# RuanJohn/Mava

Measured on AMD Instinct MI355X. Metric: env-steps/sec (whole node), ff_mappo RWARE tiny-4ag, higher is better.
Workload: dtype f32 via 2 x f16 split operands on the MFMA (3 products, f32 accumulate); 1 GPU; ff_mappo RWARE tiny-4ag-shaped synthetic obs, 4096 envs/GPU (update_batch_size=1 x num_envs=4096), rollout_length=128, ppo_epochs=4, num_minibatches=2, agents=4, obs=70/264, actions=5, one step = one PPO update = 524288 env-steps per GPU; parallelism=dp1

## Files before the change

### include/mava_hip.h

```cpp
#ifndef MAVA_HIP_H
#define MAVA_HIP_H

#include <stddef.h>
#include <stdint.h>

#ifdef __cplusplus
extern "C" {
#endif

typedef struct ihipStream_t* mava_stream_t;

const char* mava_last_error(void);
int mava_abi_version(void);

typedef struct mava_ctx mava_ctx;
enum {
  MAVA_CTX_MATMUL_MODE = 0,
  MAVA_CTX_CRITIC_AGGREGATION = 1,
  MAVA_CTX_GAE_VARIANT = 2,
  MAVA_CTX_POLICY_VARIANT = 3,
  MAVA_CTX_H2_LAUNCHES = 4,
  MAVA_CTX_TRAIN_VARIANT = 5,
  MAVA_CTX_W8_LAUNCHES = 6,
  MAVA_CTX_W1_SPLIT_FRESH = 7,
  MAVA_CTX_EXACT_TILES = 8,
  MAVA_CTX_X16_LAUNCHES = 9
};
int mava_ctx_create(mava_ctx** out);
int mava_ctx_destroy(mava_ctx* ctx);
int mava_ctx_set(mava_ctx* ctx, int key, long value);
int mava_ctx_get(const mava_ctx* ctx, int key, long* value);

int mava_gae_f32(const mava_ctx* ctx, const float* reward, const float* value, const uint8_t* done,
                 const float* last_val, const uint8_t* last_done, int T, int N, float gamma,
                 float lambda, float* adv, float* tgt, mava_stream_t s);

int mava_permutation_i32(long n, uint64_t seed, uint64_t counter, int32_t* out, mava_stream_t s);
int mava_permutation_batched_i32(long n, uint64_t seed, uint64_t counter, int n_perm, int32_t* out, long out_stride,
                                 mava_stream_t s);

int mava_clip_adam(float* p, const float* g, float* m, float* v, int32_t* count,
                   const int* seg_off, const float* seg_lr, int n_seg, float grad_scale,
                   float max_norm, int decay, int steps_per_update, int num_updates, float b1,
                   float b2, float eps, const float* loss_sums, float vf_coef, float ent_coef,
                   float* metrics_out, mava_stream_t s);

size_t mava_ppo_finish_workspace_bytes(int Pa, int Pc);
int mava_ppo_finish_f32(mava_ctx* ctx, const float* slab_a, long stride_a, const float* slab_c, long stride_c, int n_slab,
                        int Pa, int Pc, float* g, float* p, float* m, float* v, int32_t* count, float lr_a, float lr_c,
                        float grad_scale, float max_norm, int decay, int steps_per_update, int num_updates, float b1,
                        float b2, float eps, float vf_coef, float ent_coef, float* metrics_out, int critic_din,
                        void* workspace, size_t workspace_bytes, mava_stream_t s);

int mava_slab_reduce_f32(const float* slab, int n_slab, long slab_stride, int n, int accumulate,
                         float* out, mava_stream_t s);

int mava_slab_reduce2_f32(const float* slab, int n_slab, long slab_stride, int n_main,
                          float* out_main, int n_tail, float* out_tail, int accumulate,
                          mava_stream_t s);

int mava_mlp_param_count(int din, int n_out);

int mava_mlp_forward_f32(const mava_ctx* ctx, const float* params, int din, int n_out, const float* x, int x_share,
                         int rows, float* out, mava_stream_t s);

int mava_policy_step_f32(const mava_ctx* ctx, const float* actor_params, int actor_din, int n_actions,
                         const float* agents_view, const uint8_t* action_mask,
                         const float* critic_params, int critic_din, const float* critic_input,
                         int critic_share, int critic_rows, int value_broadcast, int rows,
                         uint64_t seed, uint32_t step, const uint32_t* step_base, uint32_t row_offset, int greedy,
                         const int32_t* forced_action, int32_t* action, float* log_prob,
                         float* value, float* logits, mava_stream_t s);


int mava_adv_stats_blocks(void);

int mava_adv_stats_f64(const float* advantages, const int32_t* idx, long idx_base, int Rb, int A,
                       double* partials, mava_stream_t s);
int mava_adv_stats_batched_f64(const float* advantages, const int32_t* idx, long idx_stride, int Rb, int A,
                               int n_batch, double* partials, mava_stream_t s);

int mava_ppo_actor_grad_f32(mava_ctx* ctx, const float* params, int din, int n_actions, const float* agents_view,
                            const uint8_t* action_mask, const int32_t* action,
                            const float* old_log_prob, const float* advantages,
                            const double* adv_stats, const int32_t* idx, long idx_base, int Rb,
                            int A, float clip_eps, float ent_coef, float* slab, long slab_stride,
                            int n_slab, mava_stream_t s);

int mava_policy_step_continuous_f32(const mava_ctx* ctx, const float* actor_params, int actor_din, int action_dim, float min_scale,
                                    const float* agents_view, const float* critic_params, int critic_din,
                                    const float* critic_input, int critic_share, int critic_rows,
                                    int value_broadcast, int rows, uint64_t seed, uint32_t step,
                                    const uint32_t* step_base, uint32_t row_offset, int greedy,
                                    const float* forced_action, float* action, float* log_prob, float* value,
                                    float* mean, mava_stream_t s);
int mava_ppo_actor_grad_continuous_f32(const float* params, int din, int action_dim, float min_scale, const float* agents_view,
                                       const float* action, const float* old_log_prob, const float* advantages,
                                       const double* adv_stats, const int32_t* idx, long idx_base, int Rb, int A,
                                       float clip_eps, float ent_coef, uint64_t seed, uint32_t ent_step,
                                       uint32_t row_offset, float* slab, long slab_stride, int n_slab,
                                       mava_stream_t s);

int mava_ppo_critic_grad_f32(mava_ctx* ctx, const float* params, int din, const float* critic_input, int x_share,
                             const float* old_value, const float* targets, const int32_t* idx,
                             long idx_base, int Rb, int A, float clip_eps, float vf_coef,
                             float* slab, long slab_stride, int n_slab, mava_stream_t s);

int mava_ppo_critic_grad_x16_f32(mava_ctx* ctx, const float* params, int din, const float* critic_input, int x_share,
                                 const float* old_value, const float* targets, const int32_t* idx,
                                 long idx_base, int Rb, int A, float clip_eps, float vf_coef,
                                 float* slab, long slab_stride, int n_slab, const uint16_t* input16,
                                 const uint32_t* input16_valid, mava_stream_t s);


int mava_synth_rware_step(int E, int A, int O, int n_actions, int gs_tiles, int state_dim, int time_limit,
                          uint64_t seed, uint32_t t, const uint32_t* t_base, uint32_t env_offset, int is_reset,
                          int32_t* step_count, float* run_return, int32_t* run_length,
                          float* ep_return, int32_t* ep_length, float* agents_view,
                          float* global_state, uint8_t* action_mask, int32_t* obs_step_count,
                          float* reward, uint8_t* done, float* info_return, int32_t* info_length,
                          uint8_t* info_terminal, const int32_t* action, int reward_mode, mava_stream_t s);

int mava_lbf_step(int E, int A, int F, int G, int fov, int max_agent_level, int force_coop, int individual_rewards,
                  int time_limit, uint64_t seed, uint32_t t, const uint32_t* t_base, uint32_t env_offset, int is_reset,
                  int32_t* agent_pos, int32_t* agent_level, int32_t* food_pos, int32_t* food_level, uint8_t* food_alive,
                  float* total_food_level, int32_t* step_count, float* run_return, int32_t* run_length,
                  float* ep_return, int32_t* ep_length, float* agents_view, float* global_state,
                  uint8_t* action_mask, int32_t* obs_step_count, float* reward, uint8_t* done, float* info_return,
                  int32_t* info_length, uint8_t* info_terminal, const int32_t* action, mava_stream_t s);

int mava_lbf_step_real_next(int E, int A, int F, int G, int fov, int max_agent_level, int force_coop, int individual_rewards,
                            int time_limit, uint64_t seed, uint32_t t, const uint32_t* t_base, uint32_t env_offset, int is_reset,
                            int32_t* agent_pos, int32_t* agent_level, int32_t* food_pos, int32_t* food_level, uint8_t* food_alive,
                            float* total_food_level, int32_t* step_count, float* run_return, int32_t* run_length,
                            float* ep_return, int32_t* ep_length, float* agents_view, float* global_state,
                            uint8_t* action_mask, int32_t* obs_step_count, float* reward, uint8_t* done, float* info_return,
                            int32_t* info_length, uint8_t* info_terminal, const int32_t* action, float* real_view,
                            uint8_t* real_mask, uint8_t* terminated, mava_stream_t s);

int mava_rware_step(int E, int A, int S, int R, int H, int W, int sensor_range, int time_limit, int collision_terminates,
                    const uint32_t* highway_rows, const int32_t* shelf_home, uint64_t seed, uint32_t t,
                    const uint32_t* t_base, uint32_t env_offset, int is_reset, int32_t* agent_pos, int32_t* agent_dir,
                    int32_t* agent_carry, int32_t* shelf_pos, int32_t* request_queue, int32_t* step_count,
                    float* run_return, int32_t* run_length, float* ep_return, int32_t* ep_length, float* agents_view,
                    float* global_state, uint8_t* action_mask, int32_t* obs_step_count, float* reward, uint8_t* done,
                    float* info_return, int32_t* info_length, uint8_t* info_terminal, const int32_t* action,
                    mava_stream_t s);

int mava_rware_step_real_next(int E, int A, int S, int R, int H, int W, int sensor_range, int time_limit,
                              int collision_terminates, const uint32_t* highway_rows, const int32_t* shelf_home,
                              uint64_t seed, uint32_t t, const uint32_t* t_base, uint32_t env_offset, int is_reset,
                              int32_t* agent_pos, int32_t* agent_dir, int32_t* agent_carry, int32_t* shelf_pos,
                              int32_t* request_queue, int32_t* step_count, float* run_return, int32_t* run_length,
                              float* ep_return, int32_t* ep_length, float* agents_view, float* global_state,
                              uint8_t* action_mask, int32_t* obs_step_count, float* reward, uint8_t* done,
                              float* info_return, int32_t* info_length, uint8_t* info_terminal, const int32_t* action,
                              float* real_view, uint8_t* real_mask, uint8_t* terminated, mava_stream_t s);

int mava_connector_step(int E, int A, int G, int time_limit, uint64_t seed, uint32_t t, const uint32_t* t_base,
                        uint32_t env_offset, int is_reset, int32_t* head, int32_t* target, uint8_t* connected,
                        uint8_t* grid, int32_t* step_count, float* run_return, int32_t* run_length, float* ep_return,
                        int32_t* ep_length, float* agents_view, float* global_state, uint8_t* action_mask,
                        int32_t* obs_step_count, float* reward, uint8_t* done, float* info_return, int32_t* info_length,
                        uint8_t* info_terminal, const int32_t* action, mava_stream_t s);

// ... 31 lines not shown
int mava_smax_step_real_next(int E, int A, int Ne, uint64_t ally_types, uint64_t enemy_types, int time_limit,
                             int see_enemy_actions, int walls_cause_death, uint64_t seed, uint32_t t,
                             const uint32_t* t_base, uint32_t env_offset, int is_reset, float* pos, float* health,
                             int32_t* cd, int32_t* last_action, int32_t* step_count, float* run_return,
                             int32_t* run_length, float* ep_return, int32_t* ep_length, float* agents_view,
                             float* global_state, uint8_t* action_mask, int32_t* obs_step_count, float* reward,
                             uint8_t* done, float* info_return, int32_t* info_length, uint8_t* info_terminal,
                             uint8_t* info_won, const int32_t* action, float* real_view, uint8_t* real_mask,
                             uint8_t* terminated, mava_stream_t s);

int mava_spread_step(int E, int A, int add_agent_id, int time_limit, uint64_t seed, uint32_t t, const uint32_t* t_base,
                     uint32_t env_offset, int is_reset, float* agent_pos, float* landmark_pos, int32_t* step_count,
                     float* run_return, int32_t* run_length, float* ep_return, int32_t* ep_length, float* agents_view,
                     float* global_state, uint8_t* action_mask, int32_t* obs_step_count, float* reward, uint8_t* done,
                     float* info_return, int32_t* info_length, uint8_t* info_terminal, const float* action,
                     mava_stream_t s);

int mava_spread_step_real_next(int E, int A, int add_agent_id, int time_limit, uint64_t seed, uint32_t t,
                               const uint32_t* t_base, uint32_t env_offset, int is_reset, float* agent_pos,
                               float* landmark_pos, int32_t* step_count, float* run_return, int32_t* run_length,
                               float* ep_return, int32_t* ep_length, float* agents_view, float* global_state,
                               uint8_t* action_mask, int32_t* obs_step_count, float* reward, uint8_t* done,
                               float* info_return, int32_t* info_length, uint8_t* info_terminal, const float* action,
                               float* real_view, uint8_t* real_mask, uint8_t* terminated, float* real_state,
                               mava_stream_t s);

int mava_rollout_ff_f32(const float* actor_params, int n_actions, const float* critic_params, int critic_shared,
                        int E, int A, int O, int T, int time_limit, uint64_t policy_seed, uint64_t env_seed,
                        uint32_t t0, uint32_t row_offset, uint32_t env_offset, int reward_mode,
                        int32_t* step_count, float* run_return, int32_t* run_length, float* ep_return,
                        int32_t* ep_length, float* agents_view, float* global_state, uint8_t* action_mask,
                        int32_t* obs_step_count, int32_t* action, float* value, float* reward, float* log_prob,
                        uint8_t* done, float* last_val, float* info_return, int32_t* info_length,
                        uint8_t* info_terminal, float* adv, float* tgt, float gamma, float gae_lambda, mava_stream_t s);
int mava_rollout_ff_tail_f32(const float* actor_params, int n_actions, const float* critic_params, int critic_shared,
                             int E, int A, int O, int T, int time_limit, uint64_t policy_seed, uint64_t env_seed,
                             uint32_t t0, uint32_t row_offset, uint32_t env_offset, int reward_mode,
                             int32_t* step_count, float* run_return, int32_t* run_length, float* ep_return,
                             int32_t* ep_length, float* agents_view, float* global_state, uint8_t* action_mask,
                             int32_t* obs_step_count, int32_t* action, float* value, float* reward, float* log_prob,
                             uint8_t* done, float* last_val, float* info_return, int32_t* info_length,
                             uint8_t* info_terminal, float* adv, float* tgt, float gamma, float gae_lambda,
                             float* last_reward, uint8_t* last_done, int32_t* step_counter, mava_stream_t s);
int mava_rollout_ff_x16_f32(const float* actor_params, int n_actions, const float* critic_params, int critic_shared,
                            int E, int A, int O, int T, int time_limit, uint64_t policy_seed, uint64_t env_seed,
                            uint32_t t0, uint32_t row_offset, uint32_t env_offset, int reward_mode,
                            int32_t* step_count, float* run_return, int32_t* run_length, float* ep_return,
                            int32_t* ep_length, float* agents_view, float* global_state, uint8_t* action_mask,
                            int32_t* obs_step_count, int32_t* action, float* value, float* reward, float* log_prob,
                            uint8_t* done, float* last_val, float* info_return, int32_t* info_length,
                            uint8_t* info_terminal, float* adv, float* tgt, float gamma, float gae_lambda,
                            float* last_reward, uint8_t* last_done, int32_t* step_counter, uint16_t* state16,
                            uint32_t* state16_valid, mava_stream_t s);
int mava_rollout_carry(int T, int E, int A, int obs_dim, long gs_dim, int n_actions, float* agents_view,
                       float* global_state, uint8_t* action_mask, int32_t* step_count, mava_stream_t s);


int mava_rec_dense_f32(const mava_ctx* ctx, const float* x, int x_rowmajor, const int32_t* idx, int Rm, int E, int A,
                       int x_share, int x_ld, int accumulate, const float* w, int ldw, const float* bias,
                       const float* gate, float* y, int y_ld, int K, int N, int rows, int relu, mava_stream_t s);

int mava_rec_xty_f32(const mava_ctx* ctx, const float* x, int x_rowmajor, const int32_t* idx, int Rm, int E, int A,
                     int x_share, int x_ld, const float* y, int y_ld, const float* y_tail, int y_split, int y_tail_ld, int K, int N,
                     int rows, int want_bias, float out_scale, float* slab, long slab_stride, int n_slab, mava_stream_t s);
int mava_rec_gather_t32_f32(const float* x, const int32_t* idx, int Rm, int E, int A, int x_share, int x_ld, int K,
                            int rows, int k_pad, float* out, mava_stream_t s);

int mava_gru_scan_fwd_f32(const mava_ctx* ctx, int T, int Rm, int E, int A, const int32_t* idx, const uint8_t* done,
                          const float* h0, int h0_t32, const float* wh, const float* bhn,
                          const float* gi, float* hs, float* hprev, float* saved, mava_stream_t s);

int mava_gru_scan_bwd_f32(const mava_ctx* ctx, int T, int Rm, int E, int A, const int32_t* idx, const uint8_t* done,
                          const float* wh, const float* saved, const float* hprev, const float* dh_out,
                          float* dgi, float* dgh, int dgh_n_only, mava_stream_t s);

int mava_seq_actor_loss_f32(int T, int Rm, int E, int A, int n_actions, const int32_t* idx,
                            const float* logits, const uint8_t* mask, const int32_t* action,
                            const float* old_log_prob, const float* advantages, const double* adv_stats,
                            int n_stats, float clip_eps, float ent_coef, float grad_scale, float* dlogits,
                            float* loss_partials, int n_blocks, mava_stream_t s);
int mava_seq_actor_loss_continuous_f32(int T, int Rm, int E, int A, int action_dim, float min_scale, const int32_t* idx,
                                       const float* mean, const float* log_std, const float* log_std_rows,
                                       const float* action, const float* old_log_prob, const float* advantages,
                                       const double* adv_stats, int n_stats, float clip_eps, float ent_coef, uint64_t seed,
                                       uint32_t ent_step, uint32_t row_offset, float grad_scale, float* dmean,
                                       float* dlog_std_rows, float* loss_partials, float* dscale_partials, int n_blocks,
                                       mava_stream_t s);
int mava_seq_sample_continuous_f32(int rows, int action_dim, float min_scale, const float* mean, const float* log_std,
                                   const float* log_std_rows, uint64_t seed,
                                   uint32_t step, uint32_t row_offset, int greedy, float* action, float* log_prob,
                                   mava_stream_t s);
int mava_seq_critic_loss_f32(int T, int Rm, int E, int A, int agents_per_row, const int32_t* idx, const float* values,
                             const float* old_value, const float* targets, float clip_eps, float vf_coef,
                             float grad_scale, float* dvalues, float* loss_partials, int n_blocks, mava_stream_t s);

int mava_rec_out_f32(int T, int Rm, int E, int A, int n_out, int agents_per_row, const int32_t* idx, const float* hs,
                     const float* params_post_head, const uint8_t* mask, const int32_t* action, const float* f0,
                     const float* f1, const double* adv_stats, int n_stats, float clip_eps, float coef, float grad_scale,
                     int is_actor, float* dh, float* slab, long slab_stride, int n_slab, mava_stream_t s);

int mava_seq_sample_f32(int rows, int n_actions, const float* logits, const uint8_t* mask, uint64_t seed,
                        uint32_t step, uint32_t row_offset, int greedy, int32_t* action, float* log_prob,
                        mava_stream_t s);

int mava_rec_step_f32(const float* actor_params, int actor_din, int n_actions, const float* agents_view,
                      const uint8_t* action_mask, const uint8_t* done_a, const float* h_actor_in,
// ... 131 lines not shown
```

### mava_amd/_lib.py

```python
from __future__ import annotations

import ctypes as C
import os
from typing import Optional

import torch

_HERE = os.path.dirname(os.path.abspath(__file__))
LIB_PATH = os.environ.get("MAVA_LIB_PATH") or os.path.join(_HERE, "libmavahip.so")

_lib: Optional[C.CDLL] = None


class MavaHipError(RuntimeError):
    pass


vp = C.c_void_p
i32 = C.c_int
u32 = C.c_uint32
u64 = C.c_uint64
f32 = C.c_float
lng = C.c_long

_SIGNATURES = {
    "mava_abi_version": [],
    "mava_ctx_create": [vp],
    "mava_ctx_destroy": [vp],
    "mava_ctx_set": [vp, i32, lng],
    "mava_ctx_get": [vp, i32, vp],
    "mava_gae_f32": [vp, vp, vp, vp, vp, vp, i32, i32, f32, f32, vp, vp, vp],
    "mava_permutation_i32": [lng, u64, u64, vp, vp],
    "mava_permutation_batched_i32": [lng, u64, u64, i32, vp, lng, vp],
    "mava_clip_adam": [vp, vp, vp, vp, vp, C.POINTER(i32), C.POINTER(f32), i32, f32, f32, i32, i32, i32,
                       f32, f32, f32, vp, f32, f32, vp, vp],
    "mava_slab_reduce_f32": [vp, i32, lng, i32, i32, vp, vp],
    "mava_ppo_finish_workspace_bytes": [i32, i32],
    "mava_ppo_finish_f32": [vp, vp, lng, vp, lng, i32, i32, i32, vp, vp, vp, vp, vp, f32, f32, f32, f32, i32, i32, i32, f32, f32, f32,
                            f32, f32, vp, i32, vp, C.c_size_t, vp],
    "mava_slab_reduce2_f32": [vp, i32, lng, i32, vp, i32, vp, i32, vp],
    "mava_mlp_param_count": [i32, i32],
    "mava_mlp_forward_f32": [vp, vp, i32, i32, vp, i32, i32, vp, vp],
    "mava_policy_step_f32": [vp, vp, i32, i32, vp, vp, vp, i32, vp, i32, i32, i32, i32, u64, u32, vp, u32, i32,
                             vp, vp, vp, vp, vp, vp],
    "mava_policy_step_continuous_f32": [vp, vp, i32, i32, f32, vp, vp, i32, vp, i32, i32, i32, i32, u64, u32, vp, u32, i32, vp, vp, vp, vp, vp, vp],
    "mava_ppo_actor_grad_continuous_f32": [vp, i32, i32, f32, vp, vp, vp, vp, vp, vp, lng, i32, i32, f32, f32, u64, u32, u32, vp, lng, i32, vp],
    "mava_seq_actor_loss_continuous_f32": [i32, i32, i32, i32, i32, f32, vp, vp, vp, vp, vp, vp, vp, vp, i32, f32, f32, u64, u32, u32, f32, vp, vp, vp, vp, i32, vp],
    "mava_seq_sample_continuous_f32": [i32, i32, f32, vp, vp, vp, u64, u32, u32, i32, vp, vp, vp],
    "mava_adv_stats_blocks": [],
    "mava_adv_stats_f64": [vp, vp, lng, i32, i32, vp, vp],
    "mava_adv_stats_batched_f64": [vp, vp, lng, i32, i32, i32, vp, vp],
    "mava_ppo_actor_grad_f32": [vp, vp, i32, i32, vp, vp, vp, vp, vp, vp, vp, lng, i32, i32, f32, f32, vp, lng, i32,
                                vp],
    "mava_ppo_critic_grad_f32": [vp, vp, i32, vp, i32, vp, vp, vp, lng, i32, i32, f32, f32, vp, lng, i32, vp],
    "mava_ppo_critic_grad_x16_f32": [vp, vp, i32, vp, i32, vp, vp, vp, lng, i32, i32, f32, f32, vp, lng, i32, vp, vp, vp],
    "mava_synth_rware_step": [i32, i32, i32, i32, i32, i32, i32, u64, u32, vp, u32, i32] + [vp] * 14 + [vp, i32, vp],
    "mava_lbf_step": [i32] * 9 + [u64, u32, vp, u32, i32] + [vp] * 21 + [vp],
    "mava_lbf_step_real_next": [i32] * 9 + [u64, u32, vp, u32, i32] + [vp] * 24 + [vp],
    "mava_rware_step": [i32] * 9 + [vp, vp, u64, u32, vp, u32, i32] + [vp] * 20 + [vp],
    "mava_rware_step_real_next": [i32] * 9 + [vp, vp, u64, u32, vp, u32, i32] + [vp] * 23 + [vp],
    "mava_connector_step": [i32] * 4 + [u64, u32, vp, u32, i32] + [vp] * 19 + [vp],
    "mava_connector_step_real_next": [i32] * 4 + [u64, u32, vp, u32, i32] + [vp] * 22 + [vp],
    "mava_cleaner_step": [i32] * 5 + [u64, u32, vp, u32, i32] + [vp] * 18 + [vp],
    "mava_cleaner_step_real_next": [i32] * 5 + [u64, u32, vp, u32, i32] + [vp] * 21 + [vp],
    "mava_smax_step": [i32] * 3 + [u64, u64] + [i32] * 3 + [u64, u32, vp, u32, i32] + [vp] * 20 + [vp],
    "mava_smax_step_real_next": [i32] * 3 + [u64, u64] + [i32] * 3 + [u64, u32, vp, u32, i32] + [vp] * 23 + [vp],
    "mava_spread_step": [i32] * 4 + [u64, u32, vp, u32, i32] + [vp] * 17 + [vp],
    "mava_spread_step_real_next": [i32] * 4 + [u64, u32, vp, u32, i32] + [vp] * 21 + [vp],
    "mava_rec_q_step_f32": [vp, i32, i32, vp, vp, vp, vp, vp, i32, f32, u64, u32, u32, vp, vp, vp],
    "mava_replay_add_f32": [i32] * 6 + [vp] * 16 + [vp],
    "mava_replay_sample_f32": [i32] * 5 + [u32, i32, i32, i32, u64, u32] + [vp] * 17 + [vp],
    "mava_q_td_loss_f32": [i32, i32, i32, i32] + [vp] * 7 + [f32, f32, vp, vp, i32, vp],
    "mava_target_update_f32": [lng, vp, vp, f32, i32, vp],
    "mava_qmix_state_t32_f32": [i32] * 6 + [vp] * 4 + [vp],
    "mava_qmix_td_f32": [i32] * 7 + [vp] * 15 + [f32, f32] + [vp] * 6 + [i32, vp],
    "mava_sac_replay_add_f32": [i32] * 7 + [vp] * 14 + [vp],
    "mava_sac_replay_sample_f32": [i32] * 5 + [u32, i32, i32, u64, u32] + [vp] * 15 + [vp],
    "mava_sac_sample_f32": [i32, i32, i32, f32, vp, vp, u64, u32, u32, vp, vp, vp, vp],
    "mava_sac_concat_f32": [i32] * 7 + [vp] * 4 + [i32, vp],
    "mava_sac_q_loss_f32": [i32] * 3 + [vp] * 8 + [f32, f32] + [vp] * 4 + [i32, vp],
    "mava_sac_actor_grad_f32": [i32] * 4 + [f32] + [vp] * 9 + [i32, i32, i32, f32, f32] + [vp] * 3 + [i32, vp],
    "mava_sac_alpha_loss_f32": [i32, i32, vp, vp, f32, vp, vp, vp],
    "mava_rollout_ff_f32": [vp, i32, vp, i32, i32, i32, i32, i32, i32, u64, u64, u32, u32, u32, i32] + [vp] * 18 + [vp, vp, f32, f32, vp],
    "mava_rollout_ff_tail_f32": [vp, i32, vp, i32, i32, i32, i32, i32, i32, u64, u64, u32, u32, u32, i32] + [vp] * 18
                                + [vp, vp, f32, f32, vp, vp, vp, vp],
    "mava_rollout_ff_x16_f32": [vp, i32, vp, i32, i32, i32, i32, i32, i32, u64, u64, u32, u32, u32, i32] + [vp] * 18
                               + [vp, vp, f32, f32, vp, vp, vp, vp, vp, vp],
    "mava_rollout_carry": [i32, i32, i32, i32, lng, i32, vp, vp, vp, vp, vp],
    "mava_rec_dense_f32": [vp, vp, i32, vp, i32, i32, i32, i32, i32, i32, vp, i32, vp, vp, vp, i32, i32, i32, i32, i32, vp],
    "mava_rec_xty_f32": [vp, vp, i32, vp, i32, i32, i32, i32, i32, vp, i32, vp, i32, i32, i32, i32, i32, i32, f32, vp, lng, i32, vp],
    "mava_rec_gather_t32_f32": [vp, vp, i32, i32, i32, i32, i32, i32, i32, i32, vp, vp],
    "mava_gru_scan_fwd_f32": [vp, i32, i32, i32, i32, vp, vp, vp, i32, vp, vp, vp, vp, vp, vp, vp],
    "mava_t32_gru_mask_f32": [vp, vp, vp, i32, i32, i32, lng, vp, vp],
    "mava_t32_gru_gates_f32": [vp, vp, vp, vp, i32, lng, vp, vp, vp, vp, vp, i32, i32, vp],
    "mava_t32_gru_gates_bwd_f32": [vp, vp, vp, vp, vp, vp, vp, i32, i32, i32, lng, vp, vp, vp, vp],
    "mava_gru_scan_bwd_f32": [vp, i32, i32, i32, i32, vp, vp, vp, vp, vp, vp, vp, vp, i32, vp],
    "mava_seq_actor_loss_f32": [i32, i32, i32, i32, i32, vp, vp, vp, vp, vp, vp, vp, i32, f32, f32, f32, vp, vp, i32, vp],
    "mava_rec_step_continuous_f32": [vp, i32, i32, f32, vp, vp, vp, vp, i32, u64, u32, u32, i32, vp, vp, vp, i32, vp, i32, vp, i32, vp, vp, i32, i32, vp, vp],
    "mava_rec_step_f32": [vp, i32, i32, vp, vp, vp, vp, vp, i32, u64, u32, u32, i32, vp, vp, vp, i32, vp, i32, vp, i32, vp, vp,
                          i32, i32, vp, vp],
    "mava_seq_critic_loss_f32": [i32, i32, i32, i32, i32, vp, vp, vp, vp, f32, f32, f32, vp, vp, i32, vp],
    "mava_rec_out_f32": [i32, i32, i32, i32, i32, i32, vp, vp, vp, vp, vp, vp, vp, vp, i32, f32, f32, f32, i32, vp, vp, lng, i32, vp],
    "mava_rec_step_pack_bytes": [i32],
    "mava_t32_norm_act_f32": [vp, i32, lng, i32, vp, i32, vp, vp, vp, vp],
    "mava_t32_norm_act_bwd_f32": [vp, vp, i32, lng, i32, vp, vp, i32, vp, vp, vp],
    "mava_t32_colsum_f32": [vp, i32, lng, f32, vp, lng, i32, vp],
    "mava_t32_im2col_f32": [vp, i32, lng, i32, i32, i32, i32, i32, vp, vp],
    "mava_t32_col2im_f32": [vp, i32, lng, i32, i32, i32, i32, i32, vp, vp],
    "mava_t32_flatten_f32": [vp, lng, i32, i32, i32, vp, vp],
    "mava_comm_unique_id": [vp],
    "mava_comm_create": [vp, i32, i32, vp],
    "mava_allreduce_sum_f32": [vp, vp, C.c_size_t, vp],
    "mava_broadcast_f32": [vp, vp, C.c_size_t, i32, vp],
    "mava_comm_destroy": [vp],
    "mava_rec_step_pack_f32": [vp, i32, vp, vp],
    "mava_rec_step_packed_f32": [vp, vp, vp, i32, i32, f32, vp, vp, vp, vp, vp, i32, u64, u32, u32, i32, vp, vp, vp, vp, i32, vp, i32, vp, i32, vp, vp, i32, i32, vp, vp],
    "mava_seq_sample_f32": [i32, i32, vp, vp, u64, u32, u32, i32, vp, vp, vp],
    "mava_t32_convert_f32": [vp, i32, i32, i32, vp, vp],
    "mava_mat_attn_fwd_f32": [vp, vp, vp, lng, i32, i32, i32, i32, i32, vp, vp, i32, vp],
    "mava_mat_attn_bwd_f32": [vp, vp, vp, vp, lng, i32, i32, i32, i32, i32, vp, vp, vp, i32, vp],
    "mava_mat_ln_fwd_f32": [vp, vp, vp, vp, i32, lng, lng, vp, vp, vp, i32, vp],
    "mava_mat_ln_bwd_f32": [vp, vp, vp, vp, i32, lng, lng, f32, vp, vp, lng, i32, vp],
    "mava_mat_gelu_f32": [vp, lng, vp, vp],
    "mava_mat_gelu_bwd_f32": [vp, vp, lng, vp, vp],
    "mava_mat_shift_onehot_f32": [vp, vp, i32, i32, i32, i32, lng, i32, vp, vp],
    "mava_mat_sample_f32": [i32, i32, i32, i32, vp, vp, u64, u32, u32, i32, vp, vp, vp],
    "mava_mat_loss_f32": [i32, i32, i32, lng, vp, vp, vp, vp, vp, vp, vp, vp, vp, vp, i32, f32, f32, f32, f32, vp, vp, vp, i32, vp],
}
_RESTYPES = {"mava_last_error": C.c_char_p, "mava_rec_step_pack_bytes": C.c_long, "mava_ppo_finish_workspace_bytes": C.c_size_t}


def declared_symbols():
    return sorted(set(_SIGNATURES) | set(_RESTYPES))


def lib() -> C.CDLL:
    global _lib
    if _lib is None:
        if not os.path.exists(LIB_PATH):
            raise MavaHipError(
                f"{LIB_PATH} is missing: build it with `python -m mava_amd.build` "
                "(hipcc --offload-arch=gfx950). There is no CPU fallback."
            )
        _lib = C.CDLL(LIB_PATH)
        _lib.mava_last_error.restype = C.c_char_p
        _lib.mava_last_error.argtypes = []
        for name, args in _SIGNATURES.items():
            fn = getattr(_lib, name)
            fn.argtypes = args
            fn.restype = _RESTYPES.get(name, C.c_int)
    return _lib


class Ctx:

    MATMUL_MODE, CRITIC_AGGREGATION, GAE_VARIANT, POLICY_VARIANT, H2_LAUNCHES, TRAIN_VARIANT, W8_LAUNCHES, W1_SPLIT_FRESH = 0, 1, 2, 3, 4, 5, 6, 7
    EXACT_TILES = 8
    X16_LAUNCHES = 9

    def __init__(self, matmul_mode: str = "f32", critic_aggregation: bool = True):
        if matmul_mode not in ("f32", "f16x2"):
            raise ValueError(f"matmul_mode must be 'f16x2' or 'f32', got {matmul_mode!r}")
        h = C.c_void_p()
        check(lib().mava_ctx_create(C.byref(h)), "mava_ctx_create")
        self.handle: Optional[int] = h.value
        self.set(self.MATMUL_MODE, 1 if matmul_mode == "f16x2" else 0)
        self.set(self.CRITIC_AGGREGATION, int(bool(critic_aggregation)))

    def set(self, key: int, value: int) -> None:
        check(lib().mava_ctx_set(self.handle, key, int(value)), "mava_ctx_set")

    def get(self, key: int) -> int:
        out = C.c_long()
        check(lib().mava_ctx_get(self.handle, key, C.byref(out)), "mava_ctx_get")
        return int(out.value)

    @property
    def matmul_mode(self) -> str:
        return "f16x2" if self.get(self.MATMUL_MODE) == 1 else "f32"

    @property
    def h2_launches(self) -> int:
        return self.get(self.H2_LAUNCHES)

    def close(self) -> None:
        if getattr(self, "handle", None) is not None and _lib is not None:
            _lib.mava_ctx_destroy(self.handle)
        self.handle = None

    def __del__(self):
        try:
            self.close()
        except Exception:
            pass


def ctx_ptr(ctx: Optional["Ctx"]) -> Optional[int]:
    return None if ctx is None else ctx.handle


def check(rc: int, what: str) -> None:
    if rc != 0:
        msg = lib().mava_last_error().decode("utf-8", "replace")
        raise MavaHipError(f"{what} failed with code {rc}: {msg}")


TIMERS: Optional[dict] = None


def launch(what: str, fn, *args, ok=(0,)) -> int:
    if TIMERS is None:
# ... 21 lines not shown
```

### mava_amd/csrc/api.cpp

```cpp
#include <stdarg.h>
#include <stdio.h>
#include <string.h>

#include "common.h"
#include "ctx.h"

static thread_local char g_err[512] = "";

void mava_set_error(const char* fmt, ...) {
  va_list ap;
  va_start(ap, fmt);
  vsnprintf(g_err, sizeof(g_err), fmt, ap);
  va_end(ap);
}

extern "C" const char* mava_last_error(void) { return g_err; }

extern "C" int mava_abi_version(void) { return 3; }

enum { CTX_MATMUL_MODE = 0, CTX_CRITIC_AGGREGATION = 1, CTX_GAE_VARIANT = 2, CTX_POLICY_VARIANT = 3, CTX_H2_LAUNCHES = 4, CTX_TRAIN_VARIANT = 5, CTX_W8_LAUNCHES = 6, CTX_W1_SPLIT_FRESH = 7, CTX_EXACT_TILES = 8, CTX_X16_LAUNCHES = 9 };

extern "C" int mava_ctx_create(mava_ctx** out) {
  MAVA_ARG_CHECK(out != nullptr, 0, "mava_ctx_create: null output pointer");
  mava_ctx* c = new mava_ctx();
  c->matmul_mode = 0;
  c->critic_aggregation = 1;
  c->gae_variant = 0;
  c->policy_variant = 0;
  c->h2_launches = 0;
  c->train_variant = 0;
  c->w8_launches = 0;
  c->w1_split[0] = c->w1_split[1] = nullptr;
  for (int i = 0; i < 2; ++i) {
    c->w1_fresh[i] = 0;
    c->w1_key_params[i] = nullptr;
    c->w1_key_din[i] = c->w1_key_steps[i] = 0;
  }
  c->exact_tiles = nullptr;
  *out = c;
  return MAVA_OK;
}

extern "C" int mava_ctx_destroy(mava_ctx* c) {
  if (c == nullptr) return MAVA_OK;
  for (int i = 0; i < 2; ++i)
    if (c->w1_split[i] != nullptr) (void)hipFree(c->w1_split[i]);
  if (c->exact_tiles != nullptr) (void)hipFree(c->exact_tiles);
  delete c;
  return MAVA_OK;
}

extern "C" int mava_ctx_set(mava_ctx* c, int key, long value) {
  MAVA_ARG_CHECK(c != nullptr, 0, "mava_ctx_set: null context");
  switch (key) {
    case CTX_MATMUL_MODE:
      MAVA_ARG_CHECK(value == 0 || value == 1, 1, "mava_ctx_set: matmul mode %ld (0 = exact f32, 1 = f16x2)", value);
      c->matmul_mode = (int)value;
      c->w1_fresh[0] = c->w1_fresh[1] = 0;
      return MAVA_OK;
    case CTX_CRITIC_AGGREGATION: c->critic_aggregation = value ? 1 : 0; return MAVA_OK;
    case CTX_GAE_VARIANT: c->gae_variant = (int)value; return MAVA_OK;
    case CTX_POLICY_VARIANT: c->policy_variant = (int)value; return MAVA_OK;
    case CTX_H2_LAUNCHES: c->h2_launches = value; return MAVA_OK;
    case CTX_TRAIN_VARIANT: c->train_variant = (int)value; return MAVA_OK;
    case CTX_W8_LAUNCHES: c->w8_launches = value; return MAVA_OK;
    case CTX_W1_SPLIT_FRESH:
      MAVA_ARG_CHECK(value == 0, 1, "mava_ctx_set: MAVA_CTX_W1_SPLIT_FRESH can only be cleared (0) by the caller");
      c->w1_fresh[0] = c->w1_fresh[1] = 0;
      return MAVA_OK;
    case CTX_EXACT_TILES:
      MAVA_ARG_CHECK(value == 0, 1, "mava_ctx_set: MAVA_CTX_EXACT_TILES can only be reset (0) by the caller");
      if (c->exact_tiles != nullptr) {
        MAVA_HIP_CHECK(hipDeviceSynchronize());
        MAVA_HIP_CHECK(hipMemset(c->exact_tiles, 0, sizeof(unsigned long long)));
      }
      return MAVA_OK;
    case CTX_X16_LAUNCHES:
      MAVA_ARG_CHECK(value == 0, 1, "mava_ctx_set: MAVA_CTX_X16_LAUNCHES can only be reset (0) by the caller");
      if (c->exact_tiles != nullptr) {
        MAVA_HIP_CHECK(hipDeviceSynchronize());
        MAVA_HIP_CHECK(hipMemset(c->exact_tiles + 1, 0, sizeof(unsigned long long)));
      }
      return MAVA_OK;
    default: mava_set_error("mava_ctx_set: unknown key %d", key); return MAVA_EARG(2);
  }
}

extern "C" int mava_ctx_get(const mava_ctx* c, int key, long* value) {
  MAVA_ARG_CHECK(c != nullptr && value != nullptr, 0, "mava_ctx_get: null argument");
  switch (key) {
    case CTX_MATMUL_MODE: *value = c->matmul_mode; return MAVA_OK;
    case CTX_CRITIC_AGGREGATION: *value = c->critic_aggregation; return MAVA_OK;
    case CTX_GAE_VARIANT: *value = c->gae_variant; return MAVA_OK;
    case CTX_POLICY_VARIANT: *value = c->policy_variant; return MAVA_OK;
    case CTX_H2_LAUNCHES: *value = c->h2_launches; return MAVA_OK;
    case CTX_TRAIN_VARIANT: *value = c->train_variant; return MAVA_OK;
    case CTX_W8_LAUNCHES: *value = c->w8_launches; return MAVA_OK;
    case CTX_W1_SPLIT_FRESH: *value = c->w1_fresh[1]; return MAVA_OK;
    case CTX_EXACT_TILES:
    case CTX_X16_LAUNCHES: {
      unsigned long long n = 0;
      if (c->exact_tiles != nullptr) {
        MAVA_HIP_CHECK(hipDeviceSynchronize());
        MAVA_HIP_CHECK(hipMemcpy(&n, c->exact_tiles + (key == CTX_X16_LAUNCHES ? 1 : 0), sizeof(n), hipMemcpyDeviceToHost));
      }
      *value = (long)n;
      return MAVA_OK;
    }
    default: mava_set_error("mava_ctx_get: unknown key %d", key); return MAVA_EARG(2);
  }
}
```

### mava_amd/csrc/ppo_train.hip

```cpp
#include "mlp_core.h"
#include "ppo_train_task.h"
#include "ctx.h"
#include "tanh_normal.h"

namespace {

constexpr int STATS_BLOCKS = 128;
constexpr int LDT = 33;


#ifdef MAVA_STAMPS
#define STAMP_DECL unsigned long long st_prev = __builtin_readcyclecounter(), st_acc[16] = {0, 0, 0, 0, 0, 0, 0, 0, 0, 0, 0, 0, 0, 0, 0, 0};
#define STAMP(i)                                                   \
  do {                                                             \
    const unsigned long long st_now = __builtin_readcyclecounter(); \
    st_acc[i] += st_now - st_prev;                                 \
    st_prev = st_now;                                              \
  } while (0)
#else
#define STAMP_DECL
#define STAMP(i)
#endif

struct TrainLdsLayout {
// ... 799 lines not shown
  switch (kt) {
    case 1: return launch_xv<NO, 1, ACTOR, CONT>(tk, n_slab, s);
    case 2: return launch_xv<NO, 2, ACTOR, CONT>(tk, n_slab, s);
    case 3: return launch_xv<NO, 3, ACTOR, CONT>(tk, n_slab, s);
    case 4: return launch_xv<NO, 4, ACTOR, CONT>(tk, n_slab, s);
    case 5: case 6: return launch_xv<NO, 6, ACTOR, CONT>(tk, n_slab, s);
    case 7: case 8: case 9: return launch_xv<NO, 9, ACTOR, CONT>(tk, n_slab, s);
    default:
      mava_set_error("ppo_train: input width %d > 287 is not instantiated", tk.din);
      return MAVA_EARG(9);
  }
#endif
}

}

#ifdef MAVA_STAMPS
static unsigned long long* g_stamps = nullptr;
extern "C" int mava_debug_set_stamps(unsigned long long* p) {
  g_stamps = p;
  return MAVA_OK;
}
#else
static constexpr unsigned long long* g_stamps = nullptr;
#endif


extern "C" int mava_adv_stats_blocks(void) { return STATS_BLOCKS; }

int g_train_last_instance = 0;
extern "C" int mava_debug_train_last_instance(void) { return g_train_last_instance; }

extern "C" int mava_adv_stats_f64(const float* adv, const int32_t* idx, long idx_base, int Rb, int A,
                                  double* partials, hipStream_t s) {
  MAVA_ARG_CHECK(Rb >= 1 && A >= 1, 0, "mava_adv_stats_f64: Rb=%d A=%d", Rb, A);
  MAVA_ARG_CHECK(adv && partials, 1, "mava_adv_stats_f64: null pointer argument");
  hipLaunchKernelGGL(adv_stats_kernel, dim3(STATS_BLOCKS), dim3(256), 0, s, adv, idx, idx_base, Rb, A,
                     partials, 0L);
  MAVA_LAUNCH_CHECK();
  return MAVA_OK;
}

extern "C" int mava_adv_stats_batched_f64(const float* adv, const int32_t* idx, long idx_stride, int Rb, int A,
                                          int n_batch, double* partials, hipStream_t s) {
  MAVA_ARG_CHECK(Rb >= 1 && A >= 1 && n_batch >= 1 && n_batch <= 65535 && idx_stride >= 0, 0,
                 "mava_adv_stats_batched_f64: Rb=%d A=%d n_batch=%d idx_stride=%ld", Rb, A, n_batch, idx_stride);
  MAVA_ARG_CHECK(adv && idx && partials, 1, "mava_adv_stats_batched_f64: null pointer argument");
  hipLaunchKernelGGL(adv_stats_kernel, dim3(STATS_BLOCKS, n_batch), dim3(256), 0, s, adv, idx, 0L, Rb, A, partials,
                     idx_stride);
  MAVA_LAUNCH_CHECK();
  return MAVA_OK;
}

extern "C" int mava_ppo_actor_grad_f32(mava_ctx* ctx, const float* params, int din, int n_actions,
                                       const float* agents_view, const uint8_t* action_mask,
                                       const int32_t* action, const float* old_log_prob,
                                       const float* advantages, const double* adv_stats,
                                       const int32_t* idx, long idx_base, int Rb, int A,
                                       float clip_eps, float ent_coef, float* slab, long slab_stride,
                                       int n_slab, hipStream_t s) {
  MAVA_ARG_CHECK(din >= 1 && n_actions >= 1 && n_actions <= 32, 0,
                 "mava_ppo_actor_grad_f32: din=%d n_actions=%d unsupported", din, n_actions);
  MAVA_ARG_CHECK(Rb >= 1 && A >= 1 && n_slab >= 1 && n_slab <= 1024 && (long)Rb * A < (1L << 31), 1,
                 "mava_ppo_actor_grad_f32: Rb=%d A=%d n_slab=%d", Rb, A, n_slab);
  MAVA_ARG_CHECK(slab_stride >= mlp_param_count(din, n_actions) + 2, 2,
                 "mava_ppo_actor_grad_f32: slab_stride too small");
  MAVA_ARG_CHECK(params && agents_view && action && old_log_prob && advantages && adv_stats && slab, 3,
                 "mava_ppo_actor_grad_f32: null pointer argument");
  TrainTask tk = {};
  tk.params = params; tk.x = agents_view; tk.din = din; tk.no = n_actions; tk.xshare = 1; tk.agg = 1;
  tk.xv = pick_xv(agents_view, din); tk.A = A; tk.idx = idx; tk.idx_base = idx_base; tk.Rb = Rb;
  tk.mask = action_mask; tk.action = action; tk.old_logp = old_log_prob; tk.adv = advantages;
  tk.stats = adv_stats; tk.clip_eps = clip_eps; tk.ent_coef = ent_coef; tk.slab = slab;
  tk.slab_stride = slab_stride;
  tk.stamps = g_stamps;
  if (mava_ctx_matmul_mode(ctx) == 1) {
    const int rc = mava_train_h2_launch(ctx, tk, n_slab, true, s);
    if (rc <= 0) return rc;
  }
  if (n_actions <= 8) return dispatch_kt<8, true>(tk, n_slab, s);
  if (n_actions <= 16) return dispatch_kt<16, true>(tk, n_slab, s);
  return dispatch_kt<32, true>(tk, n_slab, s);
}

extern "C" int mava_ppo_actor_grad_continuous_f32(const float* params, int din, int action_dim, float min_scale,
                                                  const float* agents_view, const float* action,
                                                  const float* old_log_prob, const float* advantages,
                                                  const double* adv_stats, const int32_t* idx, long idx_base, int Rb,
                                                  int A, float clip_eps, float ent_coef, uint64_t seed,
                                                  uint32_t ent_step, uint32_t row_offset, float* slab,
                                                  long slab_stride, int n_slab, hipStream_t s) {
  MAVA_ARG_CHECK(din >= 1 && action_dim >= 1 && action_dim <= 16, 0,
                 "mava_ppo_actor_grad_continuous_f32: din=%d action_dim=%d unsupported (action_dim <= 16)", din,
                 action_dim);
  MAVA_ARG_CHECK(Rb >= 1 && A >= 1 && n_slab >= 1 && n_slab <= 1024 && (long)Rb * A < (1L << 31), 1,
                 "mava_ppo_actor_grad_continuous_f32: Rb=%d A=%d n_slab=%d", Rb, A, n_slab);
  MAVA_ARG_CHECK(slab_stride >= mlp_param_count(din, action_dim) + action_dim + 2, 2,
                 "mava_ppo_actor_grad_continuous_f32: slab_stride too small");
  MAVA_ARG_CHECK(params && agents_view && action && old_log_prob && advantages && adv_stats && slab, 3,
                 "mava_ppo_actor_grad_continuous_f32: null pointer argument");
  TrainTask tk = {};
  tk.params = params; tk.x = agents_view; tk.din = din; tk.no = action_dim; tk.xshare = 1; tk.agg = 1;
  tk.xv = pick_xv(agents_view, din); tk.A = A; tk.idx = idx; tk.idx_base = idx_base; tk.Rb = Rb;
  tk.action_f = action; tk.old_logp = old_log_prob; tk.adv = advantages;
  tk.stats = adv_stats; tk.clip_eps = clip_eps; tk.ent_coef = ent_coef; tk.slab = slab;
  tk.slab_stride = slab_stride;
  tk.seed_lo = (uint32_t)seed; tk.seed_hi = (uint32_t)(seed >> 32); tk.ent_step = ent_step; tk.row_offset = row_offset;
  tk.min_scale = min_scale;
  tk.stamps = g_stamps;
  if (action_dim <= 8) return dispatch_kt<8, true, true>(tk, n_slab, s);
  return dispatch_kt<16, true, true>(tk, n_slab, s);
}

static int critic_grad_impl(mava_ctx* ctx, const float* params, int din, const float* critic_input, int x_share,
                            const float* old_value, const float* targets, const int32_t* idx, long idx_base, int Rb, int A,
                            float clip_eps, float vf_coef, float* slab, long slab_stride, int n_slab, const uint16_t* input16,
                            const uint32_t* input16_valid, hipStream_t s) {
  MAVA_ARG_CHECK(din >= 1 && x_share >= 1, 0, "mava_ppo_critic_grad_f32: din=%d x_share=%d", din, x_share);
  MAVA_ARG_CHECK(Rb >= 1 && A >= 1 && n_slab >= 1 && n_slab <= 1024 && (long)Rb * A < (1L << 31), 1,
                 "mava_ppo_critic_grad_f32: Rb=%d A=%d n_slab=%d", Rb, A, n_slab);
  MAVA_ARG_CHECK(slab_stride >= mlp_param_count(din, 1) + 2, 2,
                 "mava_ppo_critic_grad_f32: slab_stride too small");
  MAVA_ARG_CHECK(params && critic_input && old_value && targets && slab, 3,
                 "mava_ppo_critic_grad_f32: null pointer argument");
  TrainTask tk = {};
  tk.params = params; tk.x = critic_input; tk.din = din; tk.no = 1; tk.xshare = x_share; tk.agg = 1;
  if (mava_ctx_critic_aggregation(ctx) && A > 1 && A <= 8 && x_share == A) {
    tk.agg = A;
    tk.xshare = 1;
  }
  tk.xv = pick_xv(critic_input, din); tk.A = A; tk.idx = idx; tk.idx_base = idx_base; tk.Rb = Rb;
  tk.old_value = old_value; tk.targets = targets; tk.clip_eps = clip_eps; tk.vf_coef = vf_coef;
  tk.slab = slab; tk.slab_stride = slab_stride;
  tk.stamps = g_stamps;
  tk.x16 = reinterpret_cast<const _Float16*>(input16); tk.x16_valid = input16_valid;
  int rc = 1;
  if (mava_ctx_matmul_mode(ctx) == 1) rc = mava_train_h2_launch(ctx, tk, n_slab, false, s);
  if (ctx != nullptr) ctx->w1_fresh[1] = 0;
  if (rc <= 0) return rc;
  return dispatch_kt<1, false>(tk, n_slab, s);
}

extern "C" int mava_ppo_critic_grad_f32(mava_ctx* ctx, const float* params, int din, const float* critic_input,
                                        int x_share, const float* old_value, const float* targets,
                                        const int32_t* idx, long idx_base, int Rb, int A,
                                        float clip_eps, float vf_coef, float* slab, long slab_stride,
                                        int n_slab, hipStream_t s) {
  return critic_grad_impl(ctx, params, din, critic_input, x_share, old_value, targets, idx, idx_base, Rb, A, clip_eps, vf_coef,
                          slab, slab_stride, n_slab, nullptr, nullptr, s);
}

extern "C" int mava_ppo_critic_grad_x16_f32(mava_ctx* ctx, const float* params, int din, const float* critic_input,
                                            int x_share, const float* old_value, const float* targets,
                                            const int32_t* idx, long idx_base, int Rb, int A,
                                            float clip_eps, float vf_coef, float* slab, long slab_stride,
                                            int n_slab, const uint16_t* input16, const uint32_t* input16_valid,
                                            hipStream_t s) {
  MAVA_ARG_CHECK((input16 == nullptr) == (input16_valid == nullptr), 3,
                 "mava_ppo_critic_grad_x16_f32: input16 and input16_valid go together");
  return critic_grad_impl(ctx, params, din, critic_input, x_share, old_value, targets, idx, idx_base, Rb, A, clip_eps, vf_coef,
                          slab, slab_stride, n_slab, input16, input16_valid, s);
}
```

### mava_amd/csrc/ppo_train_h2.hip

```cpp
#include "h2_core.h"
#include "ppo_train_task.h"
#include "ctx.h"

#include <type_traits>

#ifndef MAVA_GW_DEPTH
#define MAVA_GW_DEPTH 0
#endif
#define GW_DEPTH MAVA_GW_DEPTH
#ifndef MAVA_GW_DEPTH_WIDE
#define MAVA_GW_DEPTH_WIDE 0
#endif
#ifndef MAVA_P1_EARLY_HALVES
#define MAVA_P1_EARLY_HALVES 2
#endif
#ifndef MAVA_P1_EARLY_RING
#define MAVA_P1_EARLY_RING 3
#endif

namespace {

using namespace h2;

constexpr int STATS_BLOCKS = 128;
// ... 1022 lines not shown
      slab[Pn + 1] = ((red[4 * NO + 1] + red[4 * NO + 3]) + red[4 * NO + 5]) + red[4 * NO + 7];
    }
  } else {
#pragma unroll
    for (int q = 0; q < 16; ++q) {
      float v = aW3r[q];
#pragma unroll
      for (int m = 1; m < 32; m <<= 1) v += __shfl_xor(v, m, 64);
      if (r == 0) slab[oW3 + 32 * w + (q & 3) + 8 * (q >> 2) + 4 * h] = v * invR;
    }
    float v = ab3, l = loss_a;
    for (int o = 32; o > 0; o >>= 1) {
      v += __shfl_down(v, o, 64);
      l += __shfl_down(l, o, 64);
    }
    if (lane == 0) { red[2 * w] = v; red[2 * w + 1] = l; }
    __syncthreads();
    if (tid == 0) {
      slab[oB3] = (((red[0] + red[2]) + red[4]) + red[6]) * invR;
      slab[Pn] = ((red[1] + red[3]) + red[5]) + red[7];
      slab[Pn + 1] = 0.0f;
    }
  }
}

template <int NO, int S1, bool ACTOR, bool WIDE, int XV>
__global__ __launch_bounds__(WIDE ? 512 : 256, WIDE ? 2 : 1) void ppo_train_h2_kernel(TrainTask tk, H2Layout L,
                                                                                     const uint4* __restrict__ w1p) {
  extern __shared__ __attribute__((aligned(16))) u8 lds[];
  if constexpr (WIDE) {
    constexpr bool X16_CAPABLE = !ACTOR && XV == 4;
    bool x16 = false;
    if constexpr (X16_CAPABLE) {
      if (tk.x16_valid != nullptr) x16 = __builtin_amdgcn_readfirstlane((int)*tk.x16_valid) == 1;
    }
    if (X16_CAPABLE && x16) {
      if constexpr (X16_CAPABLE) {
        if (threadIdx.x < 256) {
          h2_body<NO, S1, ACTOR, WIDE, XV, 1, true>(tk, L, w1p, lds);
        } else {
          h2_body<NO, S1, ACTOR, WIDE, XV, 2, true>(tk, L, w1p, lds);
        }
      }
    } else if (threadIdx.x < 256) {
      h2_body<NO, S1, ACTOR, WIDE, XV, 1>(tk, L, w1p, lds);
    } else {
      h2_body<NO, S1, ACTOR, WIDE, XV, 2>(tk, L, w1p, lds);
    }
  } else {
    h2_body<NO, S1, ACTOR, WIDE, XV, 0>(tk, L, w1p, lds);
  }
}

template <int NO, int S1, bool ACTOR, bool WIDE, int XV>
int launch_h2(mava_ctx* ctx, const TrainTask& tk, int n_slab, hipStream_t s) {
  const H2Layout L = make_h2_layout<NO, S1, WIDE>(ACTOR);
  MAVA_ARG_CHECK(L.end <= 163840, 8, "ppo_train_h2: %d bytes of LDS exceed the 160 KiB of a CU", L.end);
  static bool attr_set = false;
  if (!attr_set) {
    MAVA_HIP_CHECK(hipFuncSetAttribute((const void*)ppo_train_h2_kernel<NO, S1, ACTOR, WIDE, XV>,
                                       hipFuncAttributeMaxDynamicSharedMemorySize, L.end));
    attr_set = true;
  }
  const uint4* w1p = nullptr;
  if (WIDE) {
    void*& slot = ctx->w1_split[ACTOR ? 0 : 1];
    if (slot == nullptr) MAVA_HIP_CHECK(hipMalloc(&slot, W1_SPLIT_BYTES));
    uint4* const buf = static_cast<uint4*>(slot);
    const int kind = ACTOR ? 0 : 1;
    int& fresh = ctx->w1_fresh[kind];
    const bool keyed = ctx->w1_key_params[kind] == tk.params && ctx->w1_key_din[kind] == tk.din && ctx->w1_key_steps[kind] == S1;
    if (!(fresh && keyed)) {
      hipLaunchKernelGGL((pack_w1_kernel<S1>), dim3(1), dim3(256), 0, s, tk.params, tk.din, buf, ACTOR ? 1.0f : W_SCALE_CRITIC);
      MAVA_LAUNCH_CHECK();
    }
    fresh = 0;
    w1p = buf;
    if (ctx->exact_tiles == nullptr) {
      void* word = nullptr;
      MAVA_HIP_CHECK(hipMalloc(&word, 2 * sizeof(unsigned long long)));
      ctx->exact_tiles = static_cast<unsigned long long*>(word);
      MAVA_HIP_CHECK(hipMemsetAsync(word, 0, 2 * sizeof(unsigned long long), s));
    }
  }
  TrainTask tkl = tk;
  tkl.exact_tiles = WIDE ? ctx->exact_tiles : nullptr;
  const bool x16_ok = WIDE && !ACTOR && XV == 4 && tk.x16 != nullptr && tk.x16_valid != nullptr && tk.din % 8 == 0 &&
                      (uintptr_t)tk.x16 % 16 == 0 && tk.force_xlo == 0;
  if (!x16_ok) { tkl.x16 = nullptr; tkl.x16_valid = nullptr; }
  tkl.x16_launches = x16_ok ? ctx->exact_tiles + 1 : nullptr;
  g_train_last_instance = train_instance_id(2, ACTOR, false, WIDE, NO, S1, XV);
  hipLaunchKernelGGL((ppo_train_h2_kernel<NO, S1, ACTOR, WIDE, XV>), dim3(n_slab), dim3(WIDE ? 512 : 256), L.end, s, tkl, L,
                     w1p);
  MAVA_LAUNCH_CHECK();
  return MAVA_OK;
}

template <int NO, int S1, bool ACTOR, bool WIDE>
int dispatch_xv(mava_ctx* ctx, const TrainTask& tk, int n_slab, hipStream_t s) {
  const uintptr_t a = (uintptr_t)tk.x;
  if constexpr (WIDE) {
    if (tk.din % 4 == 0 && a % 16 == 0) return launch_h2<NO, S1, ACTOR, WIDE, 4>(ctx, tk, n_slab, s);
  } else {
    if (tk.din % 2 == 0 && a % 8 == 0) return launch_h2<NO, S1, ACTOR, WIDE, 2>(ctx, tk, n_slab, s);
  }
  return launch_h2<NO, S1, ACTOR, WIDE, 1>(ctx, tk, n_slab, s);
}

template <int NO, bool ACTOR>
int dispatch_s1(mava_ctx* ctx, const TrainTask& tk, int n_slab, hipStream_t s) {
  const int s1 = (tk.din + 1 + 15) / 16;
  switch (s1) {
#ifndef MAVA_FAST_BUILD
    case 1: return dispatch_xv<NO, 1, ACTOR, false>(ctx, tk, n_slab, s);
    case 2: return dispatch_xv<NO, 2, ACTOR, false>(ctx, tk, n_slab, s);
    case 3: return dispatch_xv<NO, 3, ACTOR, false>(ctx, tk, n_slab, s);
    case 4: return dispatch_xv<NO, 4, ACTOR, false>(ctx, tk, n_slab, s);
    case 6: return dispatch_xv<NO, 6, ACTOR, false>(ctx, tk, n_slab, s);
    case 7: case 8: case 9: case 10: case 11: case 12: return dispatch_xv<NO, 12, ACTOR, true>(ctx, tk, n_slab, s);
#endif
    case 5: return dispatch_xv<NO, 5, ACTOR, false>(ctx, tk, n_slab, s);
    case 13: case 14: case 15: case 16: case 17: case 18: return dispatch_xv<NO, 18, ACTOR, true>(ctx, tk, n_slab, s);
    default: return 1;
  }
}

}

static int h2_dispatch(mava_ctx* ctx, const TrainTask& tk, int n_slab, bool actor, hipStream_t s) {
  if (actor) {
    if (tk.action_f != nullptr) return 1;
    if (tk.no <= 8) return dispatch_s1<8, true>(ctx, tk, n_slab, s);
#ifndef MAVA_FAST_BUILD
    if (tk.no <= 16) return dispatch_s1<16, true>(ctx, tk, n_slab, s);
    return dispatch_s1<32, true>(ctx, tk, n_slab, s);
#else
    return 1;
#endif
  }
  return dispatch_s1<1, false>(ctx, tk, n_slab, s);
}

int mava_train_h2_launch(mava_ctx* ctx, const TrainTask& tk_in, int n_slab, bool actor, hipStream_t s) {
  TrainTask tk = tk_in;
  tk.force_xlo = (ctx->train_variant & 2) != 0;
  if ((ctx->train_variant & 1) == 0) {
    const int rc8 = mava_train_w8_launch(tk, n_slab, actor, s);
    if (rc8 <= 0) {
      if (rc8 == 0) { ++ctx->h2_launches; ++ctx->w8_launches; }
      return rc8;
    }
  }
  const int rc = h2_dispatch(ctx, tk, n_slab, actor, s);
  if (rc == 0) ++ctx->h2_launches;
  return rc;
}
```

### mava_amd/csrc/ppo_train_task.h

```cpp
#pragma once
#include <stdint.h>

#include "common.h"

struct TrainTask {
  const float* params;
  const float* x;
  int din, no, xshare, xv;
  int A;
  int agg;
  const int32_t* idx;
  long idx_base;
  int Rb;
  const uint8_t* mask;
  const int32_t* action;
  const float* action_f;
  uint32_t seed_lo, seed_hi, ent_step, row_offset;
  float min_scale;
  const float* old_logp;
  const float* adv;
  const double* stats;
  const float* old_value;
  const float* targets;
  float clip_eps, ent_coef, vf_coef;
  float* slab;
  long slab_stride;
  unsigned long long* stamps;
  int force_xlo;
  unsigned long long* exact_tiles;
  const _Float16* x16;
  const uint32_t* x16_valid;
  unsigned long long* x16_launches;
};

struct mava_ctx;
int mava_train_w8_launch(const TrainTask& tk, int n_slab, bool actor, hipStream_t s);
int mava_train_h2_launch(mava_ctx* ctx, const TrainTask& tk, int n_slab, bool actor, hipStream_t s);

extern int g_train_last_instance;
constexpr int train_instance_id(int family, bool actor, bool cont, bool wide, int no, int k, int xv) {
  return family * 1000000 + ((actor ? 1 : 0) + (cont ? 2 : 0) + (wide ? 4 : 0)) * 100000 + no * 1000 + k * 10 + xv;
}
```

### mava_amd/csrc/ppo_train_w8.hip

```cpp
#include "h2_core.h"
#include "ppo_train_task.h"
#include "ctx.h"

namespace {

using namespace h2;
typedef float f32x4 __attribute__((ext_vector_type(4)));

constexpr int STATS_BLOCKS = 128;
#ifndef MAVA_W8_GWD
#define MAVA_W8_GWD 1
#endif
constexpr int GWD = MAVA_W8_GWD;

#ifdef MAVA_STAMPS
#define WSTAMP_DECL unsigned long long ws_prev = __builtin_readcyclecounter(), ws_acc[16] = {0, 0, 0, 0, 0, 0, 0, 0, 0, 0, 0, 0, 0, 0, 0, 0};
#define WSTAMP(i)                                                   \
  do {                                                              \
    __builtin_amdgcn_sched_barrier(0);                              \
    const unsigned long long ws_now = __builtin_readcyclecounter(); \
    ws_acc[i] += ws_now - ws_prev;                                  \
    ws_prev = ws_now;                                               \
    __builtin_amdgcn_sched_barrier(0);                              \
  } while (0)
// ... 10 lines not shown
  c = __builtin_amdgcn_mfma_f32_16x16x32_f16(a.hi, b.lo, c, 0, 0, 0);
  return __builtin_amdgcn_mfma_f32_16x16x32_f16(a.hi, b.hi, c, 0, 0, 0);
}
__device__ __forceinline__ f32x4 mfma2w_blo0(const Frag& a, const half8& bhi, f32x4 c) {
  c = __builtin_amdgcn_mfma_f32_16x16x32_f16(a.lo, bhi, c, 0, 0, 0);
  return __builtin_amdgcn_mfma_f32_16x16x32_f16(a.hi, bhi, c, 0, 0, 0);
}
__device__ __forceinline__ f32x4 mfma2w_alo0(const half8& ahi, const Frag& b, f32x4 c) {
  c = __builtin_amdgcn_mfma_f32_16x16x32_f16(ahi, b.lo, c, 0, 0, 0);
  return __builtin_amdgcn_mfma_f32_16x16x32_f16(ahi, b.hi, c, 0, 0, 0);
}
__device__ __forceinline__ f32x4 mfma3k16(const Frag4& a, const Frag4& b, f32x4 c) {
  c = __builtin_amdgcn_mfma_f32_16x16x16f16(a.lo, b.hi, c, 0, 0, 0);
  c = __builtin_amdgcn_mfma_f32_16x16x16f16(a.hi, b.lo, c, 0, 0, 0);
  return __builtin_amdgcn_mfma_f32_16x16x16f16(a.hi, b.hi, c, 0, 0, 0);
}
__device__ __forceinline__ Frag4 split4(const f32x4& v) {
  Frag4 f;
#pragma unroll
  for (int r = 0; r < 4; ++r) {
    _Float16 a, b;
    split1(v[r], a, b);
    f.hi[r] = a;
    f.lo[r] = b;
  }
  return f;
}

constexpr int WROW = 256;
constexpr int WPLANE32 = 32 * WROW;
constexpr int WIMG = 2 * WPLANE32;
constexpr int W2PLANE = 128 * WROW;
constexpr int DYROW = 48;
constexpr int DYPLANE = 32 * DYROW;
__host__ __device__ inline int w8_sw(int row) { return ((row & 3) << 1) | (((row >> 3) & 1) * 9); }
__host__ __device__ inline int w8_off(int row, int chunk) { return WROW * row + 16 * (chunk ^ w8_sw(row)); }

struct W8Layout {
  int h1, dz2, dz1, w2, xs, dy, small, end;
};
inline W8Layout make_w8_layout() {
  W8Layout L;
  L.h1 = 0;
  L.dz2 = L.h1 + WIMG;
  L.dz1 = L.dz2 + WIMG;
  L.w2 = L.dz1 + WIMG;
  L.xs = L.w2 + 2 * W2PLANE;
  L.dy = L.xs + 2 * WIMG;
  L.small = L.dy + 2 * DYPLANE;
  L.end = L.small + (32 + 16 + 16) * 4;
  return L;
}

template <int NO, int S1, int XV, int W2R, bool ACTOR, int ROLE>
__device__ __forceinline__ void w8_body(const TrainTask& tk, const W8Layout& L, u8* lds) {
  constexpr bool DO_LOSS = ROLE != 2, DO_STAGE = ROLE != 1;
  constexpr float WS = ACTOR ? 1.0f : W_SCALE_CRITIC, WU = 1.0f / WS;
  constexpr int KT1 = 2 * S1;
  u8* const H1I = lds + L.h1;
  u8* const DZ2I = lds + L.dz2;
  u8* const DZ1I = lds + L.dz1;
  u8* const W2I = lds + L.w2;
  u8* const DYI = lds + L.dy;
  float* const YP = reinterpret_cast<float*>(lds + L.dz2);
  constexpr int YSTR = (NO == 8) ? 9 : NO;
  float* const B3s = reinterpret_cast<float*>(lds + L.small);
  float* const misc = B3s + 32;
  unsigned* const xflag = reinterpret_cast<unsigned*>(misc + 2);

  const int tid = threadIdx.x;
  const int l = tid & 63, v = tid >> 6, i = l & 15, kg = l >> 4;
  const int din = tk.din, no = tk.no;
  const long R = (long)tk.Rb * tk.A;
  const float invR = 1.0f / (float)R;
  const float* const P = tk.params;
  const int oW2 = mlp_off_w2(din), oW3 = mlp_off_w3(din);

  for (int o = tid * 16; o < L.end; o += 512 * 16) *reinterpret_cast<uint4*>(lds + o) = make_uint4(0, 0, 0, 0);
  __syncthreads();
  if (tid < no) B3s[tid] = P[mlp_off_b3(din, no) + tid];
  if (tid < 64) {
    const int b = tid >> 5, row = tid & 31;
    *reinterpret_cast<_Float16*>(lds + L.xs + b * WIMG + w8_off(row, din >> 3) + 2 * (din & 7)) = (_Float16)1.0f;
  }
  {
    const int n = tid & 127, k0 = 32 * (tid >> 7);
    float carry = 0.0f;
#pragma unroll 8
    for (int k = k0; k < k0 + 32; ++k) {
      _Float16 x0, x1;
      split1_carry(P[oW2 + k * MLP_H + n] * WS, carry, x0, x1);
      const int o = w8_off(k, n >> 3) + 2 * (n & 7);
      *reinterpret_cast<_Float16*>(W2I + o) = x0;
      *reinterpret_cast<_Float16*>(W2I + W2PLANE + o) = x1;
    }
  }
  if (ACTOR && tid == 0) {
    double s1 = 0.0, s2 = 0.0;
    for (int b = 0; b < STATS_BLOCKS; ++b) { s1 += tk.stats[2 * b]; s2 += tk.stats[2 * b + 1]; }
    const double mean = s1 / (double)R;
    double var = s2 / (double)R - mean * mean;
    if (var < 0.0) var = 0.0;
    misc[0] = (float)mean;
    misc[1] = 1.0f / ((float)sqrt(var) + 1e-8f);
  }
  Frag W1f[S1], W2f[W2R > 0 ? W2R : 1];
  {
    float c1 = 0.0f, c2 = 0.0f;
#pragma unroll
// ... 40 lines not shown
  float ab2[4] = {0, 0, 0, 0}, ab3 = 0.0f, loss_a = 0.0f, loss_b = 0.0f;

  constexpr int LOSS_THREADS = 32 * NO;
  static_assert(ROLE == 0 ? LOSS_THREADS == 512 : LOSS_THREADS == 256, "role split belongs to 8 action lanes");
  const int lrow = tid / NO, lo = tid & (NO - 1);
  constexpr int TPR = (ROLE == 2) ? 8 : 16;
  const int st = (ROLE == 2) ? (tid - 256) : tid;
  const int srow = st / TPR, l16 = st % TPR;
  const int nv = din / XV;
  constexpr int NPC = (32 * S1 / XV + TPR - 1) / TPR;
  constexpr int NR = DO_STAGE ? NPC * XV : 1;
  const uint32_t Au = (uint32_t)tk.A;
  const uint32_t q_step = 32u * gridDim.x, b_step = q_step / Au, a_step = q_step % Au;
  const uint32_t b_last = (uint32_t)(R - 1) / Au, a_last = (uint32_t)(R - 1) % Au;
  struct Cursor { uint32_t q, b, a; };
  auto cursor_at = [&](int rr) {
    Cursor c;
    c.q = 32u * blockIdx.x + (uint32_t)rr;
    c.b = c.q / Au;
    c.a = c.q - c.b * Au;
    return c;
  };
  auto cursor_advance = [&](Cursor& c) {
    c.q += q_step; c.b += b_step; c.a += a_step;
    if (c.a >= Au) { c.a -= Au; c.b += 1u; }
  };
  auto cursor_gather = [&](const Cursor& c, int32_t& p_raw, uint32_t& a_out) {
    const bool in = c.q < (uint32_t)R;
    const uint32_t b = in ? c.b : b_last;
    a_out = in ? c.a : a_last;
    p_raw = tk.idx ? tk.idx[b] : (int32_t)(tk.idx_base + (long)b);
  };
  auto stage_row = [&](int32_t p_raw, uint32_t a) -> uint32_t {
    const uint32_t fr = (uint32_t)p_raw * Au + a;
    if constexpr (ACTOR) return fr;
    else return (tk.xshare == 1) ? fr : ((uint32_t)tk.xshare == Au ? (uint32_t)p_raw : fr / (uint32_t)tk.xshare);
  };
  auto stage_issue = [&](uint32_t fr, float (&xr)[NR]) {
    const float* xrow = tk.x + (long)fr * din;
#pragma unroll
    for (int k = 0; k < NPC; ++k) {
      const int c = l16 + TPR * k;
      const int cc = (c < nv) ? c : 0;
      if (XV == 2) {
        const float2 t = reinterpret_cast<const float2*>(xrow)[cc];
        xr[2 * k] = t.x; xr[2 * k + 1] = t.y;
      } else {
        xr[k] = xrow[cc];
      }
    }
  };
  u8* const xs_dummy = reinterpret_cast<u8*>(misc + 8);
  const int xsw = 16 * w8_sw(srow);
  auto stage_commit = [&](int buf, const float (&xr)[NR]) {
    u8* base = lds + L.xs + buf * WIMG + WROW * srow;
    uint32_t lo_any = 0;
#pragma unroll
    for (int k = 0; k < NPC; ++k) {
      const int c = l16 + TPR * k;
      const bool ok = c < nv;
      const int col = XV * c;
      u8* qa = ok ? (base + ((16 * (col >> 3)) ^ xsw) + 2 * (col & 7)) : xs_dummy;
      u8* qb = ok ? (qa + WPLANE32) : xs_dummy;
      if (XV == 2) {
        typedef _Float16 half2v __attribute__((ext_vector_type(2)));
        half2v a, b;
#pragma unroll
        for (int e = 0; e < 2; ++e) { _Float16 x0, x1; split1(xr[2 * k + e], x0, x1); a[e] = x0; b[e] = x1; }
        *reinterpret_cast<half2v*>(qa) = a;
        *reinterpret_cast<half2v*>(qb) = b;
        lo_any |= __builtin_bit_cast(uint32_t, b) & 0x7FFF7FFFu;
      } else {
        _Float16 x0, x1;
        split1(xr[k], x0, x1);
        *reinterpret_cast<_Float16*>(qa) = x0;
        *reinterpret_cast<_Float16*>(qb) = x1;
        lo_any |= (uint32_t)__builtin_bit_cast(uint16_t, x1) & 0x7FFFu;
      }
    }
    if (lo_any != 0) xflag[buf] = 1u;
  };
  auto load_row = [&](uint32_t fr, int& act, float& f0, float& f1, uint32_t& m) {
    if constexpr (ACTOR) {
      act = tk.action[fr];
      f0 = tk.old_logp[fr];
      f1 = tk.adv[fr];
      const uint8_t* mk = (tk.mask != nullptr && lo < no) ? (tk.mask + (long)fr * no + lo) : nullptr;
      m = 1u;
      if (mk != nullptr) m = *mk;
    } else {
      act = 0;
      f0 = tk.old_value[fr];
      f1 = tk.targets[fr];
      m = 0u;
    }
  };

  const long ntiles = (R + 31) / 32;
  long it = blockIdx.x;
  float xr[NR];
  int r_act = 0, n_act = 0;
  float r_f0 = 0.0f, r_f1 = 0.0f, n_f0 = 0.0f, n_f1 = 0.0f;
  uint32_t r_m = 1u, n_m = 1u;
  Cursor cs = cursor_at(DO_STAGE ? srow : 0), cl = cursor_at(DO_LOSS ? lrow : 0);
  int32_t ps_next = 0, pl_next = 0;
  uint32_t as_next = 0, al_next = 0;
  if (it < ntiles) {
    if constexpr (DO_STAGE) {
      cursor_gather(cs, ps_next, as_next);
      stage_issue(stage_row(ps_next, as_next), xr);
    }
    if constexpr (DO_LOSS) {
      cursor_gather(cl, pl_next, al_next);
      load_row((uint32_t)pl_next * Au + al_next, r_act, r_f0, r_f1, r_m);
    }
    if constexpr (DO_STAGE) {
      stage_commit(0, xr);
      cursor_advance(cs);
    }
    if constexpr (DO_LOSS) cursor_advance(cl);
    if (it + gridDim.x < ntiles) {
      if constexpr (DO_STAGE) { cursor_gather(cs, ps_next, as_next); cursor_advance(cs); }
      if constexpr (DO_LOSS) { cursor_gather(cl, pl_next, al_next); cursor_advance(cl); }
    }
  }
  __syncthreads();

  const int swi = w8_sw(i);
  int rdA[4];
#pragma unroll
  for (int s = 0; s < 4; ++s) rdA[s] = WROW * i + 16 * ((4 * s + kg) ^ swi);
  const int wrA = WROW * i + 16 * ((2 * v + (kg >> 1)) ^ swi) + 8 * (kg & 1);
  const int tq = i >> 2, tp = i & 3;
  const int trow = 8 * kg + tq;
  const int trb = WROW * trow + 8 * (tp & 1);
  const int thx = 16 * ((tp >> 1) ^ w8_sw(trow));
  int trA[8];
#pragma unroll
  for (int t = 0; t < 8; ++t) {
    trA[t] = trb + ((32 * t) ^ thx);
    asm volatile("" : "+v"(trA[t]));
  }
  auto tr_addr = [&](int t) -> int { return trA[t]; };
  const int trOwn = tr_addr(v);
  auto read_tr = [&](const u8* img, int plane, int a0) -> Frag {
    Frag f;
    f.hi = read_tr8(img + a0, WROW);
    f.lo = read_tr8(img + plane + a0, WROW);
    return f;
  };
  auto read_row = [&](const u8* img, int plane, int a0) -> Frag { return read_row_frag(img, plane, a0); };
  const int dyRd = DYROW * i + 8 * kg;
  const int dyTr = DYROW * trow + 8 * tp;
  int buf = 0;

  WSTAMP_DECL
  for (; it < ntiles; it += gridDim.x, buf ^= 1) {
    WSTAMP(14);
    const long itn = it + gridDim.x;
    const bool have_next = itn < ntiles;
    const u8* const XSI = lds + L.xs + buf * WIMG;
    uint32_t xrow_next = DO_STAGE ? stage_row(ps_next, as_next) : 0u, lrow_next = DO_LOSS ? ((uint32_t)pl_next * Au + al_next) : 0u;
    if constexpr (DO_STAGE) asm volatile("" : "+v"(xrow_next));
    if constexpr (DO_LOSS) asm volatile("" : "+v"(lrow_next));

    f32x4 acc[2] = {f32x4{0, 0, 0, 0}, f32x4{0, 0, 0, 0}};
    const bool x_lo = __builtin_amdgcn_readfirstlane((int)xflag[buf]) != 0 || tk.force_xlo != 0;
    if (x_lo) {
      Frag xb[2];
#pragma unroll
      for (int nt = 0; nt < 2; ++nt) xb[nt] = read_row(XSI + 4096 * nt, WPLANE32, rdA[0]);
#pragma unroll
      for (int s = 0; s < S1; ++s) {
        Frag b[2] = {xb[0], xb[1]};
        if (s + 1 < S1) {
#pragma unroll
          for (int nt = 0; nt < 2; ++nt) xb[nt] = read_row(XSI + 4096 * nt, WPLANE32, rdA[(s + 1) & 3]);
        }
#pragma unroll
        for (int nt = 0; nt < 2; ++nt) acc[nt] = mfma3w(W1f[s], b[nt], acc[nt]);
        __builtin_amdgcn_sched_barrier(0);
      }
    } else {
      half8 xb[2];
#pragma unroll
      for (int nt = 0; nt < 2; ++nt) xb[nt] = *reinterpret_cast<const half8*>(XSI + 4096 * nt + rdA[0]);
#pragma unroll
      for (int s = 0; s < S1; ++s) {
        const half8 b[2] = {xb[0], xb[1]};
        if (s + 1 < S1) {
#pragma unroll
          for (int nt = 0; nt < 2; ++nt) xb[nt] = *reinterpret_cast<const half8*>(XSI + 4096 * nt + rdA[(s + 1) & 3]);
        }
#pragma unroll
        for (int nt = 0; nt < 2; ++nt) acc[nt] = mfma2w_blo0(W1f[s], b[nt], acc[nt]);
        __builtin_amdgcn_sched_barrier(0);
      }
    }
    WSTAMP(0);
    uint32_t relu1 = 0;
#pragma unroll
    for (int nt = 0; nt < 2; ++nt) {
#pragma unroll
      for (int r = 0; r < 4; ++r) {
        acc[nt][r] = fmaxf(ACTOR ? acc[nt][r] : acc[nt][r] * WU, 0.0f);
        relu1 |= (acc[nt][r] > 0.0f) ? (1u << (4 * nt + r)) : 0u;
      }
      const Frag4 f = split4(acc[nt]);
      *reinterpret_cast<half4*>(H1I + 4096 * nt + wrA) = f.hi;
      *reinterpret_cast<half4*>(H1I + 4096 * nt + WPLANE32 + wrA) = f.lo;
    }
    WSTAMP(1);
    if (have_next) {
      if constexpr (DO_STAGE) stage_issue(xrow_next, xr);
      if constexpr (DO_LOSS) load_row(lrow_next, n_act, n_f0, n_f1, n_m);
      if (itn + gridDim.x < ntiles) {
        if constexpr (DO_STAGE) { cursor_gather(cs, ps_next, as_next); cursor_advance(cs); }
        if constexpr (DO_LOSS) { cursor_gather(cl, pl_next, al_next); cursor_advance(cl); }
      }
    }
    WSTAMP(2);
    __syncthreads();
    WSTAMP(3);
    if constexpr (DO_STAGE) {
      if (tid == (ROLE == 2 ? 256 : 0)) xflag[buf ^ 1] = 0u;
    }

    f32x4 h2[2];
#pragma unroll
    for (int nt = 0; nt < 2; ++nt) h2[nt] = f32x4{b2r[0], b2r[1], b2r[2], b2r[3]};
    {
      Frag hb[2], wn;
#pragma unroll
      for (int nt = 0; nt < 2; ++nt) hb[nt] = read_row(H1I + 4096 * nt, WPLANE32, rdA[0]);
      if constexpr (W2R < 1) wn = read_tr(W2I, W2PLANE, trOwn);
#pragma unroll
      for (int s = 0; s < 4; ++s) {
        Frag b[2] = {hb[0], hb[1]};
        const Frag a = (s < W2R) ? W2f[s < W2R ? s : 0] : wn;
        if (s + 1 < 4) {
#pragma unroll
          for (int nt = 0; nt < 2; ++nt) hb[nt] = read_row(H1I + 4096 * nt, WPLANE32, rdA[s + 1]);
          if (s + 1 >= W2R) wn = read_tr(W2I + 32 * (s + 1) * WROW, W2PLANE, trOwn);
        }
#pragma unroll
        for (int nt = 0; nt < 2; ++nt) h2[nt] = mfma3w(a, b[nt], h2[nt]);
        __builtin_amdgcn_sched_barrier(0);
      }
    }
    WSTAMP(4);
    uint32_t relu2 = 0;
#pragma unroll
    for (int nt = 0; nt < 2; ++nt) {
#pragma unroll
      for (int r = 0; r < 4; ++r) {
        h2[nt][r] = fmaxf(ACTOR ? h2[nt][r] : h2[nt][r] * WU, 0.0f);
        relu2 |= (h2[nt][r] > 0.0f) ? (1u << (4 * nt + r)) : 0u;
      }
      const Frag4 f = split4(h2[nt]);
      *reinterpret_cast<half4*>(DZ1I + 4096 * nt + wrA) = f.hi;
      *reinterpret_cast<half4*>(DZ1I + 4096 * nt + WPLANE32 + wrA) = f.lo;
      const f32x4 y = mfma3k16(W3h, f, f32x4{0, 0, 0, 0});
#pragma unroll
      for (int r = 0; r < 4; ++r) {
        if (4 * kg + r < NO) YP[(v * 32 + 16 * nt + i) * YSTR + 4 * kg + r] = y[r] * W3_UNSCALE;
      }
    }
    WSTAMP(5);
    __syncthreads();
    WSTAMP(6);

    if constexpr (DO_LOSS) {
      const float lo_c = 1.0f - tk.clip_eps, hi_c = 1.0f + tk.clip_eps;
      const bool rvalid = (it * 32 + lrow) < R;
      const float* yp = YP + lrow * YSTR + lo;
      float y = B3s[lo];
#pragma unroll
// ... 1 lines not shown
      float dyo = 0.0f, pg_row = 0.0f, ent_row = 0.0f;
      if constexpr (ACTOR) {
        const bool legal = (lo < no) && (r_m != 0u);
        const float z = legal ? y : -FLT_MAX;
        auto fmax_op = [](float a, float b) { return fmaxf(a, b); };
        auto add_op = [](float a, float b) { return a + b; };
        const float mx = group_allreduce<NO>(z, fmax_op);
        const float se = group_allreduce<NO>(expf(z - mx), add_op);
        const float logp = (mx == -FLT_MAX) ? ((lo < no) ? -logf((float)no) : -FLT_MAX) : z - (mx + logf(se));
        const float pr = expf(logp);
        const float ent = group_allreduce<NO>((pr > 0.0f) ? -(pr * logp) : 0.0f, add_op);
        const int act = r_act;
        const float lp = group_allreduce<NO>((lo == act) ? logp : 0.0f, add_op);
        const float gae = (r_f1 - adv_mean) * adv_rstd;
        const float ratio = expf(lp - r_f0);
        const float rc = fminf(fmaxf(ratio, lo_c), hi_c);
        const float l1 = ratio * gae, l2 = rc * gae;
        const float pg = -fminf(l1, l2);
        const bool inside = (ratio >= lo_c) && (ratio <= hi_c);
        const float g1 = (l1 < l2) ? 1.0f : ((l1 == l2) ? 0.5f : 0.0f);
        const float g2 = inside ? (1.0f - g1) : 0.0f;
        const float dlp = rvalid ? (-(g1 + g2) * gae * ratio) : 0.0f;
        const float ec = rvalid ? tk.ent_coef : 0.0f;
        const float oh = (lo == act) ? 1.0f : 0.0f;
        const float pl2 = (pr > 0.0f) ? logp : 0.0f;
        dyo = dlp * (oh - pr) + ec * pr * (pl2 + ent);
        if (z == -FLT_MAX) dyo = 0.0f;
        pg_row = pg;
        ent_row = ent;
      } else {
        const float ov = r_f0, tg = r_f1;
        const float diff = y - ov;
        const float vclip = ov + fminf(fmaxf(diff, -tk.clip_eps), tk.clip_eps);
        const float e1 = y - tg, e2 = vclip - tg;
        const float l1 = e1 * e1, l2 = e2 * e2;
        const bool inside = (diff >= -tk.clip_eps) && (diff <= tk.clip_eps);
        const float g1 = (l1 > l2) ? 1.0f : ((l1 == l2) ? 0.5f : 0.0f);
        const float g2 = inside ? (1.0f - g1) : 0.0f;
        dyo = (rvalid && lo == 0) ? (tk.vf_coef * (g1 * e1 + g2 * e2)) : 0.0f;
        pg_row = 0.5f * fmaxf(l1, l2);
      }
      _Float16 da, db;
      split1(dyo, da, db);
      *reinterpret_cast<_Float16*>(DYI + lrow * DYROW + 2 * lo) = da;
      *reinterpret_cast<_Float16*>(DYI + DYPLANE + lrow * DYROW + 2 * lo) = db;
      ab3 += dyo;
      if (rvalid && lo == 0) {
        loss_a += pg_row * invR;
        loss_b += ent_row * invR;
      }
      r_act = n_act; r_f0 = n_f0; r_f1 = n_f1; r_m = n_m;
    }
    if constexpr (DO_STAGE) {
      if (have_next) stage_commit(buf ^ 1, xr);
    }
    WSTAMP(7);
    __syncthreads();
    WSTAMP(8);

    {
      Frag a, b;
      a.hi = read_tr8(DYI + dyTr, DYROW);
      a.lo = read_tr8(DYI + DYPLANE + dyTr, DYROW);
      b = read_tr(DZ1I, WPLANE32, trOwn);
      gW3 = mfma3w(a, b, gW3);
    }
    f32x4 dz[2];
#pragma unroll
    for (int nt = 0; nt < 2; ++nt) {
      Frag4 b;
      b.hi = *reinterpret_cast<const half4*>(DYI + 16 * nt * DYROW + dyRd);
      b.lo = *reinterpret_cast<const half4*>(DYI + DYPLANE + 16 * nt * DYROW + dyRd);
      dz[nt] = mfma3k16(W3d, b, f32x4{0, 0, 0, 0});
#pragma unroll
      for (int r = 0; r < 4; ++r) {
        dz[nt][r] = ((relu2 >> (4 * nt + r)) & 1u) ? dz[nt][r] * W3_UNSCALE : 0.0f;
        ab2[r] += dz[nt][r];
      }
      const Frag4 f = split4(dz[nt]);
      *reinterpret_cast<half4*>(DZ2I + 4096 * nt + wrA) = f.hi;
      *reinterpret_cast<half4*>(DZ2I + 4096 * nt + WPLANE32 + wrA) = f.lo;
    }
    WSTAMP(9);
    {
      const Frag b = read_tr(DZ2I, WPLANE32, trOwn);
      Frag an[GWD];
#pragma unroll
      for (int t = 0; t < GWD; ++t) an[t] = read_tr(H1I, WPLANE32, tr_addr(t));
#pragma unroll
      for (int t = 0; t < 8; ++t) {
        const Frag a = an[t % GWD];
        if (t + GWD < 8) an[t % GWD] = read_tr(H1I, WPLANE32, tr_addr(t + GWD));
        gW2[t] = mfma3w(a, b, gW2[t]);
        __builtin_amdgcn_sched_barrier(0);
      }
    }
    WSTAMP(10);
    __syncthreads();
    WSTAMP(11);

    {
      acc[0] = f32x4{0, 0, 0, 0};
      acc[1] = f32x4{0, 0, 0, 0};
      Frag an = read_row(W2I + 4096 * v, W2PLANE, rdA[0]);
      Frag bn[2];
#pragma unroll
      for (int nt = 0; nt < 2; ++nt) bn[nt] = read_row(DZ2I + 4096 * nt, WPLANE32, rdA[0]);
// ... 6 lines not shown
#pragma unroll
          for (int nt = 0; nt < 2; ++nt) bn[nt] = read_row(DZ2I + 4096 * nt, WPLANE32, rdA[s + 1]);
        }
#pragma unroll
        for (int nt = 0; nt < 2; ++nt) acc[nt] = mfma3w(a, b[nt], acc[nt]);
        __builtin_amdgcn_sched_barrier(0);
      }
#pragma unroll
      for (int nt = 0; nt < 2; ++nt) {
#pragma unroll
        for (int r = 0; r < 4; ++r) acc[nt][r] = ((relu1 >> (4 * nt + r)) & 1u) ? (ACTOR ? acc[nt][r] : acc[nt][r] * WU) : 0.0f;
        const Frag4 f = split4(acc[nt]);
        *reinterpret_cast<half4*>(DZ1I + 4096 * nt + wrA) = f.hi;
        *reinterpret_cast<half4*>(DZ1I + 4096 * nt + WPLANE32 + wrA) = f.lo;
      }
    }
    WSTAMP(12);
    {
      const Frag b = read_tr(DZ1I, WPLANE32, trOwn);
      constexpr int D1 = GWD < KT1 ? GWD : KT1;
      if (x_lo) {
        Frag an[D1];
#pragma unroll
        for (int t = 0; t < D1; ++t) an[t] = read_tr(XSI, WPLANE32, tr_addr(t));
#pragma unroll
        for (int t = 0; t < KT1; ++t) {
          const Frag a = an[t % D1];
          if (t + D1 < KT1) an[t % D1] = read_tr(XSI, WPLANE32, tr_addr(t + D1));
          gW1[t] = mfma3w(a, b, gW1[t]);
          __builtin_amdgcn_sched_barrier(0);
        }
      } else {
        half8 an[D1];
#pragma unroll
        for (int t = 0; t < D1; ++t) an[t] = read_tr8(XSI + tr_addr(t), WROW);
#pragma unroll
        for (int t = 0; t < KT1; ++t) {
          const half8 a = an[t % D1];
          if (t + D1 < KT1) an[t % D1] = read_tr8(XSI + tr_addr(t + D1), WROW);
          gW1[t] = mfma2w_alo0(a, b, gW1[t]);
          __builtin_amdgcn_sched_barrier(0);
        }
      }
    }
    WSTAMP(13);
  }
#ifdef MAVA_STAMPS
  if (tk.stamps != nullptr && blockIdx.x == 0 && l == 0) {
    for (int k = 0; k < 16; ++k) tk.stamps[v * 16 + k] = ws_acc[k];
  }
#endif

  __syncthreads();
  float* slab = tk.slab + (long)blockIdx.x * tk.slab_stride;
  const int oB2 = mlp_off_b2(din), oB3 = mlp_off_b3(din, no);
  const int Pn = mlp_param_count(din, no);
#pragma unroll
  for (int t = 0; t < KT1; ++t)
#pragma unroll
    for (int r = 0; r < 4; ++r) {
      const int k = 16 * t + 4 * kg + r;
      if (k <= din) slab[k * MLP_H + 16 * v + i] = gW1[t][r] * invR;
    }
#pragma unroll
  for (int t = 0; t < 8; ++t)
#pragma unroll
    for (int r = 0; r < 4; ++r) slab[oW2 + (16 * t + 4 * kg + r) * MLP_H + 16 * v + i] = gW2[t][r] * invR;
#pragma unroll
  for (int r = 0; r < 4; ++r) {
    float x = ab2[r];
#pragma unroll
    for (int m = 1; m < 16; m <<= 1) x += __shfl_xor(x, m, 64);
    if (i == 0) slab[oB2 + 16 * v + 4 * kg + r] = x * invR;
    const int o = 4 * kg + r;
    if (o < no) slab[oW3 + (16 * v + i) * no + o] = gW3[r] * invR;
  }
  float* red = reinterpret_cast<float*>(lds + L.h1);
  if constexpr (DO_LOSS) {
    float x = ab3;
#pragma unroll
    for (int m = NO; m < 64; m <<= 1) x += __shfl_xor(x, m, 64);
    if (l < NO) red[v * NO + l] = x;
    for (int o = 32; o > 0; o >>= 1) {
      loss_a += __shfl_down(loss_a, o, 64);
      loss_b += __shfl_down(loss_b, o, 64);
    }
    if (l == 0) { red[8 * NO + 2 * v] = loss_a; red[8 * NO + 2 * v + 1] = loss_b; }
  }
  __syncthreads();
  constexpr int LW = LOSS_THREADS / 64;
  if (tid < no) {
    float x = 0.0f;
#pragma unroll
    for (int u = 0; u < LW; ++u) x += red[u * NO + tid];
    slab[oB3 + tid] = x * invR;
  }
  if (tid == 0) {
    float a = 0.0f, b = 0.0f;
#pragma unroll
    for (int u = 0; u < LW; ++u) { a += red[8 * NO + 2 * u]; b += red[8 * NO + 2 * u + 1]; }
    slab[Pn] = a;
    slab[Pn + 1] = b;
  }
}

constexpr int w8_w2r(int no, int s1, int xv) {
#ifdef MAVA_W8_W2R
  return MAVA_W8_W2R;
#else
  return (no == 8) ? ((s1 <= 2) ? 2 : ((s1 == 3 && xv == 2) ? 2 : 0)) : ((s1 <= 2) ? 2 : 0);
#endif
}
template <int NO, int S1, int XV, int W2R, bool ACTOR>
__global__ __launch_bounds__(512, 2) void ppo_train_w8_kernel(TrainTask tk, W8Layout L) {
  extern __shared__ __attribute__((aligned(16))) u8 lds[];
  if constexpr (NO == 8) {
    if (threadIdx.x < 256) {
      w8_body<NO, S1, XV, W2R, ACTOR, 1>(tk, L, lds);
    } else {
      w8_body<NO, S1, XV, W2R, ACTOR, 2>(tk, L, lds);
    }
  } else {
    w8_body<NO, S1, XV, W2R, ACTOR, 0>(tk, L, lds);
  }
}

template <int NO, int S1, int XV, bool ACTOR>
int launch_w8(const TrainTask& tk, int n_slab, hipStream_t s) {
  const W8Layout L = make_w8_layout();
  static bool attr_set = false;
  if (!attr_set) {
    MAVA_HIP_CHECK(hipFuncSetAttribute((const void*)ppo_train_w8_kernel<NO, S1, XV, w8_w2r(NO, S1, XV), ACTOR>, hipFuncAttributeMaxDynamicSharedMemorySize,
                                       L.end));
    attr_set = true;
  }
  g_train_last_instance = train_instance_id(3, ACTOR, false, false, NO, S1, XV);
  hipLaunchKernelGGL((ppo_train_w8_kernel<NO, S1, XV, w8_w2r(NO, S1, XV), ACTOR>), dim3(n_slab), dim3(512), L.end, s, tk, L);
  MAVA_LAUNCH_CHECK();
  return MAVA_OK;
}

template <int NO, int S1, bool ACTOR>
int dispatch_w8_xv(const TrainTask& tk, int n_slab, hipStream_t s) {
  if (tk.din % 2 == 0 && ((uintptr_t)tk.x) % 8 == 0) return launch_w8<NO, S1, 2, ACTOR>(tk, n_slab, s);
  if constexpr (S1 == 4) return 1;
  else return launch_w8<NO, S1, 1, ACTOR>(tk, n_slab, s);
}

template <int NO, bool ACTOR>
int dispatch_w8(const TrainTask& tk, int n_slab, hipStream_t s) {
  const int s1 = (tk.din + 1 + 31) / 32;
  switch (s1) {
#ifndef MAVA_FAST_BUILD
    case 1: return dispatch_w8_xv<NO, 1, ACTOR>(tk, n_slab, s);
    case 2: return dispatch_w8_xv<NO, 2, ACTOR>(tk, n_slab, s);
    case 4: return dispatch_w8_xv<NO, 4, ACTOR>(tk, n_slab, s);
#endif
    case 3: return dispatch_w8_xv<NO, 3, ACTOR>(tk, n_slab, s);
    default: return 1;
  }
}

}

int mava_train_w8_launch(const TrainTask& tk, int n_slab, bool actor, hipStream_t s) {
  if (tk.action_f != nullptr || tk.din + 1 > 128) return 1;
  if (!actor) {
    if (tk.agg > 1 || tk.no != 1) return 1;
    return dispatch_w8<8, false>(tk, n_slab, s);
  }
  if (tk.no <= 8) return dispatch_w8<8, true>(tk, n_slab, s);
#ifndef MAVA_FAST_BUILD
  if (tk.no <= 16) return dispatch_w8<16, true>(tk, n_slab, s);
#endif
  return 1;
}
```

### mava_amd/csrc/rollout_h2.hip

```cpp
#include "h2_core.h"

#ifdef MAVA_STAMPS
#define RSTAMP_DECL unsigned long long rs_prev = __builtin_readcyclecounter(), rs_acc[8] = {0, 0, 0, 0, 0, 0, 0, 0};
#define RSTAMP(i)                                                   \
  do {                                                              \
    __builtin_amdgcn_sched_barrier(0);                              \
    const unsigned long long rs_now = __builtin_readcyclecounter(); \
    rs_acc[i] += rs_now - rs_prev;                                  \
    rs_prev = rs_now;                                               \
    __builtin_amdgcn_sched_barrier(0);                              \
  } while (0)
static __device__ unsigned long long g_rollout_stamps[16];
#else
#define RSTAMP_DECL
#define RSTAMP(i)
#endif

namespace {
using namespace h2;
typedef _Float16 half2v __attribute__((ext_vector_type(2)));

constexpr uint32_t ENV_STREAM = 0x454E5653u;
constexpr uint32_t POLICY_STREAM = 0x504f4c49u;

struct RolloutArgs {
  const float* pa;
  const float* pc;
  int E, A, O, no, T, time_limit;
  uint32_t pseed_lo, pseed_hi, eseed_lo, eseed_hi;
  uint32_t t0;
  uint32_t row_offset;
  uint32_t env_offset;
  int reward_mode;
  int32_t* step_count;
  float* run_return; int32_t* run_length; float* ep_return; int32_t* ep_length;
  float* agents_view;
  float* global_state;
  uint8_t* action_mask;
  int32_t* obs_step_count;
  int32_t* action; float* value; float* reward; float* log_prob; uint8_t* done;
  float* last_val;
  float* info_return; int32_t* info_length; uint8_t* info_terminal;
  float* adv; float* tgt;
  float gamma, lam;
  float* last_reward; uint8_t* last_done; int32_t* step_counter;
  _Float16* state16; uint32_t* state16_valid;
};

#define MAVA_AS4 __attribute__((address_space(4)))
__device__ __forceinline__ const MAVA_AS4 RolloutArgs& args_here() {
  const MAVA_AS4 RolloutArgs* p = (const MAVA_AS4 RolloutArgs*)__builtin_amdgcn_kernarg_segment_ptr();
  asm volatile("" : "+s"(p));
  return *p;
}

__device__ __forceinline__ uint32_t div_small(uint32_t x, uint32_t m) { return __umul24(x, m) >> 16; }

struct RolloutLds {
  int xa, xa_row, xa_plane, xc, xc_row, xc_plane, h1, wl, ypa, ypc, act, mask, small, gum, xlf, end;
};
constexpr int W1_REG_STEPS = 12;

template <int NO, int S1A, int S1C, bool SHARED>
constexpr RolloutLds make_rollout_lds() {
  constexpr int KTA = (S1A + 1) / 2, KTC = (S1C + 1) / 2;
  RolloutLds L{};
  L.xa = 0;
  L.xa_row = 2 * 32 * KTA + 16;
  L.xa_plane = 32 * L.xa_row;
  L.xc = L.xa + 2 * 2 * L.xa_plane;
  L.xc_row = 2 * 32 * KTC + 16;
  L.xc_plane = ((S1C > W1_REG_STEPS) ? 16 : 32) * L.xc_row;
  L.h1 = L.xc + (SHARED ? 2 * L.xc_plane : 0);
  L.wl = L.h1 + (SHARED ? 3 : 4) * IMG_BYTES;
  L.ypa = L.wl + ((S1C > W1_REG_STEPS) ? (S1C - W1_REG_STEPS) * 4 * 64 * 32 : 0);
  L.ypc = L.ypa + 2 * 4 * 32 * (NO + 1) * 4;
  L.act = L.ypc + 2 * 4 * 32 * 4;
  L.mask = L.act + 64 * 4;
  L.small = L.mask + 64 * 32;
  L.gum = L.small + (128 + 32 + 128 + 4 + 128) * 4;
  L.gum = (L.gum + 15) & ~15;
  L.xlf = L.gum + 64 * NO * 4;
  L.end = L.xlf + 16;
  L.end = (L.end + 15) & ~15;
  return L;
}

template <int NO, int S1A, int S1C, bool SHARED, int ROLE>
__device__ __forceinline__ void rollout_body(const RolloutArgs& a, u8* lds) {
  constexpr bool ACT_ROLE = ROLE == 0;
  constexpr RolloutLds L = make_rollout_lds<NO, S1A, S1C, SHARED>();
  const int t512 = threadIdx.x;
  const int tid = t512 & 255, lane = tid & 63, w = tid >> 6, h = lane >> 5, r = lane & 31;
  const int A = a.A, O = a.O, no = a.no, W = A + O, E = a.E;
  const int EB = 64 / A;
  const int e0 = blockIdx.x * EB;
  const int din_a = W, din_c = SHARED ? A * O : W;
  constexpr int NTC = SHARED ? 1 : 2;
  float* const B2a = reinterpret_cast<float*>(lds + L.small);
// ... 31 lines not shown
  Frag W1r[S1REG], W2r[8], W3h[2];
  {
    float c1 = 0.0f, c2 = 0.0f;
#pragma unroll
    for (int s = 0; s < S1R; ++s) {
      float v[8];
#pragma unroll
      for (int e = 0; e < 8; ++e) {
        const int k = 16 * s + 8 * h + e;
        v[e] = (k <= din_r) ? PR[k * MLP_H + 32 * w + r] : 0.0f;
      }
      const Frag f = split8_carry(v, c1);
      if (s < S1REG) {
        W1r[s] = f;
      } else {
        WL[512 * (s - S1REG)] = __builtin_bit_cast(uint4, f.hi);
        WL[512 * (s - S1REG) + 1] = __builtin_bit_cast(uint4, f.lo);
      }
      __builtin_amdgcn_sched_barrier(0);
    }
#pragma unroll
    for (int s = 0; s < 8; ++s) {
      float v[8];
#pragma unroll
      for (int e = 0; e < 8; ++e) v[e] = PR[oW2r + (16 * s + 8 * h + e) * MLP_H + 32 * w + r];
      W2r[s] = split8_carry(v, c2);
      __builtin_amdgcn_sched_barrier(0);
    }
#pragma unroll
    for (int s = 0; s < (ACT_ROLE ? 2 : 0); ++s) {
      float v[8];
#pragma unroll
      for (int e = 0; e < 8; ++e) {
        const int f = 32 * w + 16 * s + 8 * (e >> 2) + 4 * h + (e & 3);
        v[e] = (r < no) ? a.pa[oW3a + f * no + r] * W3_SCALE : 0.0f;
      }
      W3h[s] = split8(v);
    }
  }
  {
    const long slot0_av = 0;
    uint32_t lo_any = 0, lo_gs = 0;
    for (int i = t512; i < 64 * W; i += 512) {
      const int row = i / W, c = i - row * W;
      const int e = e0 + row / A;
      const float v = (e < E) ? a.agents_view[slot0_av + ((long)e0 * A + row) * W + c] : 0.0f;
      _Float16 x0, x1;
      split1(v, x0, x1);
      u8* p = lds + L.xa + (row >> 5) * 2 * xa_plane + (row & 31) * xa_row + 2 * c;
      *reinterpret_cast<_Float16*>(p) = x0;
      *reinterpret_cast<_Float16*>(p + xa_plane) = x1;
      lo_any |= (uint32_t)__builtin_bit_cast(uint16_t, x1) & 0x7FFFu;
    }
    if (t512 < 64) {
      u8* p = lds + L.xa + (t512 >> 5) * 2 * xa_plane + (t512 & 31) * xa_row + 2 * din_a;
      *reinterpret_cast<_Float16*>(p) = (_Float16)1.0f;
    }
    if (SHARED) {
      const int gw = A * O;
      for (int i = t512; i < EB * gw; i += 512) {
        const int le = i / gw, c = i - le * gw;
        const float v = (e0 + le < E) ? a.global_state[(long)(e0 + le) * gw + c] : 0.0f;
        _Float16 x0, x1;
        split1(v, x0, x1);
        u8* p = lds + L.xc + le * xc_row + 2 * c;
        *reinterpret_cast<_Float16*>(p) = x0;
        *reinterpret_cast<_Float16*>(p + xc_plane) = x1;
        lo_gs |= (uint32_t)__builtin_bit_cast(uint16_t, x1) & 0x7FFFu;
      }
      lo_any |= lo_gs;
      if (lo_gs != 0) XLF[1] = 1u;
      if (t512 < XC_ROWS) *reinterpret_cast<_Float16*>(lds + L.xc + t512 * xc_row + 2 * din_c) = (_Float16)1.0f;
    }
    for (int i = t512; i < 64 * no; i += 512) {
      const int row = i / no, o = i - row * no;
      MASK[row * 32 + o] = (e0 + row / A < E) ? a.action_mask[((long)e0 * A + row) * no + o] : 1;
    }
    if (lo_any != 0) *XLF = 1u;
  }
  __syncthreads();

  const int lgA = __builtin_ctz((unsigned)A);
  const int bk_le = tid >> lgA, bk_ag = tid & (A - 1);
  const bool bk_on = !ACT_ROLE && tid < 64 && (e0 + bk_le) < E;
  const long bk_k = (long)e0 * A + tid;
  int sc_reg = bk_on ? a.step_count[bk_k] : 0;
  float rr_reg = 0.0f, er_reg = 0.0f;
  int rl_reg = 0, el_reg = 0;
  if (bk_on && bk_ag == 0) {
    rr_reg = a.run_return[e0 + bk_le]; rl_reg = a.run_length[e0 + bk_le];
    er_reg = a.ep_return[e0 + bk_le]; el_reg = a.ep_length[e0 + bk_le];
  }

  const bool x_lo = __builtin_amdgcn_readfirstlane((int)*XLF) != 0;
  if (SHARED && ACT_ROLE && tid == 0 && a.state16_valid != nullptr) {
    uint32_t seen = 0;
    if (XLF[1] != 0) seen = atomicOr(a.state16_valid, 0x80000000u);
    asm volatile("" : "+v"(seen) : : "memory");
    const uint32_t old = atomicAdd(a.state16_valid, 2u);
    if (((old >> 1) & 0x3FFFFFFFu) == gridDim.x - 1u) *a.state16_valid = (old & 0x80000000u) ? 0u : 1u;
  }
  const int rowB = r * IMG_ROW + 16 * h;
  const long EA = (long)E * A;
  const uint32_t nch = (O - 2 + 15) / 16 > 0 ? (O - 2 + 15) / 16 : 1;

  constexpr int NT = ACT_ROLE ? 2 : NTC;
  RSTAMP_DECL
  auto forward = [&](bool active, bool noise, uint32_t noise_step) __attribute__((always_inline)) {
    f32x16 z[NT];
#pragma unroll
    for (int i = 0; i < NT; ++i)
#pragma unroll
      for (int q = 0; q < 16; ++q) z[i][q] = 0.0f;
    if (active) {
      auto x_frag = [&](int s, int t) {
        return (!ACT_ROLE && SHARED) ? read_row_frag(lds + L.xc, xc_plane, (r & (XC_ROWS - 1)) * xc_row + 16 * h + 32 * s)
                                     : read_row_frag(lds + L.xa + t * 2 * xa_plane, xa_plane, r * xa_row + 16 * h + 32 * s);
      };
      auto w_frag = [&](int s) {
        Frag wf;
        wf.hi = __builtin_bit_cast(half8, WL[512 * (s - S1REG)]);
        wf.lo = __builtin_bit_cast(half8, WL[512 * (s - S1REG) + 1]);
        return wf;
      };
      auto x_hi = [&](int s, int t) -> half8 {
        return (!ACT_ROLE && SHARED)
                   ? *reinterpret_cast<const half8*>(lds + L.xc + (r & (XC_ROWS - 1)) * xc_row + 16 * h + 32 * s)
                   : *reinterpret_cast<const half8*>(lds + L.xa + t * 2 * xa_plane + r * xa_row + 16 * h + 32 * s);
      };
      if (x_lo) {
      Frag bn[NT], wn;
#pragma unroll
      for (int t = 0; t < NT; ++t) bn[t] = x_frag(0, t);
      if (S1REG == 0) wn = w_frag(0);
#pragma unroll
      for (int s = 0; s < S1R; ++s) {
        Frag b[NT];
#pragma unroll
        for (int t = 0; t < NT; ++t) b[t] = bn[t];
        const Frag wf = (s < S1REG) ? W1r[s < S1REG ? s : 0] : wn;
        if (s + 1 < S1R) {
#pragma unroll
          for (int t = 0; t < NT; ++t) bn[t] = x_frag(s + 1, t);
          if (s + 1 >= S1REG) wn = w_frag(s + 1);
        }
#pragma unroll
        for (int t = 0; t < NT; ++t) z[t] = mfma3(wf, b[t], z[t]);
        __builtin_amdgcn_sched_barrier(0);
      }
      } else {
      half8 bn[NT];
      Frag wn;
#pragma unroll
// ... 117 lines not shown
          part += __shfl_xor(part, 32, 64);
          if (h == 0) YPC[(t * 4 + w) * 32 + r] = part;
        }
      }
    }
    RSTAMP(2);
    __syncthreads();
    RSTAMP(3);
  };
  auto value_of = [&](int crow) -> float {
    const float* yp = YPC + (crow >> 5) * 4 * 32 + (crow & 31);
    return (((yp[0] + yp[32]) + yp[64]) + yp[96]) + B3c[0];
  };

  const int rows_ok = min(64, (E - e0) * A), envs_ok = min(EB, E - e0);
  const int AO = A * O;
  const uint32_t no_m = 65536u / (uint32_t)no + 1u, nch_m = 65536u / nch + 1u;
  const int tid_w = tid, wo_q = (W >> 1) > 0 ? (W >> 1) : 1, gs_q = (AO >> 2) > 0 ? (AO >> 2) : 1;
  const int wo_dr = 256 / wo_q, gs_dr = 256 / gs_q;
  const uint32_t wo_m = 65536u / (uint32_t)wo_q + 1u, gs_m = 65536u / (uint32_t)gs_q + 1u;
  auto write_gs = [&](long slot, bool f32_too) {
    const auto& a = args_here();
    int tid = tid_w;
    asm volatile("" : "+v"(tid));
    if (SHARED && a.global_state != nullptr) {
      float* dst = a.global_state + (slot * E + e0) * (long)AO;
      if ((AO & 3) == 0) {
        const bool h16 = a.state16 != nullptr;
        uint4* const dst16 = h16 ? reinterpret_cast<uint4*>(a.state16 + (slot * E + e0) * (long)AO) : nullptr;
        const int Q = AO >> 2, d_r = gs_dr, d_f = 256 - d_r * Q;
        int le = (int)div_small((uint32_t)tid, gs_m), k = tid - le * Q;
        for (int j = tid; j < EB * Q; j += 256) {
          if (le < envs_ok) {
            if (f32_too) {
              const half4 v = *reinterpret_cast<const half4*>(lds + L.xc + le * xc_row + 8 * k);
              reinterpret_cast<float4*>(dst)[j] = make_float4((float)v[0], (float)v[1], (float)v[2], (float)v[3]);
            }
            if (h16 && (k & 1) == 0) dst16[j >> 1] = *reinterpret_cast<const uint4*>(lds + L.xc + le * xc_row + 8 * k);
          }
          le += d_r; k += d_f;
          if (k >= Q) { k -= Q; ++le; }
        }
      } else if (f32_too) {
        const int d_r = 256 / AO, d_f = 256 - d_r * AO;
        int le = tid / AO, k = tid - le * AO;
        for (int j = tid; j < EB * AO; j += 256) {
          if (le < envs_ok) dst[j] = (float)*reinterpret_cast<const _Float16*>(lds + L.xc + le * xc_row + 2 * k);
          le += d_r; k += d_f;
          if (k >= AO) { k -= AO; ++le; }
        }
      }
    }
  };
  auto write_out = [&](long slot, bool part_gs) {
    const auto& a = args_here();
    int tid = tid_w;
    asm volatile("" : "+v"(tid));
    if (!part_gs) {
      float* dst = a.agents_view + (slot * EA + (long)e0 * A) * W;
      if ((W & 1) == 0) {
        const int W2 = W >> 1, d_r = wo_dr, d_f = 256 - d_r * W2;
        int row = (int)div_small((uint32_t)tid, wo_m), f = tid - row * W2;
        for (int j = tid; j < 64 * W2; j += 256) {
          if (row < rows_ok) {
            const u8* xa = lds + L.xa + (row >> 5) * 2 * xa_plane + (row & 31) * xa_row;
            const half2v v = *reinterpret_cast<const half2v*>(xa + 4 * f);
            reinterpret_cast<float2*>(dst)[j] = make_float2((float)v[0], (float)v[1]);
          }
          row += d_r; f += d_f;
          if (f >= W2) { f -= W2; ++row; }
        }
      } else {
        const int d_r = 256 / W, d_f = 256 - d_r * W;
        int row = tid / W, f = tid - row * W;
        for (int j = tid; j < 64 * W; j += 256) {
          if (row < rows_ok) {
            const u8* xa = lds + L.xa + (row >> 5) * 2 * xa_plane + (row & 31) * xa_row;
            dst[j] = (float)*reinterpret_cast<const _Float16*>(xa + 2 * f);
          }
          row += d_r; f += d_f;
          if (f >= W) { f -= W; ++row; }
        }
      }
    }
    if (part_gs) write_gs(slot, true);
    if (!part_gs) {
      uint8_t* dst = a.action_mask + (slot * EA + (long)e0 * A) * no;
      for (int j = tid; j < rows_ok * no; j += 256) {
        const int row = (int)div_small((uint32_t)j, no_m), o = j - row * no;
        dst[j] = MASK[row * 32 + o];
      }
    }
  };

  const int T_steps = a.T;
  const uint32_t t0 = a.t0;
  if (SHARED && ACT_ROLE && a.state16 != nullptr) write_gs(0L, false);
  for (int t = 0; t < T_steps; ++t) {
    const uint32_t step = t0 + (uint32_t)t;
    forward(true, true, step);
    const auto& a = args_here();
    if (ACT_ROLE) {
      constexpr int RPP = 256 / NO;
#pragma unroll
      for (int pass = 0; pass < 64 / RPP; ++pass) {
        const int row = pass * RPP + tid / NO, o = tid & (NO - 1);
        const float* yp = YPA + (((row >> 5) * 4) * 32 + (row & 31)) * (NO + 1) + o;
        const float y = (((yp[0] + yp[32 * (NO + 1)]) + yp[2 * 32 * (NO + 1)]) + yp[3 * 32 * (NO + 1)]) + B3a[o];
        const bool legal = (o < no) && (MASK[row * 32 + o] != 0);
        const float z = legal ? y : -FLT_MAX;
        auto fmax_op = [](float p, float q) { return fmaxf(p, q); };
        auto add_op = [](float p, float q) { return p + q; };
        const float mx = group_allreduce<NO>(z, fmax_op);
        const float se = group_allreduce<NO>(expf(z - mx), add_op);
        const float logp = (mx == -FLT_MAX) ? ((o < no) ? -logf((float)no) : -FLT_MAX) : z - (mx + logf(se));
        float sc = (o < no) ? (z + GUM[row * NO + o]) : -FLT_MAX;
        if (!(sc > -FLT_MAX)) sc = -FLT_MAX;
        int best = o;
#pragma unroll
        for (int m = 1; m < NO; m <<= 1) {
          const float so = __shfl_xor(sc, m, 64);
          const int bo = __shfl_xor(best, m, 64);
          const bool take = (so > sc) || (so == sc && bo < best);
          sc = take ? so : sc;
          best = take ? bo : best;
        }
        const float lp = group_allreduce<NO>((o == best) ? logp : 0.0f, add_op);
        const int e = e0 + (row >> lgA);
        if (o == 0) {
          ACT[row] = best;
          if (e < E) {
            const long k = (long)t * EA + (long)e0 * A + row;
            a.action[k] = best;
            a.log_prob[k] = lp;
          }
        }
      }
    } else {
      if (tid < 64 && (e0 + (tid >> lgA)) < E) {
        a.value[(long)t * EA + (long)e0 * A + tid] = value_of(SHARED ? (tid >> lgA) : tid);
      }
      if (t > 0) write_out((long)t, false);
    }
    if (ACT_ROLE && t > 0) write_out((long)t, true);
    RSTAMP(4);
    __syncthreads();
    RSTAMP(5);
    {
      const auto& a = args_here();
      const uint32_t tn = step + 1;
// ... 173 lines not shown
  if (!ACT_ROLE && blockIdx.x == 0 && tid == 0 && a.step_counter != nullptr) *a.step_counter += a.T;
  }
}

template <int NO, int S1A, int S1C, bool SHARED>
__global__ __launch_bounds__(512, 2) void rollout_h2_kernel(RolloutArgs a) {
  extern __shared__ __attribute__((aligned(16))) u8 lds[];
  if (threadIdx.x < 256) {
    rollout_body<NO, S1A, S1C, SHARED, 0>(a, lds);
  } else {
    rollout_body<NO, S1A, S1C, SHARED, 1>(a, lds);
  }
}

int g_rollout_last_instance = 0;

template <int NO, int S1A, int S1C, bool SHARED>
int launch_rollout(const RolloutArgs& a, hipStream_t s) {
  g_rollout_last_instance = NO * 100000 + S1A * 1000 + S1C * 10 + (SHARED ? 1 : 0);
  constexpr RolloutLds L = make_rollout_lds<NO, S1A, S1C, SHARED>();
  MAVA_ARG_CHECK(L.end <= 163840, 8, "mava_rollout_ff_f32: %d bytes of LDS exceed the 160 KiB of a CU", L.end);
  const int lds_bytes = L.end > 83968 ? L.end : 83968;
  static bool attr_set = false;
  if (!attr_set) {
    MAVA_HIP_CHECK(hipFuncSetAttribute((const void*)rollout_h2_kernel<NO, S1A, S1C, SHARED>,
                                       hipFuncAttributeMaxDynamicSharedMemorySize, lds_bytes));
    attr_set = true;
  }
  const int EB = 64 / a.A;
  hipLaunchKernelGGL((rollout_h2_kernel<NO, S1A, S1C, SHARED>), dim3(mava_cdiv(a.E, EB)), dim3(512), lds_bytes, s, a);
  MAVA_LAUNCH_CHECK();
  return MAVA_OK;
}

}

#ifdef MAVA_STAMPS
extern "C" int mava_debug_get_rollout_stamps(unsigned long long* out16) {
  return -(int)hipMemcpyFromSymbol(out16, HIP_SYMBOL(g_rollout_stamps), 16 * sizeof(unsigned long long));
}
#endif

extern "C" int mava_debug_rollout_last_instance(void) { return g_rollout_last_instance; }

static int rollout_ff_impl(const float* actor_params, int n_actions, const float* critic_params, int critic_shared,
                           int E, int A, int O, int T, int time_limit, uint64_t policy_seed, uint64_t env_seed,
                           uint32_t t0, uint32_t row_offset, uint32_t env_offset, int reward_mode,
                           int32_t* step_count, float* run_return, int32_t* run_length, float* ep_return,
                           int32_t* ep_length, float* agents_view, float* global_state, uint8_t* action_mask,
                           int32_t* obs_step_count, int32_t* action, float* value, float* reward, float* log_prob,
                           uint8_t* done, float* last_val, float* info_return, int32_t* info_length,
                           uint8_t* info_terminal, float* adv, float* tgt, float gamma, float gae_lambda,
                           float* last_reward, uint8_t* last_done, int32_t* step_counter, uint16_t* state16,
                           uint32_t* state16_valid, hipStream_t s) {
  MAVA_ARG_CHECK(E >= 1 && A >= 1 && O >= 2 && T >= 1 && n_actions >= 1 && time_limit >= 1, 0,
                 "mava_rollout_ff_f32: bad shape E=%d A=%d O=%d T=%d nA=%d", E, A, O, T, n_actions);
  MAVA_ARG_CHECK(actor_params && critic_params && step_count && run_return && run_length && ep_return && ep_length &&
                     agents_view && action_mask && obs_step_count && action && value && reward && log_prob && done &&
                     last_val && info_return && info_length && info_terminal && (!critic_shared || global_state),
                 1, "mava_rollout_ff_f32: null pointer argument");
  if (64 % A != 0 || n_actions > 8) return 1;
  if (critic_shared && A < 2) return 1;
  const int s1a = (A + O + 1 + 15) / 16, s1c = critic_shared ? (A * O + 1 + 15) / 16 : s1a;
  RolloutArgs a = {};
  a.pa = actor_params; a.pc = critic_params; a.E = E; a.A = A; a.O = O; a.no = n_actions; a.T = T; a.time_limit = time_limit;
  a.pseed_lo = (uint32_t)policy_seed; a.pseed_hi = (uint32_t)(policy_seed >> 32);
  a.eseed_lo = (uint32_t)env_seed; a.eseed_hi = (uint32_t)(env_seed >> 32);
  a.t0 = t0; a.row_offset = row_offset; a.env_offset = env_offset; a.reward_mode = reward_mode;
  a.step_count = step_count; a.run_return = run_return; a.run_length = run_length; a.ep_return = ep_return;
  a.ep_length = ep_length; a.agents_view = agents_view; a.global_state = critic_shared ? global_state : nullptr;
  a.action_mask = action_mask; a.obs_step_count = obs_step_count; a.action = action; a.value = value; a.reward = reward;
  a.log_prob = log_prob; a.done = done; a.last_val = last_val; a.info_return = info_return; a.info_length = info_length;
  a.info_terminal = info_terminal;
  MAVA_ARG_CHECK((adv == nullptr) == (tgt == nullptr), 1, "mava_rollout_ff_f32: adv and tgt go together");
  a.adv = adv; a.tgt = tgt; a.gamma = gamma; a.lam = gae_lambda;
  a.last_reward = last_reward; a.last_done = last_done; a.step_counter = step_counter;
  MAVA_ARG_CHECK((state16 == nullptr) == (state16_valid == nullptr), 1, "mava_rollout_ff_x16_f32: state16 and state16_valid go together");
  MAVA_ARG_CHECK(state16 == nullptr || (critic_shared && (A * O) % 8 == 0 && (uintptr_t)state16 % 16 == 0), 2,
                 "mava_rollout_ff_x16_f32: state16 needs the shared critic, A*O %% 8 == 0 (A*O=%d) and 16-byte alignment", A * O);
  a.state16 = reinterpret_cast<_Float16*>(state16); a.state16_valid = state16_valid;
  if (critic_shared) {
    if (s1a == 5 && s1c == 17 && A >= 4) return launch_rollout<8, 5, 17, true>(a, s);
#ifndef MAVA_FAST_BUILD
    if (s1a <= 2 && s1c <= 2) return launch_rollout<8, 2, 2, true>(a, s);
    if (s1a <= 2 && s1c <= 4) return launch_rollout<8, 2, 4, true>(a, s);
    if (s1a <= 5 && s1c <= 9) return launch_rollout<8, 5, 9, true>(a, s);
#endif
    return 1;
  }
  if (s1a == 5) return launch_rollout<8, 5, 5, false>(a, s);
#ifndef MAVA_FAST_BUILD
  if (s1a <= 2) return launch_rollout<8, 2, 2, false>(a, s);
#endif
  return 1;
}

extern "C" int mava_rollout_ff_f32(const float* actor_params, int n_actions, const float* critic_params, int critic_shared,
                                   int E, int A, int O, int T, int time_limit, uint64_t policy_seed, uint64_t env_seed,
                                   uint32_t t0, uint32_t row_offset, uint32_t env_offset, int reward_mode,
                                   int32_t* step_count, float* run_return, int32_t* run_length, float* ep_return,
                                   int32_t* ep_length, float* agents_view, float* global_state, uint8_t* action_mask,
                                   int32_t* obs_step_count, int32_t* action, float* value, float* reward, float* log_prob,
                                   uint8_t* done, float* last_val, float* info_return, int32_t* info_length,
                                   uint8_t* info_terminal, float* adv, float* tgt, float gamma, float gae_lambda,
                                   hipStream_t s) {
  return rollout_ff_impl(actor_params, n_actions, critic_params, critic_shared, E, A, O, T, time_limit, policy_seed, env_seed,
                         t0, row_offset, env_offset, reward_mode, step_count, run_return, run_length, ep_return, ep_length,
                         agents_view, global_state, action_mask, obs_step_count, action, value, reward, log_prob, done,
                         last_val, info_return, info_length, info_terminal, adv, tgt, gamma, gae_lambda, nullptr, nullptr,
                         nullptr, nullptr, nullptr, s);
}

extern "C" int mava_rollout_ff_tail_f32(const float* actor_params, int n_actions, const float* critic_params,
                                        int critic_shared, int E, int A, int O, int T, int time_limit,
                                        uint64_t policy_seed, uint64_t env_seed, uint32_t t0, uint32_t row_offset,
                                        uint32_t env_offset, int reward_mode, int32_t* step_count, float* run_return,
                                        int32_t* run_length, float* ep_return, int32_t* ep_length, float* agents_view,
                                        float* global_state, uint8_t* action_mask, int32_t* obs_step_count,
                                        int32_t* action, float* value, float* reward, float* log_prob, uint8_t* done,
                                        float* last_val, float* info_return, int32_t* info_length, uint8_t* info_terminal,
                                        float* adv, float* tgt, float gamma, float gae_lambda, float* last_reward,
                                        uint8_t* last_done, int32_t* step_counter, hipStream_t s) {
  MAVA_ARG_CHECK(last_reward && last_done, 1, "mava_rollout_ff_tail_f32: null pointer argument");
  return rollout_ff_impl(actor_params, n_actions, critic_params, critic_shared, E, A, O, T, time_limit, policy_seed, env_seed,
                         t0, row_offset, env_offset, reward_mode, step_count, run_return, run_length, ep_return, ep_length,
                         agents_view, global_state, action_mask, obs_step_count, action, value, reward, log_prob, done,
                         last_val, info_return, info_length, info_terminal, adv, tgt, gamma, gae_lambda, last_reward,
                         last_done, step_counter, nullptr, nullptr, s);
}

extern "C" int mava_rollout_ff_x16_f32(const float* actor_params, int n_actions, const float* critic_params,
                                       int critic_shared, int E, int A, int O, int T, int time_limit,
                                       uint64_t policy_seed, uint64_t env_seed, uint32_t t0, uint32_t row_offset,
                                       uint32_t env_offset, int reward_mode, int32_t* step_count, float* run_return,
                                       int32_t* run_length, float* ep_return, int32_t* ep_length, float* agents_view,
                                       float* global_state, uint8_t* action_mask, int32_t* obs_step_count,
                                       int32_t* action, float* value, float* reward, float* log_prob, uint8_t* done,
                                       float* last_val, float* info_return, int32_t* info_length, uint8_t* info_terminal,
                                       float* adv, float* tgt, float gamma, float gae_lambda, float* last_reward,
                                       uint8_t* last_done, int32_t* step_counter, uint16_t* state16,
                                       uint32_t* state16_valid, hipStream_t s) {
  MAVA_ARG_CHECK((last_reward == nullptr) == (last_done == nullptr) && (last_reward != nullptr || step_counter == nullptr), 1,
                 "mava_rollout_ff_x16_f32: last_reward, last_done (and step_counter) go together");
  return rollout_ff_impl(actor_params, n_actions, critic_params, critic_shared, E, A, O, T, time_limit, policy_seed, env_seed,
                         t0, row_offset, env_offset, reward_mode, step_count, run_return, run_length, ep_return, ep_length,
                         agents_view, global_state, action_mask, obs_step_count, action, value, reward, log_prob, done,
                         last_val, info_return, info_length, info_terminal, adv, tgt, gamma, gae_lambda, last_reward,
                         last_done, step_counter, state16, state16_valid, s);
}

namespace {
struct CarryArgs {
  uint8_t* base[4];
  long slot_bytes[4];
  int T;
};
template <typename V>
__device__ __forceinline__ void carry_copy(uint8_t* dst, const uint8_t* src, long bytes) {
  const long nv = bytes / (long)sizeof(V), stride = (long)gridDim.x * blockDim.x;
  const long i0 = (long)blockIdx.x * blockDim.x + threadIdx.x;
  for (long i = i0; i < nv; i += stride) reinterpret_cast<V*>(dst)[i] = reinterpret_cast<const V*>(src)[i];
  for (long i = nv * (long)sizeof(V) + i0; i < bytes; i += stride) dst[i] = src[i];
}
__global__ __launch_bounds__(256) void rollout_carry_kernel(CarryArgs c) {
  uint8_t* const dst = c.base[blockIdx.y];
  const long bytes = c.slot_bytes[blockIdx.y];
  if (dst == nullptr || bytes <= 0) return;
  const uint8_t* const src = dst + (long)c.T * bytes;
  const uintptr_t al = reinterpret_cast<uintptr_t>(dst) | reinterpret_cast<uintptr_t>(src);
  if ((al & 15) == 0) carry_copy<uint4>(dst, src, bytes);
  else if ((al & 3) == 0) carry_copy<uint32_t>(dst, src, bytes);
  else carry_copy<uint8_t>(dst, src, bytes);
}
}

extern "C" int mava_rollout_carry(int T, int E, int A, int obs_dim, long gs_dim, int n_actions, float* agents_view,
                                  float* global_state, uint8_t* action_mask, int32_t* step_count, hipStream_t s) {
  MAVA_ARG_CHECK(T >= 1 && E >= 1 && A >= 1 && obs_dim >= 1 && gs_dim >= 0 && n_actions >= 1, 0,
                 "mava_rollout_carry: bad shape T=%d E=%d A=%d obs_dim=%d gs_dim=%ld nA=%d", T, E, A, obs_dim, gs_dim, n_actions);
  MAVA_ARG_CHECK(agents_view && action_mask && step_count && (gs_dim == 0 || global_state), 1,
                 "mava_rollout_carry: null pointer argument");
  CarryArgs c = {};
  c.T = T;
  c.base[0] = reinterpret_cast<uint8_t*>(agents_view); c.slot_bytes[0] = (long)E * A * obs_dim * 4;
  c.base[1] = gs_dim ? reinterpret_cast<uint8_t*>(global_state) : nullptr; c.slot_bytes[1] = (long)E * gs_dim * 4;
  c.base[2] = action_mask; c.slot_bytes[2] = (long)E * A * n_actions;
  c.base[3] = reinterpret_cast<uint8_t*>(step_count); c.slot_bytes[3] = (long)E * A * 4;
  long most = 0;
  for (int i = 0; i < 4; ++i) most = c.slot_bytes[i] > most ? c.slot_bytes[i] : most;
  const long blocks = mava_cdiv(most, 256L * 16 * 4);
  hipLaunchKernelGGL(rollout_carry_kernel, dim3((unsigned)(blocks < 1 ? 1 : blocks > 2048 ? 2048 : blocks), 4), dim3(256), 0, s, c);
  MAVA_LAUNCH_CHECK();
  return MAVA_OK;
}
```

### mava_amd/learner.py

```python
from __future__ import annotations

import math
import contextlib
import os
from typing import Any, Dict, List, Optional, Tuple

import torch

from . import ops, parallel
from .guards import check_f16_range
from .learner_common import bind_learn, matmul_ctx
from .networks import FeedForwardActor, FeedForwardValueNet, MLPTorso, make_action_head
from .types import (AdamState, ExperimentOutput, LearnerState, Observation, ObservationGlobalState, OptStates, Params,
                    TimeStep)

NUM_CU = 256


def _dist_info() -> Tuple[int, int]:
    return parallel.rank_world()


class _Replica:

# ... 77 lines not shown
            state_shape = getattr(env0, "state_shape", None) if centralised_critic else obs_shape
            self.actor_network = gn.GenericActor(gn.torso_from_config(net.actor_network.pre_torso), action_head, self.Oa, obs_shape)
            self.critic_network = gn.GenericCritic(gn.torso_from_config(net.critic_network.pre_torso), centralised_critic, self.Oc,
                                                   state_shape)
        else:
            a_torso = MLPTorso(**{k: v for k, v in net.actor_network.pre_torso.items() if k != "_target_"})
            c_torso = MLPTorso(**{k: v for k, v in net.critic_network.pre_torso.items() if k != "_target_"})
            self.actor_network = FeedForwardActor(a_torso, action_head, self.Oa)
            self.critic_network = FeedForwardValueNet(c_torso, centralised_critic, self.Oc)
        self.Pa, self.Pc = self.actor_network.num_params, self.critic_network.num_params
        self.P = self.Pa + self.Pc

        d = self.device
        self.p = torch.zeros(self.P, device=d)
        self.m = torch.zeros(self.P, device=d)
        self.v = torch.zeros(self.P, device=d)
        self.count = torch.zeros(2, dtype=torch.int32, device=d)
        self.g = torch.zeros(self.P + 4, device=d)
        self.seg_off = [0, self.Pa, self.P]
        self.seg_lr = [float(s.actor_lr), float(s.critic_lr)]

        self.Rb = self.T * self.E // self.M
        ntiles = (self.Rb * self.A + 31) // 32
        self.rccl_cus = int(s.get("rccl_cus", None) if s.get("rccl_cus", None) is not None
                            else os.environ.get("MAVA_RCCL_CUS", "8" if self.world > 1 else "0"))
        self.n_slab = max(1, min(NUM_CU - max(0, min(self.rccl_cus, NUM_CU - 1)), ntiles))
        self.slab_a = torch.zeros((self.n_slab, self.Pa + 2), device=d)
        self.slab_c = torch.zeros((self.n_slab, self.Pc + 2), device=d)
        self.stats = torch.zeros((ops.lib().mava_adv_stats_blocks(), 2), dtype=torch.float64, device=d)
        self.train_metrics = torch.zeros((self.n_upd, self.K, self.M, 4), device=d)
        self.perm_count = 0
        self.t_global = 0
        self.ent_step = 0
        self.step_dev = torch.zeros(1, dtype=torch.int32, device=d)
        mode = os.environ.get("MAVA_GRAPH_ROLLOUT", "1")
        self.graph_rollout = (mode == "force" or (mode != "0" and self.world == 1)) and not self.generic
        self._graphs: Dict[int, Any] = {}
        self._graph_seen: set = set()
        self.seed = int(s.seed)
        self.timers: Optional[Dict[str, list]] = None
        self.matmul_mode, self.ctx = matmul_ctx(s, critic_aggregation=os.environ.get("MAVA_CRITIC_AGGREGATION", "1") != "0")
        self.ctx.set(self.ctx.TRAIN_VARIANT, int(os.environ.get("MAVA_TRAIN_VARIANT", "0")))
        for net_ in (self.actor_network, self.critic_network):
            net_.ctx = self.ctx
        self.fused_rollout = (self.matmul_mode == "f16x2" and not self.continuous and not self.generic
                              and os.environ.get("MAVA_FUSED_ROLLOUT", "1") != "0"
                              and bool(getattr(env0, "supports_fused_rollout", False))
                              and int(getattr(env0, "synth_state_dim", 0)) == 0
                              and (not centralised_critic or (env0.gs_tiles == 1 and env0.global_state_shared)))
        self.x16 = (self.fused_rollout and centralised_critic and self.Oc % 8 == 0 and os.environ.get("MAVA_X16", "1") != "0")
        for rep in self.reps:
            rep.state16 = torch.zeros((self.T + 1, self.E, 1, self.Oc), dtype=torch.float16, device=d) if self.x16 else None
            rep.state16_valid = torch.zeros((1,), dtype=torch.int32, device=d) if self.x16 else None
        self._learn_calls = 0
        self.fused_tail = (self.world == 1 and not self.generic and os.environ.get("MAVA_FUSED_TAIL", "1") != "0")
        self._finish_ws = ops.ppo_finish_workspace(self.Pa, self.Pc, d) if self.fused_tail else None
        self._finish_ws_mr = (ops.ppo_finish_workspace(self.Pa, self.Pc, d)
                              if (not self.fused_tail and not self.generic and os.environ.get("MAVA_FUSED_TAIL", "1") != "0") else None)
        if self.fused_tail and self.U > 1:
            self.slab_a = torch.zeros((self.U * self.n_slab, self.Pa + 2), device=d)
            self.slab_c = torch.zeros((self.U * self.n_slab, self.Pc + 2), device=d)

    def _timed(self, name: str, fn, *args, **kwargs):
        if self.timers is None:
            return fn(*args, **kwargs)
        a, b = torch.cuda.Event(enable_timing=True), torch.cuda.Event(enable_timing=True)
        a.record()
        out = fn(*args, **kwargs)
        b.record()
        self.timers.setdefault(name, []).append((a, b))
        return out

    def init_params(self, actor_seed: int, critic_seed: int) -> None:
        self.p[: self.Pa].copy_(self.actor_network.init_flat(actor_seed))
        self.p[self.Pa :].copy_(self.critic_network.init_flat(critic_seed))
        self.m.zero_()
        self.v.zero_()
        self.count.zero_()

    def reset_envs(self) -> None:
        for rep in self.reps:
            rep.env.step_into(rep.state, 0, rep.obs_slot(0), is_reset=True)
        self.t_global = 0
        self.ent_step = 0
        self.step_dev.zero_()
        self.perm_count = 0

    def _params_tree(self) -> Params:
        lead = (1, self.U)
        return Params(self.actor_network.tree(self.p[: self.Pa], lead), self.critic_network.tree(self.p[self.Pa :], lead))

    def _opt_tree(self) -> OptStates:
        lead = (1, self.U)
        out = []
        for i, (net, sl) in enumerate(((self.actor_network, slice(0, self.Pa)), (self.critic_network, slice(self.Pa, self.P)))):
            out.append(AdamState(self.count[i].expand(1, self.U), net.tree(self.m[sl], lead), net.tree(self.v[sl], lead)))
        return OptStates(*out)

    def _timestep(self, slot: int) -> TimeStep:
        def stack(f):
            return torch.stack([f(r) for r in self.reps], 0).unsqueeze(0)

        av = stack(lambda r: r.agents_view[slot])
        mask = stack(lambda r: r.action_mask[slot]).bool()
        sc = stack(lambda r: r.step_count[slot])
        if self.centralised:
# ... 42 lines not shown
            self._rollout_body()
            self._bootstrap_and_gae()
        else:
            key = self.seed
            graph = self._graphs.get(key)
            if graph is None and key in self._graph_seen:
                graph = torch.cuda.CUDAGraph()
                with torch.cuda.graph(graph, capture_error_mode="thread_local"):
                    self._rollout_body()
                    self._bootstrap_and_gae()
                self._graphs[key] = graph
            if graph is None:
                self._graph_seen.add(key)
                self._rollout_body()
                self._bootstrap_and_gae()
            else:
                graph.replay()
        for rep in self.reps:
            rep.info_return[n].copy_(rep.cur_return)
            rep.info_length[n].copy_(rep.cur_length)
            rep.info_terminal[n].copy_(rep.cur_terminal)
        self.t_global += self.T

    def _rollout_fused(self, n: int) -> bool:
        s = self.config.system
        pa, pc = self.p[: self.Pa], self.p[self.Pa :]
        EA = self.E * self.A
        main = torch.cuda.current_stream() if self.device.type == "cuda" else None
        side = self.U > 1 and self.timers is None and main is not None and os.environ.get("MAVA_ROLLOUT_STREAMS", "1") != "0"
        if side and not hasattr(self, "_roll_streams"):
            from .streams import overlapping_stream

            self._roll_streams = [overlapping_stream(self.device) for _ in range(self.U - 1)]
            if any(st is None for st in self._roll_streams):
                self._roll_streams = []
        side = side and len(self._roll_streams) == self.U - 1
        if side:
            for st in self._roll_streams:
                st.wait_stream(main)
        for u, rep in enumerate(self.reps):
            env = rep.env
            with (torch.cuda.stream(self._roll_streams[u - 1]) if (side and u > 0) else contextlib.nullcontext()):
              ok = self._timed(
                "rollout_fused", ops.rollout_ff, pa, pc, n_actions=self.nA, critic_shared=self.centralised, E=self.E,
                A=self.A, O=env.raw_obs_dim, T=self.T, time_limit=env.time_limit, policy_seed=self.seed,
                env_seed=env.seed, t0=self.t_global, row_offset=(self.rank * self.U + u) * EA, env_offset=env.env_offset,
                reward_mode=1 if env.reward_mode == "match" else 0, env_state=rep.state, agents_view=rep.agents_view,
                global_state=rep.global_state, action_mask=rep.action_mask, obs_step_count=rep.step_count,
                action=rep.action, value=rep.value, reward=rep.reward, log_prob=rep.log_prob, done=rep.done,
                last_val=rep.last_val, info_return=rep.info_return[n], info_length=rep.info_length[n],
                info_terminal=rep.info_terminal[n], adv=rep.adv, tgt=rep.tgt, gamma=float(s.gamma),
                gae_lambda=float(s.gae_lambda), last_reward=rep.last_reward, last_done=rep.last_done,
                step_counter=self.step_dev if u == 0 else None,
                state16=rep.state16, state16_valid=rep.state16_valid)
              if not ok:
                assert u == 0
                self.fused_rollout = self.x16 = False
                for r in self.reps:
                    r.state16 = r.state16_valid = None
                return False
        if side:
            for st in self._roll_streams:
                main.wait_stream(st)
        return True

    def _rollout_body(self) -> None:
        pa, pc = self.p[: self.Pa], self.p[self.Pa :]
        EA = self.E * self.A
        for t in range(self.T):
            step = t
            for u, rep in enumerate(self.reps):
                av = rep.agents_view[t].view(EA, self.Oa)
                if self.centralised:
                    cx = rep.global_state[t].view(-1, self.Oc)
                else:
                    cx = av
                shared = self.critic_share == self.A and self.A > 1
                common = dict(critic_share=1 if shared else self.critic_share, critic_rows=self.E if shared else EA,
                              value_broadcast=self.A if shared else 1, seed=self.seed, step=step,
                              step_base=self.step_dev, row_offset=(self.rank * self.U + u) * EA, ctx=self.ctx)
                if self.generic:
                    self._timed("policy_step", self._generic_act, u, rep, t, step)
                elif self.continuous:
                    self._timed("policy_step", ops.policy_step_continuous, pa, pc, av, cx, action_dim=self.nA, min_scale=self.min_scale,
                                out=(rep.action[t].view(EA, self.nA), rep.log_prob[t].view(EA), rep.value[t].view(EA)),
                                **common)
                else:
                    self._timed("policy_step", ops.policy_step, pa, pc, av, rep.action_mask[t].view(EA, self.nA), cx,
                                n_actions=self.nA,
                                out=(rep.action[t].view(EA), rep.log_prob[t].view(EA), rep.value[t].view(EA)), **common)
                last = t == self.T - 1
                self._timed("env_step", rep.env.step_into, rep.state, step + 1, rep.obs_slot(t + 1), rep.reward[t], rep.done[t],
                            rep.cur_return[t], rep.cur_length[t], rep.cur_terminal[t], t_base=self.step_dev,
                            action=rep.action[t] if self._env_reads_action else None)
                if last:
                    rep.last_reward.copy_(rep.reward[t])
                    rep.last_done.copy_(rep.done[t])
        self.step_dev.add_(self.T)

    def _bootstrap_and_gae(self) -> None:
        s = self.config.system
        pc = self.p[self.Pa :]
        EA = self.E * self.A
        for rep in self.reps:
            cx = rep.global_state[self.T].view(-1, self.Oc) if self.centralised else rep.agents_view[self.T].view(EA, self.Oa)
            if self.generic:
                v = self.critic_network.net.forward(pc, self._gws_roll[1], cx.view(1, self.E, -1, self.Oc), self.critic_share, None, EA,
                                                    self.E, self.A)[0]
                rep.last_val.view(EA).copy_(v)
            else:
                ops.mlp_forward(pc, self.Oc, 1, cx, rows=EA, x_share=self.critic_share, out=rep.last_val.view(EA, 1), ctx=self.ctx)
            self._timed("gae", ops.gae, rep.reward.view(self.T, EA), rep.value.view(self.T, EA), rep.done.view(self.T, EA),
                        rep.last_val.view(EA), float(s.gamma), float(s.gae_lambda),
                        out=(rep.adv.view(self.T, EA), rep.tgt.view(self.T, EA)), ctx=self.ctx)

    def _minibatch(self, n: int, k: int, mb: int, perm: Optional[torch.Tensor]) -> None:
        s = self.config.system
        T, E, A = self.T, self.E, self.A
        TEA = T * E * A
        pa, pc = self.p[: self.Pa], self.p[self.Pa :]
        idx = None if perm is None else perm[mb * self.Rb : (mb + 1) * self.Rb]
        base = mb * self.Rb
        if self.generic:
            return self._minibatch_generic(n, k, mb, idx if idx is not None else torch.arange(base, base + self.Rb, dtype=torch.int32,
                                                                                             device=self.device))
        ns = self.n_slab
        per_rep = self.fused_tail and self.U > 1
        for u, rep in enumerate(self.reps):
            slab_a = self.slab_a[u * ns : (u + 1) * ns] if per_rep else self.slab_a
            av = rep.agents_view[:T].view(TEA, self.Oa)
            if getattr(self, "_stats_batched", False) and perm is self._perm_bufs[k]:
                stats = self._stats_all[u, k * self.M + mb]
            else:
                stats = ops.adv_stats(rep.adv.view(TEA), idx, base, self.Rb, A, out=self.stats)
            if self.continuous:
                self._timed("actor_grad", ops.ppo_actor_grad_continuous, pa, av, rep.action.view(TEA, self.nA),
                            rep.log_prob.view(TEA), rep.adv.view(TEA), stats, idx, base, self.Rb, A, self.nA,
                            float(s.clip_eps), float(s.ent_coef), self.seed, self.ent_step,
                            (self.rank * self.U + u) * TEA, slab_a, min_scale=self.min_scale)
            else:
                self._timed("actor_grad", ops.ppo_actor_grad, pa, av, rep.action_mask[:T].view(TEA, self.nA),
                            rep.action.view(TEA), rep.log_prob.view(TEA), rep.adv.view(TEA), stats, idx, base,
                            self.Rb, A, self.nA, float(s.clip_eps), float(s.ent_coef), slab_a, ctx=self.ctx)
            if not self.fused_tail:
                ops.slab_reduce2(self.slab_a, self.Pa, self.g[: self.Pa], 2, self.g[self.P : self.P + 2], accumulate=u > 0)
        w_actor = parallel.allreduce_sum_async(self.g[: self.Pa])
        for u, rep in enumerate(self.reps):
            av = rep.agents_view[:T].view(TEA, self.Oa)
            cx = rep.global_state[:T].view(-1, self.Oc) if self.centralised else av
            self._timed("critic_grad", ops.ppo_critic_grad, pc, cx, self.critic_share, rep.value.view(TEA), rep.tgt.view(TEA),
                        idx, base, self.Rb, A, float(s.clip_eps), float(s.vf_coef),
                        self.slab_c[u * ns : (u + 1) * ns] if per_rep else self.slab_c, ctx=self.ctx,
                        input16=rep.state16[:T].view(-1, self.Oc) if self.x16 else None,
                        input16_valid=rep.state16_valid if self.x16 else None)
            if not self.fused_tail:
                ops.slab_reduce2(self.slab_c, self.Pc, self.g[self.Pa : self.P], 1, self.g[self.P + 2 : self.P + 3], accumulate=u > 0)
        if self.fused_tail:
            self._timed("finish", ops.ppo_finish, self.ctx, self.slab_a, self.slab_c, self.Pa, self.Pc, self.g, self.p, self.m, self.v,
                        self.count, self.seg_lr[0], self.seg_lr[1], grad_scale=1.0 / self.U, max_norm=float(s.max_grad_norm),
                        decay=bool(s.decay_learning_rates), steps_per_update=self.K * self.M,
                        num_updates=int(s.get("num_updates", 1) or 1), vf_coef=float(s.vf_coef), ent_coef=float(s.ent_coef),
                        metrics_out=self.train_metrics[n, k, mb], critic_din=self.Oc, workspace=self._finish_ws)
            self.ent_step += 1
            return
        w_rest = parallel.allreduce_sum_async(self.g[self.Pa :])
        for wk in (w_actor, w_rest):
            if wk is not None:
                wk.wait()
        if self._finish_ws_mr is not None:
            self._timed("clip_adam", ops.ppo_finish, self.ctx, None, None, self.Pa, self.Pc, self.g, self.p, self.m, self.v, self.count,
                        self.seg_lr[0], self.seg_lr[1], grad_scale=1.0 / (self.U * self.world), max_norm=float(s.max_grad_norm),
                        decay=bool(s.decay_learning_rates), steps_per_update=self.K * self.M,
                        num_updates=int(s.get("num_updates", 1) or 1), vf_coef=float(s.vf_coef), ent_coef=float(s.ent_coef),
                        metrics_out=self.train_metrics[n, k, mb], critic_din=self.Oc, workspace=self._finish_ws_mr)
            self.ent_step += 1
            return
        self._timed("clip_adam", ops.clip_adam, self.p, self.g, self.m, self.v, self.count, self.seg_off, self.seg_lr,
                      grad_scale=1.0 / (self.U * self.world), max_norm=float(s.max_grad_norm),
                      decay=bool(s.decay_learning_rates), steps_per_update=self.K * self.M,
                      num_updates=int(s.get("num_updates", 1) or 1), loss_sums=self.g[self.P :], vf_coef=float(s.vf_coef),
                      ent_coef=float(s.ent_coef), metrics_out=self.train_metrics[n, k, mb])
        self.ent_step += 1

    def _generic_setup(self) -> None:
        d = self.device
        EA, Rm = self.E * self.A, self.Rb * self.A
        a, c = self.actor_network.net, self.critic_network.net
        self._gws_roll = (a.workspace(EA, d, False), c.workspace(EA, d, False))
        self._gws = (a.workspace(Rm, d, True), c.workspace(Rm, d, True))
        self._g_scale = float(2 ** math.ceil(math.log2(Rm)))
        self._g_dscale = torch.zeros((self._gws[0].loss_partials.shape[0], max(self.nA, 1)), device=d)

    def _generic_act(self, u: int, rep, t: int, step: int) -> None:
        if not hasattr(self, "_gws_roll"):
            self._generic_setup()
        L, st = ops.lib(), ops.stream_ptr()
        pa, pc = self.p[: self.Pa], self.p[self.Pa :]
        E, A, EA = self.E, self.A, self.E * self.A
        an = self.actor_network
        outs = an.net.forward(pa, self._gws_roll[0], rep.agents_view[t : t + 1], 1, None, EA, E, A)
        seed, row_off = self.seed & (2**64 - 1), ((self.rank * self.U + u) * EA) & 0xFFFFFFFF
        gstep = (self.t_global + step) & 0xFFFFFFFF
        if self.continuous:
            ind = an.independent_std
            ops.check(L.mava_seq_sample_continuous_f32(EA, self.nA, self.min_scale, ops.ptr(outs[0]), ops.ptr(an.log_std(pa)) if ind else None,
                                                       None if ind else ops.ptr(outs[1]), seed, gstep, row_off, 0, ops.ptr(rep.action[t]),
                                                       ops.ptr(rep.log_prob[t]), st), "mava_seq_sample_continuous_f32")
# ... 126 lines not shown
```

### mava_amd/ops.py

```python
from __future__ import annotations

import ctypes as C
from typing import Optional, Sequence, Tuple

import torch

from . import _lib
from ._lib import Ctx, check, ctx_ptr, lib, ptr, stream_ptr


def _req(t: torch.Tensor, dtype: torch.dtype, name: str, shape: Optional[Tuple[int, ...]] = None) -> None:
    if not isinstance(t, torch.Tensor):
        raise TypeError(f"{name}: expected a torch.Tensor")
    if not t.is_cuda:
        raise _lib.MavaHipError(f"{name}: tensor must live on the GPU (got {t.device}); there is no CPU path")
    if t.dtype != dtype:
        raise TypeError(f"{name}: expected dtype {dtype}, got {t.dtype}")
    if not t.is_contiguous():
        raise ValueError(f"{name}: tensor must be contiguous")
    if shape is not None and tuple(t.shape) != tuple(shape):
        raise ValueError(f"{name}: expected shape {tuple(shape)}, got {tuple(t.shape)}")


def _as_u8(t: torch.Tensor) -> torch.Tensor:
# ... 310 lines not shown
                                                 ptr(old_log_prob), ptr(advantages), ptr(stats), ptr(idx), idx_base,
                                                 Rb, A, clip_eps, ent_coef, seed & 0xFFFFFFFFFFFFFFFF,
                                                 ent_step & 0xFFFFFFFF, row_offset & 0xFFFFFFFF, ptr(slab),
                                                 slab.shape[1], slab.shape[0], stream_ptr()),
        "mava_ppo_actor_grad_continuous_f32",
    )


def adv_stats_batched(advantages: torch.Tensor, idx: torch.Tensor, Rb: int, A: int, n_batch: int,
                      out: Optional[torch.Tensor] = None) -> torch.Tensor:
    _req(advantages, torch.float32, "advantages")
    _req(idx, torch.int32, "idx")
    if idx.numel() < n_batch * Rb:
        raise ValueError("idx shorter than n_batch * Rb")
    nb = lib().mava_adv_stats_blocks()
    if out is None:
        out = torch.empty((n_batch, nb, 2), dtype=torch.float64, device=advantages.device)
    _req(out, torch.float64, "out", (n_batch, nb, 2))
    check(lib().mava_adv_stats_batched_f64(ptr(advantages), ptr(idx), Rb, Rb, A, n_batch, ptr(out), stream_ptr()),
          "mava_adv_stats_batched_f64")
    return out


def adv_stats(advantages: torch.Tensor, idx: Optional[torch.Tensor], idx_base: int, Rb: int, A: int,
              out: Optional[torch.Tensor] = None) -> torch.Tensor:
    _req(advantages, torch.float32, "advantages")
    if idx is not None:
        _req(idx, torch.int32, "idx")
        if idx.numel() < Rb:
            raise ValueError("idx shorter than Rb")
    elif (idx_base + Rb) * A > advantages.numel():
        raise ValueError("minibatch exceeds the trajectory")
    nb = lib().mava_adv_stats_blocks()
    if out is None:
        out = torch.empty((nb, 2), dtype=torch.float64, device=advantages.device)
    else:
        _req(out, torch.float64, "out", (nb, 2))
    check(lib().mava_adv_stats_f64(ptr(advantages), ptr(idx), idx_base, Rb, A, ptr(out), stream_ptr()),
          "mava_adv_stats_f64")
    return out


def _check_idx(idx, idx_base, Rb, TE):
    if idx is not None:
        _req(idx, torch.int32, "idx")
        if idx.numel() < Rb:
            raise ValueError("idx shorter than Rb")
    elif idx_base < 0 or idx_base + Rb > TE:
        raise ValueError("minibatch exceeds the trajectory")


def ppo_actor_grad(params, agents_view, action_mask, action, old_log_prob, advantages, stats, idx, idx_base: int,
                   Rb: int, A: int, n_actions: int, clip_eps: float, ent_coef: float, slab: torch.Tensor,
                   ctx: Optional[Ctx] = None) -> None:
    _req(agents_view, torch.float32, "agents_view")
    rows, din = agents_view.shape
    if rows % A:
        raise ValueError("agents_view rows must be a multiple of A")
    TE = rows // A
    _req(params, torch.float32, "params")
    P = mlp_param_count(din, n_actions)
    if params.numel() != P:
        raise ValueError(f"params: expected {P} floats")
    if action_mask is not None:
        action_mask = _as_u8(action_mask)
        _req(action_mask, torch.uint8, "action_mask", (rows, n_actions))
    _req(action, torch.int32, "action")
    _req(old_log_prob, torch.float32, "old_log_prob")
    _req(advantages, torch.float32, "advantages")
    for n, t in (("action", action), ("old_log_prob", old_log_prob), ("advantages", advantages)):
        if t.numel() != rows:
            raise ValueError(f"{n}: expected {rows} elements, got {t.numel()}")
    _req(stats, torch.float64, "stats", (lib().mava_adv_stats_blocks(), 2))
    _check_idx(idx, idx_base, Rb, TE)
    if rows >= 2 ** 31:
        raise ValueError("trajectory too large: TE*A must be < 2^31 (32-bit row arithmetic in the kernel)")
    _req(slab, torch.float32, "slab")
    if slab.dim() != 2 or slab.shape[1] < P + 2:
        raise ValueError("slab must be (n_slab, >= P+2)")
    check(
        lib().mava_ppo_actor_grad_f32(ctx_ptr(ctx), ptr(params), din, n_actions, ptr(agents_view), ptr(action_mask), ptr(action),
                                      ptr(old_log_prob), ptr(advantages), ptr(stats), ptr(idx), idx_base, Rb, A,
                                      clip_eps, ent_coef, ptr(slab), slab.shape[1], slab.shape[0], stream_ptr()),
        "mava_ppo_actor_grad_f32",
    )


def ppo_critic_grad(params, critic_input, x_share: int, old_value, targets, idx, idx_base: int, Rb: int, A: int,
                    clip_eps: float, vf_coef: float, slab: torch.Tensor, ctx: Optional[Ctx] = None,
                    input16: Optional[torch.Tensor] = None, input16_valid: Optional[torch.Tensor] = None) -> None:
    _req(critic_input, torch.float32, "critic_input")
    din = critic_input.shape[1]
    if (input16 is None) != (input16_valid is None):
        raise ValueError("input16 and input16_valid go together")
    if input16 is not None:
        _req(input16, torch.float16, "input16", tuple(critic_input.shape))
        _req(input16_valid, torch.int32, "input16_valid", (1,))
    _req(params, torch.float32, "params")
    P = mlp_param_count(din, 1)
    if params.numel() != P:
        raise ValueError(f"params: expected {P} floats")
    _req(old_value, torch.float32, "old_value")
    _req(targets, torch.float32, "targets")
    rows = old_value.numel()
    if targets.numel() != rows or rows % A:
        raise ValueError("old_value/targets must hold TE*A elements")
    if (rows + x_share - 1) // x_share > critic_input.shape[0]:
        raise ValueError("critic_input has too few rows")
    _check_idx(idx, idx_base, Rb, rows // A)
    if rows >= 2 ** 31:
        raise ValueError("trajectory too large: TE*A must be < 2^31 (32-bit row arithmetic in the kernel)")
    _req(slab, torch.float32, "slab")
    if slab.dim() != 2 or slab.shape[1] < P + 2:
        raise ValueError("slab must be (n_slab, >= P+2)")
    args = (ctx_ptr(ctx), ptr(params), din, ptr(critic_input), x_share, ptr(old_value), ptr(targets), ptr(idx), idx_base, Rb, A,
            clip_eps, vf_coef, ptr(slab), slab.shape[1], slab.shape[0])
    if input16 is not None:
        check(lib().mava_ppo_critic_grad_x16_f32(*args, ptr(input16), ptr(input16_valid), stream_ptr()), "mava_ppo_critic_grad_x16_f32")
        return
    check(lib().mava_ppo_critic_grad_f32(*args, stream_ptr()), "mava_ppo_critic_grad_f32")


def slab_reduce2(slab: torch.Tensor, n_main: int, out_main: torch.Tensor, n_tail: int, out_tail: torch.Tensor,
                 accumulate: bool = False) -> None:
    _req(slab, torch.float32, "slab")
    _req(out_main, torch.float32, "out_main")
    _req(out_tail, torch.float32, "out_tail")
    if slab.dim() != 2 or slab.shape[1] < n_main + n_tail or out_main.numel() < n_main or out_tail.numel() < n_tail:
        raise ValueError("slab_reduce2: inconsistent sizes")
    check(
        lib().mava_slab_reduce2_f32(ptr(slab), slab.shape[0], slab.shape[1], n_main, ptr(out_main), n_tail, ptr(out_tail),
                                    int(accumulate), stream_ptr()),
        "mava_slab_reduce2_f32",
    )


def rollout_ff(actor_params, critic_params, *, n_actions: int, critic_shared: bool, E: int, A: int, O: int, T: int,
               time_limit: int, policy_seed: int, env_seed: int, t0: int, row_offset: int, env_offset: int,
               reward_mode: int, env_state, agents_view, global_state, action_mask, obs_step_count, action, value,
               reward, log_prob, done, last_val, info_return, info_length, info_terminal, adv=None, tgt=None,
               gamma: float = 0.99, gae_lambda: float = 0.95, last_reward=None, last_done=None, step_counter=None,
               state16=None, state16_valid=None) -> bool:
    W = A + O
    _req(actor_params, torch.float32, "actor_params")
    _req(critic_params, torch.float32, "critic_params")
    if actor_params.numel() != mlp_param_count(W, n_actions):
        raise ValueError("actor_params: wrong size")
    if critic_params.numel() != mlp_param_count(A * O if critic_shared else W, 1):
        raise ValueError("critic_params: wrong size")
    _req(agents_view, torch.float32, "agents_view", (T + 1, E, A, W))
    if critic_shared:
        _req(global_state, torch.float32, "global_state", (T + 1, E, 1, A * O))
    _req(action_mask, torch.uint8, "action_mask", (T + 1, E, A, n_actions))
    _req(obs_step_count, torch.int32, "obs_step_count", (T + 1, E, A))
    _req(action, torch.int32, "action", (T, E, A))
    for name, t, dt in (("value", value, torch.float32), ("reward", reward, torch.float32),
                        ("log_prob", log_prob, torch.float32), ("done", done, torch.uint8)):
        _req(t, dt, name, (T, E, A))
    _req(last_val, torch.float32, "last_val", (E, A))
    if adv is not None or tgt is not None:
        _req(adv, torch.float32, "adv", (T, E, A))
        _req(tgt, torch.float32, "tgt", (T, E, A))
    _req(info_return, torch.float32, "info_return", (T, E))
    _req(info_length, torch.int32, "info_length", (T, E))
    _req(info_terminal, torch.uint8, "info_terminal", (T, E))
    _req(env_state.step_count, torch.int32, "step_count", (E, A))
    for name, t, dt in (("run_return", env_state.run_return, torch.float32), ("run_length", env_state.run_length, torch.int32),
                        ("ep_return", env_state.ep_return, torch.float32), ("ep_length", env_state.ep_length, torch.int32)):
        _req(t, dt, name, (E,))
    args = (
        ptr(actor_params), n_actions, ptr(critic_params), int(critic_shared), E, A, O, T, time_limit,
        policy_seed & 0xFFFFFFFFFFFFFFFF, env_seed & 0xFFFFFFFFFFFFFFFF, t0 & 0xFFFFFFFF, row_offset & 0xFFFFFFFF,
        env_offset & 0xFFFFFFFF, reward_mode, ptr(env_state.step_count), ptr(env_state.run_return),
        ptr(env_state.run_length), ptr(env_state.ep_return), ptr(env_state.ep_length), ptr(agents_view),
        ptr(global_state) if critic_shared else None, ptr(action_mask), ptr(obs_step_count), ptr(action), ptr(value),
        ptr(reward), ptr(log_prob), ptr(done), ptr(last_val), ptr(info_return), ptr(info_length), ptr(info_terminal),
        ptr(adv), ptr(tgt), gamma, gae_lambda)
    if (state16 is None) != (state16_valid is None):
        raise ValueError("state16 and state16_valid go together")
    if state16 is not None:
        if not critic_shared or (A * O) % 8:
            raise ValueError("state16 needs the shared critic and A * O % 8 == 0")
        _req(state16, torch.float16, "state16", (T + 1, E, 1, A * O))
        _req(state16_valid, torch.int32, "state16_valid", (1,))
        name = "mava_rollout_ff_x16_f32"
        if last_reward is not None:
            _req(last_reward, torch.float32, "last_reward", (E, A))
            _req(last_done, torch.uint8, "last_done", (E, A))
        if step_counter is not None:
            _req(step_counter, torch.int32, "step_counter", (1,))
        rc = lib().mava_rollout_ff_x16_f32(*args, ptr(last_reward), ptr(last_done), ptr(step_counter), ptr(state16),
                                           ptr(state16_valid), stream_ptr())
    elif last_reward is None and last_done is None and step_counter is None:
        name = "mava_rollout_ff_f32"
        rc = lib().mava_rollout_ff_f32(*args, stream_ptr())
    else:
        name = "mava_rollout_ff_tail_f32"
        _req(last_reward, torch.float32, "last_reward", (E, A))
        _req(last_done, torch.uint8, "last_done", (E, A))
        if step_counter is not None:
            _req(step_counter, torch.int32, "step_counter", (1,))
        rc = lib().mava_rollout_ff_tail_f32(*args, ptr(last_reward), ptr(last_done), ptr(step_counter), stream_ptr())
    if rc == 1:
        return False
    check(rc, name)
    return True
```

Measured before the change: 83.63 million env-steps/s.

## Emit padded f16 agent-view records in rollout and feed them to actor/critic grads

The rollout gains a records16 variant that writes an f16 copy of agents_view, padded to a multiple of 8 columns, next to the f32 view. The actor gradient kernel, and the critic when it is decentralised, can then read these prebuilt f16 inputs through new input16/ld parameters instead of splitting f32 operands on every epoch. The aim is to cut the input conversion and memory traffic in the f16x2 MFMA training path. In exchange the rollout writes an extra buffer and the API surface grows, and the kernels fall back to the old path when the validity flag or alignment checks fail.

```diff
diff --git a/include/mava_hip.h b/include/mava_hip.h
--- a/include/mava_hip.h
+++ b/include/mava_hip.h
@@ -24,7 +24,8 @@
   MAVA_CTX_W8_LAUNCHES = 6,
   MAVA_CTX_W1_SPLIT_FRESH = 7,
   MAVA_CTX_EXACT_TILES = 8,
-  MAVA_CTX_X16_LAUNCHES = 9
+  MAVA_CTX_X16_LAUNCHES = 9,
+  MAVA_CTX_X16_W8_LAUNCHES = 10
 };
 int mava_ctx_create(mava_ctx** out);
 int mava_ctx_destroy(mava_ctx* ctx);
@@ -110,7 +111,13 @@
                                  const float* old_value, const float* targets, const int32_t* idx,
                                  long idx_base, int Rb, int A, float clip_eps, float vf_coef,
                                  float* slab, long slab_stride, int n_slab, const uint16_t* input16,
-                                 const uint32_t* input16_valid, mava_stream_t s);
+                                 const uint32_t* input16_valid, int input16_ld, mava_stream_t s);
+
+int mava_ppo_actor_grad_x16_f32(mava_ctx* ctx, const float* params, int din, int n_actions, const float* agents_view,
+                                const uint8_t* action_mask, const int32_t* action, const float* old_log_prob,
+                                const float* advantages, const double* adv_stats, const int32_t* idx, long idx_base, int Rb,
+                                int A, float clip_eps, float ent_coef, float* slab, long slab_stride, int n_slab,
+                                const uint16_t* input16, const uint32_t* input16_valid, int input16_ld, mava_stream_t s);
 
 
 int mava_synth_rware_step(int E, int A, int O, int n_actions, int gs_tiles, int state_dim, int time_limit,
@@ -248,6 +255,16 @@
                             uint8_t* info_terminal, float* adv, float* tgt, float gamma, float gae_lambda,
                             float* last_reward, uint8_t* last_done, int32_t* step_counter, uint16_t* state16,
                             uint32_t* state16_valid, mava_stream_t s);
+int mava_rollout_ff_records16_f32(const float* actor_params, int n_actions, const float* critic_params, int critic_shared,
+                                  int E, int A, int O, int T, int time_limit, uint64_t policy_seed, uint64_t env_seed,
+                                  uint32_t t0, uint32_t row_offset, uint32_t env_offset, int reward_mode,
+                                  int32_t* step_count, float* run_return, int32_t* run_length, float* ep_return,
+                                  int32_t* ep_length, float* agents_view, float* global_state, uint8_t* action_mask,
+                                  int32_t* obs_step_count, int32_t* action, float* value, float* reward, float* log_prob,
+                                  uint8_t* done, float* last_val, float* info_return, int32_t* info_length,
+                                  uint8_t* info_terminal, float* adv, float* tgt, float gamma, float gae_lambda,
+                                  float* last_reward, uint8_t* last_done, int32_t* step_counter, uint16_t* state16,
+                                  uint32_t* state16_valid, uint16_t* view16, uint32_t* view16_valid, mava_stream_t s);
 int mava_rollout_carry(int T, int E, int A, int obs_dim, long gs_dim, int n_actions, float* agents_view,
                        float* global_state, uint8_t* action_mask, int32_t* step_count, mava_stream_t s);
 
diff --git a/mava_amd/_lib.py b/mava_amd/_lib.py
--- a/mava_amd/_lib.py
+++ b/mava_amd/_lib.py
@@ -53,7 +53,9 @@
     "mava_ppo_actor_grad_f32": [vp, vp, i32, i32, vp, vp, vp, vp, vp, vp, vp, lng, i32, i32, f32, f32, vp, lng, i32,
                                 vp],
     "mava_ppo_critic_grad_f32": [vp, vp, i32, vp, i32, vp, vp, vp, lng, i32, i32, f32, f32, vp, lng, i32, vp],
-    "mava_ppo_critic_grad_x16_f32": [vp, vp, i32, vp, i32, vp, vp, vp, lng, i32, i32, f32, f32, vp, lng, i32, vp, vp, vp],
+    "mava_ppo_critic_grad_x16_f32": [vp, vp, i32, vp, i32, vp, vp, vp, lng, i32, i32, f32, f32, vp, lng, i32, vp, vp, i32, vp],
+    "mava_ppo_actor_grad_x16_f32": [vp, vp, i32, i32, vp, vp, vp, vp, vp, vp, vp, lng, i32, i32, f32, f32, vp, lng, i32,
+                                    vp, vp, i32, vp],
     "mava_synth_rware_step": [i32, i32, i32, i32, i32, i32, i32, u64, u32, vp, u32, i32] + [vp] * 14 + [vp, i32, vp],
     "mava_lbf_step": [i32] * 9 + [u64, u32, vp, u32, i32] + [vp] * 21 + [vp],
     "mava_lbf_step_real_next": [i32] * 9 + [u64, u32, vp, u32, i32] + [vp] * 24 + [vp],
@@ -86,6 +88,8 @@
                                 + [vp, vp, f32, f32, vp, vp, vp, vp],
     "mava_rollout_ff_x16_f32": [vp, i32, vp, i32, i32, i32, i32, i32, i32, u64, u64, u32, u32, u32, i32] + [vp] * 18
                                + [vp, vp, f32, f32, vp, vp, vp, vp, vp, vp],
+    "mava_rollout_ff_records16_f32": [vp, i32, vp, i32, i32, i32, i32, i32, i32, u64, u64, u32, u32, u32, i32] + [vp] * 18
+                                     + [vp, vp, f32, f32, vp, vp, vp, vp, vp, vp, vp, vp],
     "mava_rollout_carry": [i32, i32, i32, i32, lng, i32, vp, vp, vp, vp, vp],
     "mava_rec_dense_f32": [vp, vp, i32, vp, i32, i32, i32, i32, i32, i32, vp, i32, vp, vp, vp, i32, i32, i32, i32, i32, vp],
     "mava_rec_xty_f32": [vp, vp, i32, vp, i32, i32, i32, i32, i32, vp, i32, vp, i32, i32, i32, i32, i32, i32, f32, vp, lng, i32, vp],
@@ -157,6 +161,7 @@
     MATMUL_MODE, CRITIC_AGGREGATION, GAE_VARIANT, POLICY_VARIANT, H2_LAUNCHES, TRAIN_VARIANT, W8_LAUNCHES, W1_SPLIT_FRESH = 0, 1, 2, 3, 4, 5, 6, 7
     EXACT_TILES = 8
     X16_LAUNCHES = 9
+    X16_W8_LAUNCHES = 10
 
     def __init__(self, matmul_mode: str = "f32", critic_aggregation: bool = True):
         if matmul_mode not in ("f32", "f16x2"):
diff --git a/mava_amd/csrc/api.cpp b/mava_amd/csrc/api.cpp
--- a/mava_amd/csrc/api.cpp
+++ b/mava_amd/csrc/api.cpp
@@ -18,7 +18,7 @@
 
 extern "C" int mava_abi_version(void) { return 3; }
 
-enum { CTX_MATMUL_MODE = 0, CTX_CRITIC_AGGREGATION = 1, CTX_GAE_VARIANT = 2, CTX_POLICY_VARIANT = 3, CTX_H2_LAUNCHES = 4, CTX_TRAIN_VARIANT = 5, CTX_W8_LAUNCHES = 6, CTX_W1_SPLIT_FRESH = 7, CTX_EXACT_TILES = 8, CTX_X16_LAUNCHES = 9 };
+enum { CTX_MATMUL_MODE = 0, CTX_CRITIC_AGGREGATION = 1, CTX_GAE_VARIANT = 2, CTX_POLICY_VARIANT = 3, CTX_H2_LAUNCHES = 4, CTX_TRAIN_VARIANT = 5, CTX_W8_LAUNCHES = 6, CTX_W1_SPLIT_FRESH = 7, CTX_EXACT_TILES = 8, CTX_X16_LAUNCHES = 9, CTX_X16_W8_LAUNCHES = 10 };
 
 extern "C" int mava_ctx_create(mava_ctx** out) {
   MAVA_ARG_CHECK(out != nullptr, 0, "mava_ctx_create: null output pointer");
@@ -76,10 +76,11 @@
       }
       return MAVA_OK;
     case CTX_X16_LAUNCHES:
-      MAVA_ARG_CHECK(value == 0, 1, "mava_ctx_set: MAVA_CTX_X16_LAUNCHES can only be reset (0) by the caller");
+    case CTX_X16_W8_LAUNCHES:
+      MAVA_ARG_CHECK(value == 0, 1, "mava_ctx_set: MAVA_CTX_X16_LAUNCHES / _W8_LAUNCHES can only be reset (0) by the caller");
       if (c->exact_tiles != nullptr) {
         MAVA_HIP_CHECK(hipDeviceSynchronize());
-        MAVA_HIP_CHECK(hipMemset(c->exact_tiles + 1, 0, sizeof(unsigned long long)));
+        MAVA_HIP_CHECK(hipMemset(c->exact_tiles + (key == CTX_X16_W8_LAUNCHES ? 2 : 1), 0, sizeof(unsigned long long)));
       }
       return MAVA_OK;
     default: mava_set_error("mava_ctx_set: unknown key %d", key); return MAVA_EARG(2);
@@ -98,11 +99,12 @@
     case CTX_W8_LAUNCHES: *value = c->w8_launches; return MAVA_OK;
     case CTX_W1_SPLIT_FRESH: *value = c->w1_fresh[1]; return MAVA_OK;
     case CTX_EXACT_TILES:
-    case CTX_X16_LAUNCHES: {
+    case CTX_X16_LAUNCHES:
+    case CTX_X16_W8_LAUNCHES: {
       unsigned long long n = 0;
       if (c->exact_tiles != nullptr) {
         MAVA_HIP_CHECK(hipDeviceSynchronize());
-        MAVA_HIP_CHECK(hipMemcpy(&n, c->exact_tiles + (key == CTX_X16_LAUNCHES ? 1 : 0), sizeof(n), hipMemcpyDeviceToHost));
+        MAVA_HIP_CHECK(hipMemcpy(&n, c->exact_tiles + (key == CTX_X16_W8_LAUNCHES ? 2 : key == CTX_X16_LAUNCHES ? 1 : 0), sizeof(n), hipMemcpyDeviceToHost));
       }
       *value = (long)n;
       return MAVA_OK;
diff --git a/mava_amd/csrc/ppo_train.hip b/mava_amd/csrc/ppo_train.hip
--- a/mava_amd/csrc/ppo_train.hip
+++ b/mava_amd/csrc/ppo_train.hip
@@ -875,13 +875,11 @@
   return MAVA_OK;
 }
 
-extern "C" int mava_ppo_actor_grad_f32(mava_ctx* ctx, const float* params, int din, int n_actions,
-                                       const float* agents_view, const uint8_t* action_mask,
-                                       const int32_t* action, const float* old_log_prob,
-                                       const float* advantages, const double* adv_stats,
-                                       const int32_t* idx, long idx_base, int Rb, int A,
-                                       float clip_eps, float ent_coef, float* slab, long slab_stride,
-                                       int n_slab, hipStream_t s) {
+static int actor_grad_impl(mava_ctx* ctx, const float* params, int din, int n_actions, const float* agents_view,
+                           const uint8_t* action_mask, const int32_t* action, const float* old_log_prob,
+                           const float* advantages, const double* adv_stats, const int32_t* idx, long idx_base, int Rb, int A,
+                           float clip_eps, float ent_coef, float* slab, long slab_stride, int n_slab, const uint16_t* input16,
+                           const uint32_t* input16_valid, int input16_ld, hipStream_t s) {
   MAVA_ARG_CHECK(din >= 1 && n_actions >= 1 && n_actions <= 32, 0,
                  "mava_ppo_actor_grad_f32: din=%d n_actions=%d unsupported", din, n_actions);
   MAVA_ARG_CHECK(Rb >= 1 && A >= 1 && n_slab >= 1 && n_slab <= 1024 && (long)Rb * A < (1L << 31), 1,
@@ -897,6 +895,7 @@
   tk.stats = adv_stats; tk.clip_eps = clip_eps; tk.ent_coef = ent_coef; tk.slab = slab;
   tk.slab_stride = slab_stride;
   tk.stamps = g_stamps;
+  tk.x16 = reinterpret_cast<const _Float16*>(input16); tk.x16_valid = input16_valid; tk.x16_ld = input16_ld;
   if (mava_ctx_matmul_mode(ctx) == 1) {
     const int rc = mava_train_h2_launch(ctx, tk, n_slab, true, s);
     if (rc <= 0) return rc;
@@ -904,6 +903,31 @@
   if (n_actions <= 8) return dispatch_kt<8, true>(tk, n_slab, s);
   if (n_actions <= 16) return dispatch_kt<16, true>(tk, n_slab, s);
   return dispatch_kt<32, true>(tk, n_slab, s);
+}
+
+extern "C" int mava_ppo_actor_grad_f32(mava_ctx* ctx, const float* params, int din, int n_actions,
+                                       const float* agents_view, const uint8_t* action_mask,
+                                       const int32_t* action, const float* old_log_prob,
+                                       const float* advantages, const double* adv_stats,
+                                       const int32_t* idx, long idx_base, int Rb, int A,
+                                       float clip_eps, float ent_coef, float* slab, long slab_stride,
+                                       int n_slab, hipStream_t s) {
+  return actor_grad_impl(ctx, params, din, n_actions, agents_view, action_mask, action, old_log_prob, advantages, adv_stats, idx,
+                         idx_base, Rb, A, clip_eps, ent_coef, slab, slab_stride, n_slab, nullptr, nullptr, 0, s);
+}
+
+extern "C" int mava_ppo_actor_grad_x16_f32(mava_ctx* ctx, const float* params, int din, int n_actions,
+                                           const float* agents_view, const uint8_t* action_mask,
+                                           const int32_t* action, const float* old_log_prob,
+                                           const float* advantages, const double* adv_stats,
+                                           const int32_t* idx, long idx_base, int Rb, int A,
+                                           float clip_eps, float ent_coef, float* slab, long slab_stride,
+                                           int n_slab, const uint16_t* input16, const uint32_t* input16_valid,
+                                           int input16_ld, hipStream_t s) {
+  MAVA_ARG_CHECK((input16 == nullptr) == (input16_valid == nullptr) && input16_ld >= 0, 3,
+                 "mava_ppo_actor_grad_x16_f32: input16 and input16_valid go together, input16_ld=%d", input16_ld);
+  return actor_grad_impl(ctx, params, din, n_actions, agents_view, action_mask, action, old_log_prob, advantages, adv_stats, idx,
+                         idx_base, Rb, A, clip_eps, ent_coef, slab, slab_stride, n_slab, input16, input16_valid, input16_ld, s);
 }
 
 extern "C" int mava_ppo_actor_grad_continuous_f32(const float* params, int din, int action_dim, float min_scale,
@@ -938,7 +962,7 @@
 static int critic_grad_impl(mava_ctx* ctx, const float* params, int din, const float* critic_input, int x_share,
                             const float* old_value, const float* targets, const int32_t* idx, long idx_base, int Rb, int A,
                             float clip_eps, float vf_coef, float* slab, long slab_stride, int n_slab, const uint16_t* input16,
-                            const uint32_t* input16_valid, hipStream_t s) {
+                            const uint32_t* input16_valid, int input16_ld, hipStream_t s) {
   MAVA_ARG_CHECK(din >= 1 && x_share >= 1, 0, "mava_ppo_critic_grad_f32: din=%d x_share=%d", din, x_share);
   MAVA_ARG_CHECK(Rb >= 1 && A >= 1 && n_slab >= 1 && n_slab <= 1024 && (long)Rb * A < (1L << 31), 1,
                  "mava_ppo_critic_grad_f32: Rb=%d A=%d n_slab=%d", Rb, A, n_slab);
@@ -956,7 +980,7 @@
   tk.old_value = old_value; tk.targets = targets; tk.clip_eps = clip_eps; tk.vf_coef = vf_coef;
   tk.slab = slab; tk.slab_stride = slab_stride;
   tk.stamps = g_stamps;
-  tk.x16 = reinterpret_cast<const _Float16*>(input16); tk.x16_valid = input16_valid;
+  tk.x16 = reinterpret_cast<const _Float16*>(input16); tk.x16_valid = input16_valid; tk.x16_ld = input16_ld;
   int rc = 1;
   if (mava_ctx_matmul_mode(ctx) == 1) rc = mava_train_h2_launch(ctx, tk, n_slab, false, s);
   if (ctx != nullptr) ctx->w1_fresh[1] = 0;
@@ -970,7 +994,7 @@
                                         float clip_eps, float vf_coef, float* slab, long slab_stride,
                                         int n_slab, hipStream_t s) {
   return critic_grad_impl(ctx, params, din, critic_input, x_share, old_value, targets, idx, idx_base, Rb, A, clip_eps, vf_coef,
-                          slab, slab_stride, n_slab, nullptr, nullptr, s);
+                          slab, slab_stride, n_slab, nullptr, nullptr, 0, s);
 }
 
 extern "C" int mava_ppo_critic_grad_x16_f32(mava_ctx* ctx, const float* params, int din, const float* critic_input,
@@ -978,9 +1002,9 @@
                                             const int32_t* idx, long idx_base, int Rb, int A,
                                             float clip_eps, float vf_coef, float* slab, long slab_stride,
                                             int n_slab, const uint16_t* input16, const uint32_t* input16_valid,
-                                            hipStream_t s) {
-  MAVA_ARG_CHECK((input16 == nullptr) == (input16_valid == nullptr), 3,
-                 "mava_ppo_critic_grad_x16_f32: input16 and input16_valid go together");
+                                            int input16_ld, hipStream_t s) {
+  MAVA_ARG_CHECK((input16 == nullptr) == (input16_valid == nullptr) && input16_ld >= 0, 3,
+                 "mava_ppo_critic_grad_x16_f32: input16 and input16_valid go together, input16_ld=%d", input16_ld);
   return critic_grad_impl(ctx, params, din, critic_input, x_share, old_value, targets, idx, idx_base, Rb, A, clip_eps, vf_coef,
-                          slab, slab_stride, n_slab, input16, input16_valid, s);
-}
+                          slab, slab_stride, n_slab, input16, input16_valid, input16_ld, s);
+}
diff --git a/mava_amd/csrc/ppo_train_h2.hip b/mava_amd/csrc/ppo_train_h2.hip
--- a/mava_amd/csrc/ppo_train_h2.hip
+++ b/mava_amd/csrc/ppo_train_h2.hip
@@ -1098,6 +1098,16 @@
   }
 }
 
+int ctx_counters(mava_ctx* ctx, hipStream_t s) {
+  if (ctx->exact_tiles == nullptr) {
+    void* word = nullptr;
+    MAVA_HIP_CHECK(hipMalloc(&word, 3 * sizeof(unsigned long long)));
+    ctx->exact_tiles = static_cast<unsigned long long*>(word);
+    MAVA_HIP_CHECK(hipMemsetAsync(word, 0, 3 * sizeof(unsigned long long), s));
+  }
+  return MAVA_OK;
+}
+
 template <int NO, int S1, bool ACTOR, bool WIDE, int XV>
 int launch_h2(mava_ctx* ctx, const TrainTask& tk, int n_slab, hipStream_t s) {
   const H2Layout L = make_h2_layout<NO, S1, WIDE>(ACTOR);
@@ -1122,17 +1132,13 @@
     }
     fresh = 0;
     w1p = buf;
-    if (ctx->exact_tiles == nullptr) {
-      void* word = nullptr;
-      MAVA_HIP_CHECK(hipMalloc(&word, 2 * sizeof(unsigned long long)));
-      ctx->exact_tiles = static_cast<unsigned long long*>(word);
-      MAVA_HIP_CHECK(hipMemsetAsync(word, 0, 2 * sizeof(unsigned long long), s));
-    }
+    const int rc = ctx_counters(ctx, s);
+    if (rc != MAVA_OK) return rc;
   }
   TrainTask tkl = tk;
   tkl.exact_tiles = WIDE ? ctx->exact_tiles : nullptr;
   const bool x16_ok = WIDE && !ACTOR && XV == 4 && tk.x16 != nullptr && tk.x16_valid != nullptr && tk.din % 8 == 0 &&
-                      (uintptr_t)tk.x16 % 16 == 0 && tk.force_xlo == 0;
+                      (uintptr_t)tk.x16 % 16 == 0 && tk.force_xlo == 0 && (tk.x16_ld == 0 || tk.x16_ld == tk.din);
   if (!x16_ok) { tkl.x16 = nullptr; tkl.x16_valid = nullptr; }
   tkl.x16_launches = x16_ok ? ctx->exact_tiles + 1 : nullptr;
   g_train_last_instance = train_instance_id(2, ACTOR, false, WIDE, NO, S1, XV);
@@ -1191,6 +1197,11 @@
   TrainTask tk = tk_in;
   tk.force_xlo = (ctx->train_variant & 2) != 0;
   if ((ctx->train_variant & 1) == 0) {
+    if (tk.x16 != nullptr && tk.x16_valid != nullptr) {
+      const int rcc = ctx_counters(ctx, s);
+      if (rcc != MAVA_OK) return rcc;
+      tk.x16_launches = ctx->exact_tiles + 2;
+    }
     const int rc8 = mava_train_w8_launch(tk, n_slab, actor, s);
     if (rc8 <= 0) {
       if (rc8 == 0) { ++ctx->h2_launches; ++ctx->w8_launches; }
diff --git a/mava_amd/csrc/ppo_train_task.h b/mava_amd/csrc/ppo_train_task.h
--- a/mava_amd/csrc/ppo_train_task.h
+++ b/mava_amd/csrc/ppo_train_task.h
@@ -31,6 +31,7 @@
   const _Float16* x16;
   const uint32_t* x16_valid;
   unsigned long long* x16_launches;
+  int x16_ld;
 };
 
 struct mava_ctx;
diff --git a/mava_amd/csrc/ppo_train_w8.hip b/mava_amd/csrc/ppo_train_w8.hip
--- a/mava_amd/csrc/ppo_train_w8.hip
+++ b/mava_amd/csrc/ppo_train_w8.hip
@@ -86,9 +86,10 @@
   return L;
 }
 
-template <int NO, int S1, int XV, int W2R, bool ACTOR, int ROLE>
+template <int NO, int S1, int XV, int W2R, bool ACTOR, int ROLE, bool X16 = false>
 __device__ __forceinline__ void w8_body(const TrainTask& tk, const W8Layout& L, u8* lds) {
   constexpr bool DO_LOSS = ROLE != 2, DO_STAGE = ROLE != 1;
+  static_assert(!X16 || (DO_STAGE && XV == 2), "the f16 record is read by a staging role of an XV = 2 instance");
   constexpr float WS = ACTOR ? 1.0f : W_SCALE_CRITIC, WU = 1.0f / WS;
   constexpr int KT1 = 2 * S1;
   u8* const H1I = lds + L.h1;
@@ -235,6 +236,27 @@
   };
   u8* const xs_dummy = reinterpret_cast<u8*>(misc + 8);
   const int xsw = 16 * w8_sw(srow);
+  typedef unsigned u32x4 __attribute__((ext_vector_type(4)));
+  typedef const __attribute__((address_space(1))) u32x4* x16_gptr;
+  constexpr int NPC16 = (4 * S1 + TPR - 1) / TPR;
+  const int rp16 = 8 * ((din + 8) >> 3);
+  const int nv16 = (tk.x16_ld < rp16 ? tk.x16_ld : rp16) >> 3;
+  auto stage_issue16 = [&](uint32_t fr, u32x4 (&xq)[NPC16]) {
+    const x16_gptr xrow = (x16_gptr)(tk.x16 + (long)fr * tk.x16_ld);
+#pragma unroll
+    for (int k = 0; k < NPC16; ++k) {
+      const int c = l16 + TPR * k;
+      xq[k] = xrow[(c < nv16) ? c : 0];
+    }
+  };
+  auto stage_commit16 = [&](int buf, const u32x4 (&xq)[NPC16]) {
+    u8* base = lds + L.xs + buf * WIMG + WROW * srow;
+#pragma unroll
+    for (int k = 0; k < NPC16; ++k) {
+      const int c = l16 + TPR * k;
+      *reinterpret_cast<u32x4*>((c < nv16) ? (base + ((16 * c) ^ xsw)) : xs_dummy) = xq[k];
+    }
+  };
   auto stage_commit = [&](int buf, const float (&xr)[NR]) {
     u8* base = lds + L.xs + buf * WIMG + WROW * srow;
     uint32_t lo_any = 0;
@@ -281,7 +303,14 @@
 
   const long ntiles = (R + 31) / 32;
   long it = blockIdx.x;
-  float xr[NR];
+  float xr[X16 ? 1 : NR];
+  u32x4 xq[X16 ? NPC16 : 1];
+  auto issue = [&](uint32_t fr) __attribute__((always_inline)) {
+    if constexpr (X16) stage_issue16(fr, xq); else stage_issue(fr, xr);
+  };
+  auto commit = [&](int b) __attribute__((always_inline)) {
+    if constexpr (X16) stage_commit16(b, xq); else stage_commit(b, xr);
+  };
   int r_act = 0, n_act = 0;
   float r_f0 = 0.0f, r_f1 = 0.0f, n_f0 = 0.0f, n_f1 = 0.0f;
   uint32_t r_m = 1u, n_m = 1u;
@@ -291,14 +320,14 @@
   if (it < ntiles) {
     if constexpr (DO_STAGE) {
       cursor_gather(cs, ps_next, as_next);
-      stage_issue(stage_row(ps_next, as_next), xr);
+      issue(stage_row(ps_next, as_next));
     }
     if constexpr (DO_LOSS) {
       cursor_gather(cl, pl_next, al_next);
       load_row((uint32_t)pl_next * Au + al_next, r_act, r_f0, r_f1, r_m);
     }
     if constexpr (DO_STAGE) {
-      stage_commit(0, xr);
+      commit(0);
       cursor_advance(cs);
     }
     if constexpr (DO_LOSS) cursor_advance(cl);
@@ -395,7 +424,7 @@
     }
     WSTAMP(1);
     if (have_next) {
-      if constexpr (DO_STAGE) stage_issue(xrow_next, xr);
+      if constexpr (DO_STAGE) issue(xrow_next);
       if constexpr (DO_LOSS) load_row(lrow_next, n_act, n_f0, n_f1, n_m);
       if (itn + gridDim.x < ntiles) {
         if constexpr (DO_STAGE) { cursor_gather(cs, ps_next, as_next); cursor_advance(cs); }
@@ -405,7 +434,7 @@
     WSTAMP(2);
     __syncthreads();
     WSTAMP(3);
-    if constexpr (DO_STAGE) {
+    if constexpr (DO_STAGE && !X16) {
       if (tid == (ROLE == 2 ? 256 : 0)) xflag[buf ^ 1] = 0u;
     }
 
@@ -513,7 +542,7 @@
       r_act = n_act; r_f0 = n_f0; r_f1 = n_f1; r_m = n_m;
     }
     if constexpr (DO_STAGE) {
-      if (have_next) stage_commit(buf ^ 1, xr);
+      if (have_next) commit(buf ^ 1);
     }
     WSTAMP(7);
     __syncthreads();
@@ -626,6 +655,9 @@
 #endif
 
   __syncthreads();
+  if constexpr (X16) {
+    if (st == 0 && blockIdx.x == 0 && tk.x16_launches != nullptr) atomicAdd(tk.x16_launches, 1ull);
+  }
   float* slab = tk.slab + (long)blockIdx.x * tk.slab_stride;
   const int oB2 = mlp_off_b2(din), oB3 = mlp_off_b3(din, no);
   const int Pn = mlp_param_count(din, no);
@@ -688,14 +720,31 @@
 template <int NO, int S1, int XV, int W2R, bool ACTOR>
 __global__ __launch_bounds__(512, 2) void ppo_train_w8_kernel(TrainTask tk, W8Layout L) {
   extern __shared__ __attribute__((aligned(16))) u8 lds[];
+  constexpr bool X16_CAPABLE = XV == 2;
   if constexpr (NO == 8) {
     if (threadIdx.x < 256) {
       w8_body<NO, S1, XV, W2R, ACTOR, 1>(tk, L, lds);
     } else {
-      w8_body<NO, S1, XV, W2R, ACTOR, 2>(tk, L, lds);
+      bool x16 = false;
+      if constexpr (X16_CAPABLE) {
+        if (tk.x16_valid != nullptr) x16 = __builtin_amdgcn_readfirstlane((int)*tk.x16_valid) == 1;
+      }
+      if (X16_CAPABLE && x16) {
+        if constexpr (X16_CAPABLE) w8_body<NO, S1, XV, W2R, ACTOR, 2, true>(tk, L, lds);
+      } else {
+        w8_body<NO, S1, XV, W2R, ACTOR, 2>(tk, L, lds);
+      }
     }
   } else {
-    w8_body<NO, S1, XV, W2R, ACTOR, 0>(tk, L, lds);
+    bool x16 = false;
+    if constexpr (X16_CAPABLE) {
+      if (tk.x16_valid != nullptr) x16 = __builtin_amdgcn_readfirstlane((int)*tk.x16_valid) == 1;
+    }
+    if (X16_CAPABLE && x16) {
+      if constexpr (X16_CAPABLE) w8_body<NO, S1, XV, W2R, ACTOR, 0, true>(tk, L, lds);
+    } else {
+      w8_body<NO, S1, XV, W2R, ACTOR, 0>(tk, L, lds);
+    }
   }
 }
 
@@ -708,8 +757,14 @@
                                        L.end));
     attr_set = true;
   }
+  TrainTask tkl = tk;
+  const int ld16 = tk.x16_ld != 0 ? tk.x16_ld : tk.din;
+  const bool x16_ok = XV == 2 && tk.x16 != nullptr && tk.x16_valid != nullptr && ld16 % 8 == 0 && ld16 >= tk.din &&
+                      (uintptr_t)tk.x16 % 16 == 0 && tk.force_xlo == 0 && tk.xshare == 1 && tk.agg <= 1;
+  tkl.x16_ld = ld16;
+  if (!x16_ok) { tkl.x16 = nullptr; tkl.x16_valid = nullptr; tkl.x16_launches = nullptr; }
   g_train_last_instance = train_instance_id(3, ACTOR, false, false, NO, S1, XV);
-  hipLaunchKernelGGL((ppo_train_w8_kernel<NO, S1, XV, w8_w2r(NO, S1, XV), ACTOR>), dim3(n_slab), dim3(512), L.end, s, tk, L);
+  hipLaunchKernelGGL((ppo_train_w8_kernel<NO, S1, XV, w8_w2r(NO, S1, XV), ACTOR>), dim3(n_slab), dim3(512), L.end, s, tkl, L);
   MAVA_LAUNCH_CHECK();
   return MAVA_OK;
 }
diff --git a/mava_amd/csrc/rollout_h2.hip b/mava_amd/csrc/rollout_h2.hip
--- a/mava_amd/csrc/rollout_h2.hip
+++ b/mava_amd/csrc/rollout_h2.hip
@@ -45,6 +45,8 @@
   float gamma, lam;
   float* last_reward; uint8_t* last_done; int32_t* step_counter;
   _Float16* state16; uint32_t* state16_valid;
+  _Float16* view16; uint32_t* view16_valid;
+  int v16_nc; uint32_t v16_nc_m;
 };
 
 #define MAVA_AS4 __attribute__((address_space(4)))
@@ -182,6 +184,7 @@
       *reinterpret_cast<_Float16*>(p + xa_plane) = x1;
       lo_any |= (uint32_t)__builtin_bit_cast(uint16_t, x1) & 0x7FFFu;
     }
+    if (lo_any != 0) XLF[2] = 1u;
     if (t512 < 64) {
       u8* p = lds + L.xa + (t512 >> 5) * 2 * xa_plane + (t512 & 31) * xa_row + 2 * din_a;
       *reinterpret_cast<_Float16*>(p) = (_Float16)1.0f;
@@ -223,12 +226,16 @@
   }
 
   const bool x_lo = __builtin_amdgcn_readfirstlane((int)*XLF) != 0;
-  if (SHARED && ACT_ROLE && tid == 0 && a.state16_valid != nullptr) {
+  auto publish_valid = [&](uint32_t* word, bool low_term) {
     uint32_t seen = 0;
-    if (XLF[1] != 0) seen = atomicOr(a.state16_valid, 0x80000000u);
+    if (low_term) seen = atomicOr(word, 0x80000000u);
     asm volatile("" : "+v"(seen) : : "memory");
-    const uint32_t old = atomicAdd(a.state16_valid, 2u);
-    if (((old >> 1) & 0x3FFFFFFFu) == gridDim.x - 1u) *a.state16_valid = (old & 0x80000000u) ? 0u : 1u;
+    const uint32_t old = atomicAdd(word, 2u);
+    if (((old >> 1) & 0x3FFFFFFFu) == gridDim.x - 1u) *word = (old & 0x80000000u) ? 0u : 1u;
+  };
+  if (ACT_ROLE && tid == 0) {
+    if (SHARED && a.state16_valid != nullptr) publish_valid(a.state16_valid, XLF[1] != 0);
+    if (a.view16_valid != nullptr) publish_valid(a.view16_valid, XLF[2] != 0);
   }
   const int rowB = r * IMG_ROW + 16 * h;
   const long EA = (long)E * A;
@@ -452,6 +459,19 @@
       }
     }
   };
+  auto write_view16 = [&](long slot) {
+    const auto& a = args_here();
+    if (a.view16 != nullptr) {
+      int tid = tid_w;
+      asm volatile("" : "+v"(tid));
+      const int NC = a.v16_nc;
+      uint4* const dst16 = reinterpret_cast<uint4*>(a.view16) + (slot * EA + (long)e0 * A) * NC;
+      for (int j = tid; j < rows_ok * NC; j += 256) {
+        const int row = (int)div_small((uint32_t)j, a.v16_nc_m), c = j - row * NC;
+        dst16[j] = *reinterpret_cast<const uint4*>(lds + L.xa + (row >> 5) * 2 * xa_plane + (row & 31) * xa_row + 16 * c);
+      }
+    }
+  };
   auto write_out = [&](long slot, bool part_gs) {
     const auto& a = args_here();
     int tid = tid_w;
@@ -483,6 +503,7 @@
         }
       }
     }
+    if (!part_gs) write_view16(slot);
     if (part_gs) write_gs(slot, true);
     if (!part_gs) {
       uint8_t* dst = a.action_mask + (slot * EA + (long)e0 * A) * no;
@@ -496,6 +517,7 @@
   const int T_steps = a.T;
   const uint32_t t0 = a.t0;
   if (SHARED && ACT_ROLE && a.state16 != nullptr) write_gs(0L, false);
+  if (!ACT_ROLE) write_view16(0L);
   for (int t = 0; t < T_steps; ++t) {
     const uint32_t step = t0 + (uint32_t)t;
     forward(true, true, step);
@@ -775,7 +797,7 @@
                            uint8_t* done, float* last_val, float* info_return, int32_t* info_length,
                            uint8_t* info_terminal, float* adv, float* tgt, float gamma, float gae_lambda,
                            float* last_reward, uint8_t* last_done, int32_t* step_counter, uint16_t* state16,
-                           uint32_t* state16_valid, hipStream_t s) {
+                           uint32_t* state16_valid, uint16_t* view16, uint32_t* view16_valid, hipStream_t s) {
   MAVA_ARG_CHECK(E >= 1 && A >= 1 && O >= 2 && T >= 1 && n_actions >= 1 && time_limit >= 1, 0,
                  "mava_rollout_ff_f32: bad shape E=%d A=%d O=%d T=%d nA=%d", E, A, O, T, n_actions);
   MAVA_ARG_CHECK(actor_params && critic_params && step_count && run_return && run_length && ep_return && ep_length &&
@@ -802,6 +824,10 @@
   MAVA_ARG_CHECK(state16 == nullptr || (critic_shared && (A * O) % 8 == 0 && (uintptr_t)state16 % 16 == 0), 2,
                  "mava_rollout_ff_x16_f32: state16 needs the shared critic, A*O %% 8 == 0 (A*O=%d) and 16-byte alignment", A * O);
   a.state16 = reinterpret_cast<_Float16*>(state16); a.state16_valid = state16_valid;
+  MAVA_ARG_CHECK((view16 == nullptr) == (view16_valid == nullptr), 1, "mava_rollout_ff_records16_f32: view16 and view16_valid go together");
+  MAVA_ARG_CHECK(view16 == nullptr || (uintptr_t)view16 % 16 == 0, 2, "mava_rollout_ff_records16_f32: view16 needs 16-byte alignment");
+  a.view16 = reinterpret_cast<_Float16*>(view16); a.view16_valid = view16_valid;
+  a.v16_nc = (A + O + 8) / 8; a.v16_nc_m = 65536u / (uint32_t)a.v16_nc + 1u;
   if (critic_shared) {
     if (s1a == 5 && s1c == 17 && A >= 4) return launch_rollout<8, 5, 17, true>(a, s);
 #ifndef MAVA_FAST_BUILD
@@ -831,7 +857,7 @@
                          t0, row_offset, env_offset, reward_mode, step_count, run_return, run_length, ep_return, ep_length,
                          agents_view, global_state, action_mask, obs_step_count, action, value, reward, log_prob, done,
                          last_val, info_return, info_length, info_terminal, adv, tgt, gamma, gae_lambda, nullptr, nullptr,
-                         nullptr, nullptr, nullptr, s);
+                         nullptr, nullptr, nullptr, nullptr, nullptr, s);
 }
 
 extern "C" int mava_rollout_ff_tail_f32(const float* actor_params, int n_actions, const float* critic_params,
@@ -849,7 +875,7 @@
                          t0, row_offset, env_offset, reward_mode, step_count, run_return, run_length, ep_return, ep_length,
                          agents_view, global_state, action_mask, obs_step_count, action, value, reward, log_prob, done,
                          last_val, info_return, info_length, info_terminal, adv, tgt, gamma, gae_lambda, last_reward,
-                         last_done, step_counter, nullptr, nullptr, s);
+                         last_done, step_counter, nullptr, nullptr, nullptr, nullptr, s);
 }
 
 extern "C" int mava_rollout_ff_x16_f32(const float* actor_params, int n_actions, const float* critic_params,
@@ -869,7 +895,28 @@
                          t0, row_offset, env_offset, reward_mode, step_count, run_return, run_length, ep_return, ep_length,
                          agents_view, global_state, action_mask, obs_step_count, action, value, reward, log_prob, done,
                          last_val, info_return, info_length, info_terminal, adv, tgt, gamma, gae_lambda, last_reward,
-                         last_done, step_counter, state16, state16_valid, s);
+                         last_done, step_counter, state16, state16_valid, nullptr, nullptr, s);
+}
+
+extern "C" int mava_rollout_ff_records16_f32(const float* actor_params, int n_actions, const float* critic_params,
+                                             int critic_shared, int E, int A, int O, int T, int time_limit,
+                                             uint64_t policy_seed, uint64_t env_seed, uint32_t t0, uint32_t row_offset,
+                                             uint32_t env_offset, int reward_mode, int32_t* step_count, float* run_return,
+                                             int32_t* run_length, float* ep_return, int32_t* ep_length, float* agents_view,
+                                             float* global_state, uint8_t* action_mask, int32_t* obs_step_count,
+                                             int32_t* action, float* value, float* reward, float* log_prob, uint8_t* done,
+                                             float* last_val, float* info_return, int32_t* info_length,
+                                             uint8_t* info_terminal, float* adv, float* tgt, float gamma, float gae_lambda,
+                                             float* last_reward, uint8_t* last_done, int32_t* step_counter, uint16_t* state16,
+                                             uint32_t* state16_valid, uint16_t* view16, uint32_t* view16_valid,
+                                             hipStream_t s) {
+  MAVA_ARG_CHECK((last_reward == nullptr) == (last_done == nullptr) && (last_reward != nullptr || step_counter == nullptr), 1,
+                 "mava_rollout_ff_records16_f32: last_reward, last_done (and step_counter) go together");
+  return rollout_ff_impl(actor_params, n_actions, critic_params, critic_shared, E, A, O, T, time_limit, policy_seed, env_seed,
+                         t0, row_offset, env_offset, reward_mode, step_count, run_return, run_length, ep_return, ep_length,
+                         agents_view, global_state, action_mask, obs_step_count, action, value, reward, log_prob, done,
+                         last_val, info_return, info_length, info_terminal, adv, tgt, gamma, gae_lambda, last_reward,
+                         last_done, step_counter, state16, state16_valid, view16, view16_valid, s);
 }
 
 namespace {
diff --git a/mava_amd/learner.py b/mava_amd/learner.py
--- a/mava_amd/learner.py
+++ b/mava_amd/learner.py
@@ -153,6 +153,12 @@
         for rep in self.reps:
             rep.state16 = torch.zeros((self.T + 1, self.E, 1, self.Oc), dtype=torch.float16, device=d) if self.x16 else None
             rep.state16_valid = torch.zeros((1,), dtype=torch.int32, device=d) if self.x16 else None
+        self.view16 = (self.fused_rollout and not self.continuous and self.matmul_mode == "f16x2" and self.Oa + 1 <= 128
+                       and os.environ.get("MAVA_X16", "1") != "0" and os.environ.get("MAVA_X16_ACTOR", "1") != "0")
+        rp = 8 * ((self.Oa + 8) // 8)
+        for rep in self.reps:
+            rep.view16 = torch.zeros((self.T + 1, self.E, self.A, rp), dtype=torch.float16, device=d) if self.view16 else None
+            rep.view16_valid = torch.zeros((1,), dtype=torch.int32, device=d) if self.view16 else None
         self._learn_calls = 0
         self.fused_tail = (self.world == 1 and not self.generic and os.environ.get("MAVA_FUSED_TAIL", "1") != "0")
         self._finish_ws = ops.ppo_finish_workspace(self.Pa, self.Pc, d) if self.fused_tail else None
@@ -301,12 +307,12 @@
                 info_terminal=rep.info_terminal[n], adv=rep.adv, tgt=rep.tgt, gamma=float(s.gamma),
                 gae_lambda=float(s.gae_lambda), last_reward=rep.last_reward, last_done=rep.last_done,
                 step_counter=self.step_dev if u == 0 else None,
-                state16=rep.state16, state16_valid=rep.state16_valid)
+                state16=rep.state16, state16_valid=rep.state16_valid, view16=rep.view16, view16_valid=rep.view16_valid)
               if not ok:
                 assert u == 0
-                self.fused_rollout = self.x16 = False
+                self.fused_rollout = self.x16 = self.view16 = False
                 for r in self.reps:
-                    r.state16 = r.state16_valid = None
+                    r.state16 = r.state16_valid = r.view16 = r.view16_valid = None
                 return False
         if side:
             for st in self._roll_streams:
@@ -390,18 +396,24 @@
             else:
                 self._timed("actor_grad", ops.ppo_actor_grad, pa, av, rep.action_mask[:T].view(TEA, self.nA),
                             rep.action.view(TEA), rep.log_prob.view(TEA), rep.adv.view(TEA), stats, idx, base,
-                            self.Rb, A, self.nA, float(s.clip_eps), float(s.ent_coef), slab_a, ctx=self.ctx)
+                            self.Rb, A, self.nA, float(s.clip_eps), float(s.ent_coef), slab_a, ctx=self.ctx,
+                            input16=rep.view16[:T].view(TEA, -1) if self.view16 else None,
+                            input16_valid=rep.view16_valid if self.view16 else None)
             if not self.fused_tail:
                 ops.slab_reduce2(self.slab_a, self.Pa, self.g[: self.Pa], 2, self.g[self.P : self.P + 2], accumulate=u > 0)
         w_actor = parallel.allreduce_sum_async(self.g[: self.Pa])
         for u, rep in enumerate(self.reps):
             av = rep.agents_view[:T].view(TEA, self.Oa)
             cx = rep.global_state[:T].view(-1, self.Oc) if self.centralised else av
+            in16 = in16_valid = None
+            if self.x16:
+                in16, in16_valid = rep.state16[:T].view(-1, self.Oc), rep.state16_valid
+            elif self.view16 and not self.centralised and self.critic_share == 1:
+                in16, in16_valid = rep.view16[:T].view(TEA, -1), rep.view16_valid
             self._timed("critic_grad", ops.ppo_critic_grad, pc, cx, self.critic_share, rep.value.view(TEA), rep.tgt.view(TEA),
                         idx, base, self.Rb, A, float(s.clip_eps), float(s.vf_coef),
                         self.slab_c[u * ns : (u + 1) * ns] if per_rep else self.slab_c, ctx=self.ctx,
-                        input16=rep.state16[:T].view(-1, self.Oc) if self.x16 else None,
-                        input16_valid=rep.state16_valid if self.x16 else None)
+                        input16=in16, input16_valid=in16_valid)
             if not self.fused_tail:
                 ops.slab_reduce2(self.slab_c, self.Pc, self.g[self.Pa : self.P], 1, self.g[self.P + 2 : self.P + 3], accumulate=u > 0)
         if self.fused_tail:
diff --git a/mava_amd/ops.py b/mava_amd/ops.py
--- a/mava_amd/ops.py
+++ b/mava_amd/ops.py
@@ -386,9 +386,17 @@
 
 def ppo_actor_grad(params, agents_view, action_mask, action, old_log_prob, advantages, stats, idx, idx_base: int,
                    Rb: int, A: int, n_actions: int, clip_eps: float, ent_coef: float, slab: torch.Tensor,
-                   ctx: Optional[Ctx] = None) -> None:
+                   ctx: Optional[Ctx] = None, input16: Optional[torch.Tensor] = None,
+                   input16_valid: Optional[torch.Tensor] = None) -> None:
     _req(agents_view, torch.float32, "agents_view")
     rows, din = agents_view.shape
+    if (input16 is None) != (input16_valid is None):
+        raise ValueError("input16 and input16_valid go together")
+    if input16 is not None:
+        _req(input16, torch.float16, "input16")
+        if input16.dim() != 2 or input16.shape[0] != rows or input16.shape[1] < din:
+            raise ValueError(f"input16: expected ({rows}, >= {din}), got {tuple(input16.shape)}")
+        _req(input16_valid, torch.int32, "input16_valid", (1,))
     if rows % A:
         raise ValueError("agents_view rows must be a multiple of A")
     TE = rows // A
@@ -412,12 +420,13 @@
     _req(slab, torch.float32, "slab")
     if slab.dim() != 2 or slab.shape[1] < P + 2:
         raise ValueError("slab must be (n_slab, >= P+2)")
-    check(
-        lib().mava_ppo_actor_grad_f32(ctx_ptr(ctx), ptr(params), din, n_actions, ptr(agents_view), ptr(action_mask), ptr(action),
-                                      ptr(old_log_prob), ptr(advantages), ptr(stats), ptr(idx), idx_base, Rb, A,
-                                      clip_eps, ent_coef, ptr(slab), slab.shape[1], slab.shape[0], stream_ptr()),
-        "mava_ppo_actor_grad_f32",
-    )
+    args = (ctx_ptr(ctx), ptr(params), din, n_actions, ptr(agents_view), ptr(action_mask), ptr(action), ptr(old_log_prob),
+            ptr(advantages), ptr(stats), ptr(idx), idx_base, Rb, A, clip_eps, ent_coef, ptr(slab), slab.shape[1], slab.shape[0])
+    if input16 is not None:
+        check(lib().mava_ppo_actor_grad_x16_f32(*args, ptr(input16), ptr(input16_valid), input16.shape[1], stream_ptr()),
+              "mava_ppo_actor_grad_x16_f32")
+        return
+    check(lib().mava_ppo_actor_grad_f32(*args, stream_ptr()), "mava_ppo_actor_grad_f32")
 
 
 def ppo_critic_grad(params, critic_input, x_share: int, old_value, targets, idx, idx_base: int, Rb: int, A: int,
@@ -428,7 +437,10 @@
     if (input16 is None) != (input16_valid is None):
         raise ValueError("input16 and input16_valid go together")
     if input16 is not None:
-        _req(input16, torch.float16, "input16", tuple(critic_input.shape))
+        _req(input16, torch.float16, "input16")
+        if tuple(input16.shape) != tuple(critic_input.shape) and not (
+                x_share == 1 and input16.dim() == 2 and input16.shape[0] == critic_input.shape[0] and input16.shape[1] > din):
+            raise ValueError(f"input16: expected {tuple(critic_input.shape)} (or (rows, RP > din) with x_share == 1), got {tuple(input16.shape)}")
         _req(input16_valid, torch.int32, "input16_valid", (1,))
     _req(params, torch.float32, "params")
     P = mlp_param_count(din, 1)
@@ -450,7 +462,8 @@
     args = (ctx_ptr(ctx), ptr(params), din, ptr(critic_input), x_share, ptr(old_value), ptr(targets), ptr(idx), idx_base, Rb, A,
             clip_eps, vf_coef, ptr(slab), slab.shape[1], slab.shape[0])
     if input16 is not None:
-        check(lib().mava_ppo_critic_grad_x16_f32(*args, ptr(input16), ptr(input16_valid), stream_ptr()), "mava_ppo_critic_grad_x16_f32")
+        check(lib().mava_ppo_critic_grad_x16_f32(*args, ptr(input16), ptr(input16_valid), input16.shape[1], stream_ptr()),
+              "mava_ppo_critic_grad_x16_f32")
         return
     check(lib().mava_ppo_critic_grad_f32(*args, stream_ptr()), "mava_ppo_critic_grad_f32")
 
@@ -474,7 +487,7 @@
                reward_mode: int, env_state, agents_view, global_state, action_mask, obs_step_count, action, value,
                reward, log_prob, done, last_val, info_return, info_length, info_terminal, adv=None, tgt=None,
                gamma: float = 0.99, gae_lambda: float = 0.95, last_reward=None, last_done=None, step_counter=None,
-               state16=None, state16_valid=None) -> bool:
+               state16=None, state16_valid=None, view16=None, view16_valid=None) -> bool:
     W = A + O
     _req(actor_params, torch.float32, "actor_params")
     _req(critic_params, torch.float32, "critic_params")
@@ -512,19 +525,29 @@
         ptr(adv), ptr(tgt), gamma, gae_lambda)
     if (state16 is None) != (state16_valid is None):
         raise ValueError("state16 and state16_valid go together")
+    if (view16 is None) != (view16_valid is None):
+        raise ValueError("view16 and view16_valid go together")
     if state16 is not None:
         if not critic_shared or (A * O) % 8:
             raise ValueError("state16 needs the shared critic and A * O % 8 == 0")
         _req(state16, torch.float16, "state16", (T + 1, E, 1, A * O))
         _req(state16_valid, torch.int32, "state16_valid", (1,))
-        name = "mava_rollout_ff_x16_f32"
+    if view16 is not None:
+        _req(view16, torch.float16, "view16", (T + 1, E, A, 8 * ((W + 8) // 8)))
+        _req(view16_valid, torch.int32, "view16_valid", (1,))
+    if state16 is not None or view16 is not None:
+        name = "mava_rollout_ff_records16_f32" if view16 is not None else "mava_rollout_ff_x16_f32"
         if last_reward is not None:
             _req(last_reward, torch.float32, "last_reward", (E, A))
             _req(last_done, torch.uint8, "last_done", (E, A))
         if step_counter is not None:
             _req(step_counter, torch.int32, "step_counter", (1,))
-        rc = lib().mava_rollout_ff_x16_f32(*args, ptr(last_reward), ptr(last_done), ptr(step_counter), ptr(state16),
-                                           ptr(state16_valid), stream_ptr())
+        if view16 is not None:
+            rc = lib().mava_rollout_ff_records16_f32(*args, ptr(last_reward), ptr(last_done), ptr(step_counter), ptr(state16),
+                                                     ptr(state16_valid), ptr(view16), ptr(view16_valid), stream_ptr())
+        else:
+            rc = lib().mava_rollout_ff_x16_f32(*args, ptr(last_reward), ptr(last_done), ptr(step_counter), ptr(state16),
+                                               ptr(state16_valid), stream_ptr())
     elif last_reward is None and last_done is None and step_counter is None:
         name = "mava_rollout_ff_f32"
         rc = lib().mava_rollout_ff_f32(*args, stream_ptr())
```

Result: faster. 84.82 million env-steps/s, median of 6 (+1.4%).
